# kiliant/zklaim

Measured on AMD Instinct MI355X. Metric: Groth16 proofs/sec (zklaim gadget, alt_bn128) + G1 MSM GB/s vs HBM roofline, higher is better.
Workload: dtype u32 limbs, Montgomery (254-bit Fq/Fr: 9 x 29-bit in the accumulation, reduction and NTT kernels, 8 x 32-bit elsewhere)

## Files before the change

### include/zkg.h

```cpp
#ifndef ZKG_H
#define ZKG_H

#include <stddef.h>
#include <stdint.h>

#ifdef __cplusplus
extern "C" {
#endif

#define ZKG_OK 0
#define ZKG_ERROR 1
#define ZKG_UNSATISFIED 2
#define ZKG_PROOF_BYTES 134

typedef struct zkg_r1cs {
    uint32_t num_variables;
    uint32_t num_inputs;
    uint32_t num_constraints;
    uint32_t reserved;
    const uint32_t *a_rowptr, *a_col; const uint64_t *a_val;
    const uint32_t *b_rowptr, *b_col; const uint64_t *b_val;
    const uint32_t *c_rowptr, *c_col; const uint64_t *c_val;
} zkg_r1cs;

typedef struct zkg_pk {
    zkg_r1cs cs;
    uint32_t log_m;
    uint32_t domain_size;
    const uint64_t *alpha_g1, *beta_g1, *delta_g1;
    const uint64_t *beta_g2, *delta_g2;
    const uint64_t *A_query;
    const uint64_t *B_g1;
    const uint64_t *B_g2;
    const uint64_t *H_query;
    const uint64_t *L_query;
} zkg_pk;

typedef struct zkg_crs zkg_crs;

int  zkg_init(int device);
void zkg_shutdown(void);
const char *zkg_last_error(void);
int  zkg_device_info(char *name, size_t name_len, int *compute_units);

int zkg_ntt(uint64_t *a, unsigned logN, int inverse, int coset);
int zkg_ntt_dev(void *d_a, unsigned logN, int inverse, int coset, void *stream);

int zkg_evaluation_domain_size(size_t min_size, size_t *m, int *is_step);
int zkg_ntt_domain(uint64_t *a, size_t m, int inverse, int coset);
int zkg_ntt_domain_dev(void *d_a, size_t m, int inverse, int coset, void *stream);

typedef struct zkg_domain zkg_domain;
zkg_domain *zkg_domain_new(size_t m);
void   zkg_domain_free(zkg_domain *d);
size_t zkg_domain_size(const zkg_domain *d);
size_t zkg_domain_batch_max(const zkg_domain *d);
void   zkg_domain_set_batch_max(zkg_domain *d, size_t k);
int zkg_domain_ntt_async(zkg_domain *d, void *d_a, size_t stride , size_t count,
                         int inverse, int coset, void *stream);
int zkg_domain_lagrange_async(zkg_domain *d, const uint64_t t[4], void *d_u, void *d_z, void *stream);
void zkg_domain_stats(size_t out[3]);

typedef struct zkg_qap zkg_qap;
zkg_qap *zkg_qap_new(const zkg_r1cs *cs);
void     zkg_qap_free(zkg_qap *q);
size_t   zkg_qap_domain_size(const zkg_qap *q);
uint32_t zkg_qap_num_variables(const zkg_qap *q);
size_t   zkg_qap_batch_max(const zkg_qap *q);
void     zkg_qap_set_batch_max(zkg_qap *q, size_t k);
int      zkg_qap_witness_h_async(zkg_qap *q, const void *d_witnesses, size_t stride , size_t count,
                                 void *d_h, size_t h_stride , uint32_t *d_unsat ,
                                 void *stream);
void     zkg_qap_stats(size_t out[3]);
int      zkg_qap_instance_async(zkg_qap *q, const uint64_t t[4] , void *d_abc ,
                                size_t stride , void *d_z , void *stream);
void     zkg_qap_set_column_segment(zkg_qap *q, size_t k);
void     zkg_qap_instance_stats(size_t out[2]);

int zkg_msm_g1(const uint64_t *bases, const uint64_t *scalars, size_t n, uint64_t out_jac[12]);
int zkg_msm_g2(const uint64_t *bases, const uint64_t *scalars, size_t n, uint64_t out_jac[24]);
#define ZKG_SCALARS_MONT 1
#define ZKG_SCALARS_MOSTLY_BITS 2
int zkg_msm_g1_dev(const void *d_bases, const void *d_scalars, size_t n, int scalars_mont,
                   uint64_t out_jac[12], void *stream);
int zkg_msm_g2_dev(const void *d_bases, const void *d_scalars, size_t n, int scalars_mont,
                   uint64_t out_jac[24], void *stream);
int zkg_msm_g1_host_scalars(const void *d_bases, const uint64_t *scalars, size_t n, int scalars_mont, uint64_t out_jac[12], void *stream);
int zkg_msm_host_scalars_stats(uint32_t *out, int n);
typedef struct zkg_msm_bases zkg_msm_bases;
zkg_msm_bases *zkg_msm_g1_bases_upload(const void *d_bases, size_t n);
int zkg_msm_g1_resident(zkg_msm_bases *bases, const void *d_scalars, size_t n, int scalars_mont, uint64_t out_jac[12], void *stream);
void zkg_msm_g1_bases_free(zkg_msm_bases *bases);
int zkg_msm_g1_resident_async(zkg_msm_bases *bases, const void *d_scalars, size_t n, size_t stride , size_t count,
                              int scalars_mont, void *d_out_jac , void *stream);
size_t zkg_msm_g1_resident_batch_max(const zkg_msm_bases *bases);
void zkg_msm_resident_async_stats(size_t out[3]);
int zkg_msm_combine_gpu(const uint64_t *records_jac, size_t cpw, int slots , int chunk_log, size_t vectors, uint64_t *out_jac);
typedef struct zkg_msm_g2_bases zkg_msm_g2_bases;
zkg_msm_g2_bases *zkg_msm_g2_bases_upload(const void *d_bases , size_t n);
void   zkg_msm_g2_bases_free(zkg_msm_g2_bases *bases);
int    zkg_msm_g2_resident(zkg_msm_g2_bases *bases, const void *d_scalars, size_t n, int scalars_mont, uint64_t out_jac[24], void *stream);
int    zkg_msm_g2_resident_async(zkg_msm_g2_bases *bases, const void *d_scalars, size_t n, size_t stride, size_t count,
                                 int scalars_mont, void *d_out_jac , void *stream);
size_t zkg_msm_g2_resident_batch_max(const zkg_msm_g2_bases *bases);
int    zkg_msm_combine_g2_gpu(const uint64_t *records_jac, size_t cpw, int chunk_log, size_t vectors, uint64_t *out_jac);
int zkg_msm_g1_windows_dev(const void *d_bases, const void *d_scalars, size_t n, int scalars_mont,
                           unsigned first_window, unsigned window_stride, uint64_t out_jac[12], void *stream);
int zkg_g1_sum(const uint64_t *points_jac, size_t count, uint64_t out_jac[12]);
int zkg_g2_sum(const uint64_t *points_jac, size_t count, uint64_t out_jac[24]);

typedef struct zkg_msm_shards zkg_msm_shards;
int zkg_init_multi(const int *devices, int ndev);
zkg_msm_shards *zkg_msm_g1_shards_upload(const uint64_t *bases, size_t n, const int *devices, int ndev);
void zkg_msm_g1_shards_free(zkg_msm_shards *shards);
size_t zkg_msm_g1_shards_count(const zkg_msm_shards *shards, size_t *points);
int zkg_msm_g1_multi(const zkg_msm_shards *shards, const uint64_t *scalars, uint64_t out_jac[12], uint64_t *partials_jac);
unsigned zkg_multi_rccl_calls(void);

int zkg_g1_fixed_base_dev(const uint64_t base[8], const void *d_scalars, size_t n, void *d_out_affine, void *stream);
int zkg_g2_fixed_base_dev(const uint64_t base[16], const void *d_scalars, size_t n, void *d_out_affine, void *stream);

zkg_crs *zkg_crs_upload(const zkg_pk *pk);
zkg_crs *zkg_crs_upload_blob(const void *pk_blob, size_t len);
int zkg_pk_blob_inspect(const void *pk_blob, size_t len, uint64_t out[8]);
void     zkg_crs_free(zkg_crs *crs);
int zkg_crs_shard_h(zkg_crs *crs, const int *devices, int ndev);
uint32_t zkg_crs_num_variables(const zkg_crs *crs);

int zkg_groth16_prove(const zkg_crs *crs, const uint64_t *witness, const uint64_t r[4],
                      const uint64_t s[4], int check_satisfied, uint8_t *proof_out, size_t *proof_len);
int zkg_groth16_prove_sparse(const zkg_crs *crs, const uint8_t *tags, const uint32_t *full_index, const uint64_t *full_values, size_t count,
                             const uint64_t r[4], const uint64_t s[4], int check_satisfied, uint8_t *proof_out, size_t *proof_len);
typedef struct zkg_prove_item {
    const uint64_t *witness;
    const uint8_t  *tags; const uint32_t *full_index; const uint64_t *full_values; size_t count;
    const uint64_t *r, *s;
} zkg_prove_item;
int zkg_groth16_prove_batch(const zkg_crs *crs, const zkg_prove_item *items, size_t count, int check_satisfied,
                            uint8_t *proofs_out , int *status );
void zkg_prove_batch_stats(size_t out[3]);
size_t zkg_prove_batch_chunk(const zkg_crs *crs);
int zkg_groth16_prove_dev(const zkg_crs *crs, const void *d_witness, const uint64_t r[4], const uint64_t s[4], int check_satisfied,
                          uint8_t *proof_out, size_t *proof_len, void *stream);
int zkg_groth16_prove_batch_dev(const zkg_crs *crs, const void *d_witnesses, size_t stride , size_t count,
                                const uint64_t *rs , int check_satisfied,
                                uint8_t *proofs_out , int *status , void *stream);
void zkg_prove_dev_stats(size_t out[2]);
struct zklaim_ctx;
int zkg_groth16_prove_batch_zklaim(const zkg_crs *crs, const struct zklaim_ctx *const *ctxs, size_t count, const uint64_t *rs ,
                                   int check_satisfied, uint8_t *proofs_out , int *status );
void zkg_zklaim_witness_stats(size_t out[2]);
size_t zkg_zklaim_witness_size(size_t payloads, size_t *cap_listed);
int zkg_zklaim_witness_gpu(const struct zklaim_ctx *const *ctxs, size_t count, uint8_t *tags_out , uint32_t *index_out,
                           uint64_t *values_out, size_t cap_listed , size_t *listed_counts);
int zkg_zklaim_witness_mirror(const struct zklaim_ctx *ctx, uint8_t *tags_out , uint32_t *index_out, uint64_t *values_out, size_t cap_listed,
                              size_t *listed_count);
int zkg_groth16_prove_zklaim(const zkg_crs *crs, const struct zklaim_ctx *ctx, const uint64_t r[4], const uint64_t s[4],
                             int check_satisfied, uint8_t *proof_out, size_t *proof_len);
void zkg_prove_zklaim_stats(size_t out[2]);
int zkg_zklaim_witness_gpu_parallel(const struct zklaim_ctx *const *ctxs, size_t count, uint8_t *tags_out , uint32_t *index_out,
                                    uint64_t *values_out, size_t cap_listed , size_t *listed_counts);
int zkg_zklaim_witness_mirror_parallel(const struct zklaim_ctx *ctx, uint8_t *tags_out , uint32_t *index_out, uint64_t *values_out,
                                       size_t cap_listed, size_t *listed_count);
int zkg_qap_witness_h(const zkg_crs *crs, const uint64_t *witness, uint64_t *h_out);
int zkg_prove_stage_ms(const zkg_crs *crs, float ms[8]);
int zkg_prover_peak_in_flight(int reset);

struct zklaim_ctx;
typedef struct zkg_circuit zkg_circuit;
#define ZKG_CIRCUIT_WITH_WITNESS 1
#define ZKG_CIRCUIT_REFERENCE_QUIRK 2
zkg_circuit *zkg_zklaim_circuit_new(const struct zklaim_ctx *ctx, int flags);
zkg_circuit *zkg_zklaim_witness_new(const struct zklaim_ctx *ctx);
uint32_t zkg_circuit_num_variables(const zkg_circuit *c);
void zkg_circuit_free(zkg_circuit *c);
int zkg_circuit_r1cs(const zkg_circuit *c, zkg_r1cs *out);
const uint64_t *zkg_circuit_witness(const zkg_circuit *c);
int zkg_circuit_sparse_witness(const zkg_circuit *c, const uint8_t **tags, const uint32_t **full_index, const uint64_t **full_values, size_t *count);
int zkg_circuit_is_satisfied(const zkg_circuit *c);
long zkg_circuit_first_unsatisfied(const zkg_circuit *c);
size_t zkg_zklaim_input_map(const struct zklaim_ctx *ctx, uint64_t *out, size_t cap_elems);

typedef struct zkg_keypair zkg_keypair;
zkg_keypair *zkg_groth16_setup(const zkg_r1cs *cs, const uint64_t *trapdoor);
zkg_keypair *zkg_groth16_setup_dev(const zkg_r1cs *cs, const uint64_t *trapdoor );
void zkg_keypair_free(zkg_keypair *kp);
const zkg_pk *zkg_keypair_pk(const zkg_keypair *kp);
int zkg_keypair_swapped(const zkg_keypair *kp);
size_t zkg_keypair_pk_blob(const zkg_keypair *kp, uint8_t *out, size_t cap);
size_t zkg_keypair_vk_blob(const zkg_keypair *kp, uint8_t *out, size_t cap);
int zkg_groth16_verify(const uint8_t *vk_blob, size_t vk_len, const uint64_t *primary_input, size_t n_inputs,
                       const uint8_t *proof, size_t proof_len);
int zkg_pairing_probe(const uint64_t a[4], const uint64_t b[4], uint8_t out[384]);
typedef struct zkg_verify_item {
    const uint8_t  *vk_blob;       size_t vk_len;
    const uint64_t *primary_input; size_t n_inputs;
    const uint8_t  *proof;         size_t proof_len;
} zkg_verify_item;
int zkg_groth16_verify_batch(const zkg_verify_item *items, size_t count, uint8_t *verdicts);
void zkg_verify_batch_stats(size_t out[3]);
int zkg_pairing_product(const uint64_t *g1_affine, const uint64_t *g2_affine, size_t n, uint8_t out[384]);
int  zkg_groth16_verify_each(const zkg_verify_item *items, size_t count, uint8_t *verdicts);
void zkg_verify_each_stats(size_t out[3]);
void zkg_verify_each_set_chunk(size_t positions);
int  zkg_pairing_each(const uint64_t *g1_affine, const uint64_t *g2_affine, size_t items, size_t pairs, uint8_t *out);
int  zkg_final_exp(const uint8_t *in, size_t n, int where, uint8_t *out);
int zkg_pairing_selfcheck(const uint32_t *e, int nlimbs);

int libsnark_trusted_setup(struct zklaim_ctx *ctx);
int libsnark_prove(struct zklaim_ctx *ctx);
int libsnark_verify(struct zklaim_ctx *ctx);
void zkg_compat_reset(void);
int zkg_zklaim_prove_batch(struct zklaim_ctx *const *ctxs, size_t count, int *rc);
int zkg_zklaim_verify_batch(struct zklaim_ctx *const *ctxs, size_t count, int *rc);
void zkg_zklaim_verify_batch_stats(size_t out[4]);
int zkg_proof_decode_gpu(const uint8_t *proofs, size_t count, uint64_t *A, uint64_t *B, uint64_t *C, uint8_t *ok);
int zkg_zklaim_input_sums_gpu(const struct zklaim_ctx *const *ctxs, size_t count, const uint32_t *weights, const uint8_t *mask,
                              size_t lo, size_t hi, uint64_t *sums_out, size_t cap_elems, size_t *n_elems);
size_t zkg_zklaim_input_map_mirror(const struct zklaim_ctx *ctx, uint64_t *out, size_t cap_elems);
int  zkg_zklaim_verify_each(struct zklaim_ctx *const *ctxs, size_t count, int *rc);
void zkg_zklaim_verify_each_stats(size_t out[4]);
int zkg_zklaim_ic_each(const uint64_t *ic0, const uint64_t *ic, const struct zklaim_ctx *const *ctxs, size_t count, int where, uint64_t *out);

int zkg_point_decompress(const uint8_t *records, size_t stride, size_t offset, size_t n, int g2, int where, uint64_t *out, uint32_t *flag);
int zkg_point_compress(const uint64_t *g1, const uint64_t *g2, const uint32_t *idx, size_t npoints, size_t n, int rec, int where, uint8_t *out,
                       uint8_t guard[16]);

int zkg_field_op(int field, int op, const uint64_t *a, const uint64_t *b, size_t n, uint64_t *out);

int zkg_fr29_op(int op, const uint32_t *in, size_t n, uint32_t *out);

int zkg_fq29_op(int op, const uint32_t *in, size_t n, uint32_t *out);
int zkg_fq29_op_chain(int op, int chain, const uint32_t *in, size_t n, uint32_t *out);

int zkg_fq12_op(int op, const uint32_t *a, const uint32_t *b, size_t n, int where, uint32_t *out);

int zkg_g1_add_quad29(const uint64_t *a_jac, const uint64_t *b_jac, size_t n, int chain, uint64_t *out_jac);
int zkg_g1_add_pair29(const uint64_t *a_jac, const uint64_t *b_jac, size_t n, int chain, uint64_t *out_jac);

int zkg_curve_op(int group, int op, const uint32_t *a, const uint32_t *b, const uint32_t *k, size_t n, int chain, uint32_t *out);

// ... 8 lines not shown
```

### zklaim_amd/__init__.py

```python
from .api import (ZkgError, device_info, evaluation_domain_size, fixed_base_g1_dev, fixed_base_g2_dev, g1_sum, g2_sum, init, lib, msm_g1, msm_g1_dev, msm_g1_windows_dev,
                  msm_g2, msm_g2_dev, ntt, ntt_dev, shutdown, timing_dominant_ms, timing_reset, Crs, PK, R1CS, make_r1cs, make_pk,
                  DECLARED_SYMBOLS, ZklaimCircuit, ZklaimCtx, make_ctx, zklaim_input_map, OPS, Keypair, groth16_verify, groth16_verify_batch, verify_batch_stats, groth16_prove_batch, prove_batch_stats, groth16_prove_batch_dev, prove_dev_stats, groth16_prove_batch_zklaim, zklaim_witness_stats, zklaim_witness_size, zklaim_witness_mirror, zklaim_witness_gpu, zklaim_witness_mirror_parallel, zklaim_witness_gpu_parallel, prove_zklaim_stats, pairing_product, pairing_probe, pairing_selfcheck,
                  libsnark_trusted_setup, libsnark_prove, libsnark_verify, zklaim_prove_batch, zklaim_verify_batch, zklaim_verify_batch_stats, proof_decode_gpu, zklaim_input_sums_gpu, zklaim_input_map_mirror, ctx_blob, COMPAT_SYMBOLS, field_op, fr29_op, FR29_OPS, fq29_op, FQ29_OPS, g1_add_quad29, g1_add_pair29, curve_op, CURVE_OPS, OK, ERROR, UNSATISFIED, init_multi, MsmShards, pk_blob_inspect, ResidentBases, msm_g1_host_scalars, msm_host_scalars_stats, msm_resident_async_stats, msm_combine_gpu, ResidentBasesG2, msm_combine_g2_gpu,
                  groth16_verify_each, verify_each_stats, verify_each_set_chunk, pairing_each, final_exp, fq12_op, FQ12_OPS,
                  point_decompress, point_compress, zklaim_verify_each, zklaim_verify_each_stats, zklaim_ic_each,
                  Domain, domain_stats, Qap, qap_stats, qap_instance_stats)
```

### zklaim_amd/api.py

```python
import ctypes as C
import os
import sys

import numpy as np

_HERE = os.path.dirname(os.path.abspath(__file__))
_SO = os.path.join(_HERE, "libzkg.so")

DECLARED_SYMBOLS = [
    "zkg_init", "zkg_shutdown", "zkg_last_error", "zkg_device_info", "zkg_ntt", "zkg_ntt_dev", "zkg_evaluation_domain_size", "zkg_ntt_domain", "zkg_ntt_domain_dev", "zkg_msm_g1", "zkg_msm_g2",
    "zkg_msm_g1_dev", "zkg_msm_g2_dev", "zkg_msm_g1_windows_dev", "zkg_g1_sum", "zkg_g2_sum", "zkg_g1_fixed_base_dev", "zkg_g2_fixed_base_dev",
    "zkg_groth16_prove_batch_zklaim", "zkg_zklaim_witness_stats", "zkg_zklaim_witness_size", "zkg_zklaim_witness_gpu", "zkg_zklaim_witness_mirror",
    "zkg_crs_upload", "zkg_crs_upload_blob", "zkg_pk_blob_inspect", "zkg_crs_free", "zkg_crs_num_variables", "zkg_groth16_prove", "zkg_groth16_prove_sparse", "zkg_circuit_sparse_witness", "zkg_qap_witness_h", "zkg_prove_stage_ms", "zkg_timing_reset",
    "zkg_timing_dominant_ms", "zkg_zklaim_circuit_new", "zkg_zklaim_witness_new", "zkg_circuit_num_variables", "zkg_circuit_free", "zkg_circuit_r1cs", "zkg_circuit_witness",
    "zkg_circuit_is_satisfied", "zkg_circuit_first_unsatisfied", "zkg_zklaim_input_map", "zkg_groth16_setup", "zkg_keypair_free",
    "zkg_keypair_pk", "zkg_keypair_swapped", "zkg_keypair_pk_blob", "zkg_keypair_vk_blob", "zkg_groth16_verify", "zkg_pairing_probe", "zkg_pairing_selfcheck",
    "zkg_compat_reset", "zkg_field_op", "zkg_init_multi", "zkg_msm_g1_shards_upload", "zkg_msm_g1_shards_free", "zkg_msm_g1_shards_count",
    "zkg_msm_g1_multi", "zkg_g1_add_quad29", "zkg_crs_shard_h", "zkg_msm_g1_bases_upload", "zkg_msm_g1_resident", "zkg_msm_g1_bases_free",
    "zkg_prover_peak_in_flight", "zkg_msm_g1_host_scalars", "zkg_multi_rccl_calls", "zkg_g1_add_pair29",
    "zkg_groth16_verify_batch", "zkg_pairing_product", "zkg_verify_batch_stats",
    "zkg_groth16_prove_batch", "zkg_prove_batch_stats", "zkg_prove_batch_chunk", "zkg_zklaim_prove_batch",
    "zkg_groth16_prove_zklaim", "zkg_prove_zklaim_stats", "zkg_zklaim_witness_gpu_parallel", "zkg_zklaim_witness_mirror_parallel",
    "zkg_fr29_op", "zkg_fq29_op", "zkg_fq29_op_chain",
    "zkg_zklaim_verify_batch", "zkg_zklaim_verify_batch_stats", "zkg_proof_decode_gpu", "zkg_zklaim_input_sums_gpu", "zkg_zklaim_input_map_mirror",
    "zkg_groth16_prove_dev", "zkg_groth16_prove_batch_dev", "zkg_prove_dev_stats",
    "zkg_msm_g1_resident_async", "zkg_msm_g1_resident_batch_max", "zkg_msm_resident_async_stats", "zkg_msm_combine_gpu",
    "zkg_groth16_verify_each", "zkg_verify_each_stats", "zkg_verify_each_set_chunk", "zkg_pairing_each", "zkg_final_exp",
    "zkg_fq12_op", "zkg_point_decompress", "zkg_point_compress",
    "zkg_zklaim_verify_each", "zkg_zklaim_verify_each_stats", "zkg_zklaim_ic_each",
    "zkg_curve_op",
    "zkg_domain_new", "zkg_domain_free", "zkg_domain_size", "zkg_domain_batch_max", "zkg_domain_set_batch_max", "zkg_domain_ntt_async",
    "zkg_domain_lagrange_async", "zkg_domain_stats",
    "zkg_msm_g2_bases_upload", "zkg_msm_g2_bases_free", "zkg_msm_g2_resident", "zkg_msm_g2_resident_async", "zkg_msm_g2_resident_batch_max",
    "zkg_msm_combine_g2_gpu",
    "zkg_qap_new", "zkg_qap_free", "zkg_qap_domain_size", "zkg_qap_num_variables", "zkg_qap_batch_max", "zkg_qap_set_batch_max",
    "zkg_qap_witness_h_async", "zkg_qap_stats",
    "zkg_qap_instance_async", "zkg_qap_set_column_segment", "zkg_qap_instance_stats", "zkg_groth16_setup_dev",
    "zkg_msm_host_scalars_stats",
]
COMPAT_SYMBOLS = ["libsnark_trusted_setup", "libsnark_prove", "libsnark_verify"]


OK, ERROR, UNSATISFIED = 0, 1, 2


class ZkgError(RuntimeError):
    pass


class R1CS(C.Structure):
    _fields_ = [("num_variables", C.c_uint32), ("num_inputs", C.c_uint32), ("num_constraints", C.c_uint32), ("reserved", C.c_uint32)] + \
        [(f"{m}_{f}", C.c_void_p) for m in "abc" for f in ("rowptr", "col", "val")]


class PK(C.Structure):
    _fields_ = [("cs", R1CS), ("log_m", C.c_uint32), ("domain_size", C.c_uint32)] + \
        [(k, C.c_void_p) for k in ("alpha_g1", "beta_g1", "delta_g1", "beta_g2", "delta_g2", "A_query", "B_g1", "B_g2", "H_query", "L_query")]


_lib = None


def lib():
    global _lib
    if _lib is None:
        if not os.path.exists(_SO):
            raise ZkgError(f"{_SO} is missing: build it with `python -m zklaim_amd.build` (hipcc, gfx950)")
        if "torch" not in sys.modules and not os.environ.get("ZKG_NO_TORCH"):
            try:
                import torch
            except Exception:
                pass
        _lib = C.CDLL(_SO)
        _lib.zkg_last_error.restype = C.c_char_p
        _lib.zkg_timing_dominant_ms.restype = C.c_float
        _lib.zkg_crs_upload.restype = C.c_void_p
        _lib.zkg_crs_upload.argtypes = [C.c_void_p]
        _lib.zkg_crs_upload_blob.restype = C.c_void_p
        _lib.zkg_crs_upload_blob.argtypes = [C.c_void_p, C.c_size_t]
        _lib.zkg_crs_free.argtypes = [C.c_void_p]
    return _lib


def _check(rc, what):
    if rc != 0:
        raise ZkgError(f"{what} failed (rc={rc}): {lib().zkg_last_error().decode()}")


def _p(a):
    return None if a is None else a.ctypes.data_as(C.c_void_p)


def _u64(a):
    return np.ascontiguousarray(a, dtype=np.uint64)


def _vp(x):
    return C.c_void_p(int(x) if x else 0)


_initialised = False


def init(device=0):
    global _initialised
    _check(lib().zkg_init(int(device)), "zkg_init")
    _initialised = True


def shutdown():
    global _initialised
    if _initialised:
        lib().zkg_shutdown()
    _initialised = False


def device_info():
    name = C.create_string_buffer(128); cus = C.c_int(0)
    _check(lib().zkg_device_info(name, C.c_size_t(128), C.byref(cus)), "zkg_device_info")
    return name.value.decode(), cus.value


def field_op(field, op, a, b=None):
    a = _u64(a); limbs = 8 if field == 2 else 4
    out = np.zeros_like(a)
    bb = None if b is None else _u64(b)
    _check(lib().zkg_field_op(int(field), int(op), _p(a), _p(bb), C.c_size_t(a.size // limbs), _p(out)), "zkg_field_op")
    return out


FR29_OPS = {"mul": (0, 2, 1), "mul2": (1, 4, 2), "norm": (2, 1, 1), "add_norm": (3, 2, 1), "sub_norm": (4, 2, 1), "add_lazy": (5, 2, 1), "sub_lazy": (6, 2, 1),
            "slice": (7, 1, 1), "unslice_reduce": (8, 1, 1), "r4": (9, 7, 4), "r4_stage0": (10, 7, 4), "r4_norm_stores": (11, 7, 4),
            "r4_stage0_norm_stores": (12, 7, 4), "r2_tail": (13, 3, 2), "r2_tail_stage0": (14, 3, 2)}


def fr29_op(name, x):
    op, k, m = FR29_OPS[name]
    x = np.ascontiguousarray(x, dtype=np.uint32)
    if x.ndim != 3 or x.shape[1:] != (k, 9):
        raise ZkgError(f"fr29_op {name}: input must be (n, {k}, 9), got {x.shape}")
    out = np.zeros((x.shape[0], m, 9), np.uint32)
    _check(lib().zkg_fr29_op(int(op), _p(x), C.c_size_t(x.shape[0]), _p(out)), "zkg_fr29_op")
    return out


FQ29_OPS = {"mul": (0, 2, 1), "mul2": (1, 4, 2), "sqr": (2, 1, 1), "sqr2": (3, 2, 2), "norm": (4, 1, 1), "add": (5, 2, 1), "dbl": (6, 1, 1),
            "sub_S2_1": (7, 2, 1), "sub_S4_1": (8, 2, 1), "sub_S6_1": (9, 2, 1), "sub_S4_3": (10, 2, 1), "neg_S2_1": (11, 1, 1), "is_zero": (12, 1, 1),
            "unpack": (13, 1, 1), "to29": (14, 1, 1), "from29": (15, 1, 1), "rec64": (16, 3, 3), "bucket29": (17, 5, 4), "inverse": (18, 1, 1),
            "madd": (19, 7, 5), "add_lane": (20, 8, 4), "add_pair": (21, 8, 4), "add_quad": (22, 8, 4)}


def fq29_op(name, x, chain=0):
    op, k, m = FQ29_OPS[name]
    x = np.ascontiguousarray(x, dtype=np.uint32)
    if x.ndim != 3 or x.shape[1:] != (k, 9):
        raise ZkgError(f"fq29_op {name}: input must be (n, {k}, 9), got {x.shape}")
    out = np.zeros((x.shape[0], m, 9), np.uint32)
    _check(lib().zkg_fq29_op_chain(int(op), int(chain), _p(x), C.c_size_t(x.shape[0]), _p(out)), "zkg_fq29_op")
    return out


def g1_add_quad29(a_jac, b_jac, chain=0):
    a = _u64(a_jac); b = _u64(b_jac); out = np.zeros_like(a)
    _check(lib().zkg_g1_add_quad29(_p(a), _p(b), C.c_size_t(a.size // 12), int(chain), _p(out)), "zkg_g1_add_quad29")
    return out.reshape(-1, 12)


def g1_add_pair29(a_jac, b_jac, chain=0):
    a = _u64(a_jac); b = _u64(b_jac); out = np.zeros_like(a)
    _check(lib().zkg_g1_add_pair29(_p(a), _p(b), C.c_size_t(a.size // 12), int(chain), _p(out)), "zkg_g1_add_pair29")
    return out.reshape(-1, 12)


CURVE_OPS = {"madd": 0, "add": 1, "add_quad": 2, "dbl": 3, "dbl_affine": 4, "to_affine": 5, "mul": 6}


def curve_op(group, name, a, b=None, k=None, chain=0):
    op = CURVE_OPS[name]; w = 16 if group else 8
    a = np.ascontiguousarray(a, dtype=np.uint32)
    need_a = 2 if name == "dbl_affine" else 4
    if a.ndim != 3 or a.shape[1:] != (need_a, w):
        raise ZkgError(f"curve_op {name}: a must be (n, {need_a}, {w}), got {a.shape}")
    n = a.shape[0]
    if name in ("madd", "add", "add_quad"):
        need_b = 2 if name == "madd" else 4
        b = np.ascontiguousarray(b, dtype=np.uint32)
        if b.shape != (n, need_b, w):
            raise ZkgError(f"curve_op {name}: b must be ({n}, {need_b}, {w}), got {b.shape}")
    else:
        b = None
    if name == "mul":
# ... 77 lines not shown

    def free(self):
        if self._h:
            lib().zkg_domain_free(C.c_void_p(self._h)); self._h = None


def domain_stats():
    out = (C.c_size_t * 3)()
    lib().zkg_domain_stats(out)
    return tuple(int(v) for v in out)


class Qap:

    def __init__(self, cs):
        L = lib()
        L.zkg_qap_new.restype = C.c_void_p
        L.zkg_qap_new.argtypes = [C.c_void_p]
        L.zkg_qap_free.argtypes = [C.c_void_p]
        for name in ("zkg_qap_domain_size", "zkg_qap_batch_max"):
            getattr(L, name).restype = C.c_size_t
            getattr(L, name).argtypes = [C.c_void_p]
        L.zkg_qap_num_variables.restype = C.c_uint32
        L.zkg_qap_num_variables.argtypes = [C.c_void_p]
        L.zkg_qap_set_batch_max.argtypes = [C.c_void_p, C.c_size_t]
        L.zkg_qap_witness_h_async.argtypes = [C.c_void_p, C.c_void_p, C.c_size_t, C.c_size_t, C.c_void_p, C.c_size_t, C.c_void_p, C.c_void_p]
        L.zkg_qap_instance_async.argtypes = [C.c_void_p, C.c_void_p, C.c_void_p, C.c_size_t, C.c_void_p, C.c_void_p]
        L.zkg_qap_set_column_segment.argtypes = [C.c_void_p, C.c_size_t]
        self._h = L.zkg_qap_new(C.byref(cs))
        if not self._h:
            raise ZkgError("zkg_qap_new failed: " + L.zkg_last_error().decode())
        self.m, self.n = self.domain_size(), self.num_variables()

    def witness_h_async(self, d_w_ptr, count, stride, d_h_ptr, h_stride, d_unsat_ptr=0, stream=0):
        _check(lib().zkg_qap_witness_h_async(C.c_void_p(self._h), _vp(d_w_ptr), C.c_size_t(stride), C.c_size_t(count), _vp(d_h_ptr), C.c_size_t(h_stride),
                                             _vp(d_unsat_ptr), _vp(stream)), "zkg_qap_witness_h_async")

    def instance_async(self, t, d_abc_ptr, stride=None, d_z_ptr=0, stream=0):
        tt = None if t is None else _u64(t).reshape(-1)
        if tt is not None and tt.size != 4:
            raise ZkgError("zkg_qap_instance_async: t is 4 limbs")
        _check(lib().zkg_qap_instance_async(C.c_void_p(self._h), _p(tt), _vp(d_abc_ptr), C.c_size_t(self.n + 1 if stride is None else stride), _vp(d_z_ptr),
                                            _vp(stream)), "zkg_qap_instance_async")

    def set_column_segment(self, k):
        lib().zkg_qap_set_column_segment(C.c_void_p(self._h), C.c_size_t(k))

    def domain_size(self):
        return int(lib().zkg_qap_domain_size(C.c_void_p(self._h)))

    def num_variables(self):
        return int(lib().zkg_qap_num_variables(C.c_void_p(self._h)))

    def batch_max(self):
        return int(lib().zkg_qap_batch_max(C.c_void_p(self._h)))

    def set_batch_max(self, k):
        lib().zkg_qap_set_batch_max(C.c_void_p(self._h), C.c_size_t(k))

    def free(self):
        if self._h:
            lib().zkg_qap_free(C.c_void_p(self._h)); self._h = None


def qap_stats():
    out = (C.c_size_t * 3)()
    lib().zkg_qap_stats(out)
    return tuple(int(v) for v in out)


def qap_instance_stats():
    out = (C.c_size_t * 2)()
    lib().zkg_qap_instance_stats(out)
    return tuple(int(v) for v in out)


def msm_g1(bases, scalars):
    bases = _u64(bases); scalars = _u64(scalars); out = np.zeros(12, np.uint64)
    _check(lib().zkg_msm_g1(_p(bases), _p(scalars), C.c_size_t(scalars.size // 4), _p(out)), "zkg_msm_g1")
    return out


def msm_g2(bases, scalars):
    bases = _u64(bases); scalars = _u64(scalars); out = np.zeros(24, np.uint64)
    _check(lib().zkg_msm_g2(_p(bases), _p(scalars), C.c_size_t(scalars.size // 4), _p(out)), "zkg_msm_g2")
    return out


def init_multi(devices):
    global _initialised
    d = (C.c_int * len(devices))(*devices)
    _check(lib().zkg_init_multi(d, len(devices)), "zkg_init_multi")
    _initialised = True


class MsmShards:

    def __init__(self, bases, devices):
        bases = _u64(bases)
        L = lib()
        L.zkg_msm_g1_shards_upload.restype = C.c_void_p
        L.zkg_msm_g1_shards_upload.argtypes = [C.c_void_p, C.c_size_t, C.c_void_p, C.c_int]
        L.zkg_msm_g1_shards_free.argtypes = [C.c_void_p]
        L.zkg_msm_g1_multi.argtypes = [C.c_void_p, C.c_void_p, C.c_void_p, C.c_void_p]
        d = (C.c_int * len(devices))(*devices)
        self.n = bases.size // 8; self.ndev = len(devices)
        self._h = L.zkg_msm_g1_shards_upload(_p(bases), self.n, d, len(devices))
        if not self._h:
            raise ZkgError("zkg_msm_g1_shards_upload failed: " + L.zkg_last_error().decode())

    def msm(self, scalars, with_partials=False):
        scalars = _u64(scalars); out = np.zeros(12, np.uint64); parts = np.zeros((self.ndev, 12), np.uint64)
        assert scalars.size // 4 == self.n
        _check(lib().zkg_msm_g1_multi(C.c_void_p(self._h), _p(scalars), _p(out), _p(parts)), "zkg_msm_g1_multi")
        return (out, parts) if with_partials else out

    def free(self):
        if self._h:
            lib().zkg_msm_g1_shards_free(C.c_void_p(self._h)); self._h = None

    def __del__(self):
        try:
            self.free()
        except Exception:
            pass


SCALARS_MONT, SCALARS_MOSTLY_BITS = 1, 2


def msm_g1_dev(d_bases, d_scalars, n, scalars_mont=False, stream=0, mostly_bits=False):
    out = np.zeros(12, np.uint64)
    flags = (SCALARS_MONT if scalars_mont else 0) | (SCALARS_MOSTLY_BITS if mostly_bits else 0)
    _check(lib().zkg_msm_g1_dev(_vp(d_bases), _vp(d_scalars), C.c_size_t(n), flags, _p(out), _vp(stream)), "zkg_msm_g1_dev")
    return out


def msm_g1_host_scalars(d_bases, scalars_host_ptr, n, scalars_mont=False, stream=0):
    out = np.zeros(12, np.uint64)
    lib().zkg_msm_g1_host_scalars.argtypes = [C.c_void_p, C.c_void_p, C.c_size_t, C.c_int, C.c_void_p, C.c_void_p]
    _check(lib().zkg_msm_g1_host_scalars(_vp(d_bases), _vp(scalars_host_ptr), C.c_size_t(n), SCALARS_MONT if scalars_mont else 0, _p(out), _vp(stream)), "zkg_msm_g1_host_scalars")
    return out


def msm_host_scalars_stats():
    out = (C.c_uint32 * 18)()
    words = lib().zkg_msm_host_scalars_stats(out, 18)
    if words < 2:
        return None
    pieces = int(out[0])
    return {"pieces": pieces, "stream_waits": int(out[1]),
            "heavy": [None if out[2 + 2 * k] == 0xFFFFFFFF else int(out[2 + 2 * k]) for k in range(pieces)],
            "pair": [bool(out[3 + 2 * k]) for k in range(pieces)]}


class _ResidentBases:
    _PREFIX = None
    _LIMBS = 0

    def _fn(self, suffix, argtypes, restype=C.c_int):
        fn = getattr(lib(), self._PREFIX + suffix)
        fn.argtypes = argtypes; fn.restype = restype
        return fn

    def __init__(self, d_bases, n):
        self._h = self._fn("_bases_upload", [C.c_void_p, C.c_size_t], C.c_void_p)(_vp(d_bases), C.c_size_t(n))
        if not self._h:
            raise ZkgError(self._PREFIX + "_bases_upload failed: " + last_error())
        self.n = n

    def msm(self, d_scalars, scalars_mont=False, stream=0):
        out = np.zeros(self._LIMBS, np.uint64)
        fn = self._fn("_resident", [C.c_void_p, C.c_void_p, C.c_size_t, C.c_int, C.c_void_p, C.c_void_p])
        _check(fn(C.c_void_p(self._h), _vp(d_scalars), C.c_size_t(self.n), SCALARS_MONT if scalars_mont else 0, _p(out), _vp(stream)), self._PREFIX + "_resident")
        return out

    def msm_async(self, d_scalars_ptr, d_out_ptr, count=1, stride=None, scalars_mont=False, stream=0):
        fn = self._fn("_resident_async", [C.c_void_p, C.c_void_p, C.c_size_t, C.c_size_t, C.c_size_t, C.c_int, C.c_void_p, C.c_void_p])
        _check(fn(C.c_void_p(self._h), _vp(d_scalars_ptr), C.c_size_t(self.n), C.c_size_t(self.n if stride is None else stride),
                  C.c_size_t(count), SCALARS_MONT if scalars_mont else 0, _vp(d_out_ptr), _vp(stream)), self._PREFIX + "_resident_async")

    def batch_max(self):
        return int(self._fn("_resident_batch_max", [C.c_void_p], C.c_size_t)(C.c_void_p(self._h)))

    def free(self):
        if self._h:
            self._fn("_bases_free", [C.c_void_p], None)(C.c_void_p(self._h)); self._h = None


class ResidentBases(_ResidentBases):
    _PREFIX = "zkg_msm_g1"
    _LIMBS = 12


class ResidentBasesG2(_ResidentBases):
    _PREFIX = "zkg_msm_g2"
    _LIMBS = 24


def msm_resident_async_stats():
    out = (C.c_size_t * 3)()
    lib().zkg_msm_resident_async_stats(out)
    return tuple(int(v) for v in out)


def _msm_combine(name, limbs, records_jac, cpw, slots, chunk_log, vectors, slot_args):
    rec = _u64(records_jac)
    if rec.size != vectors * cpw * slots * limbs:
        raise ZkgError("%s: records_jac must hold vectors x cpw x %s points of %d limbs" % (name, "slots" if slot_args else slots, limbs))
    out = np.zeros((vectors, limbs), np.uint64)
    fn = getattr(lib(), "zkg_" + name)
    fn.argtypes = [C.c_void_p, C.c_size_t] + [C.c_int] * len(slot_args) + [C.c_int, C.c_size_t, C.c_void_p]
    _check(fn(_p(rec), C.c_size_t(cpw), *slot_args, int(chunk_log), C.c_size_t(vectors), _p(out)), "zkg_" + name)
    return out


def msm_combine_gpu(records_jac, cpw, slots, chunk_log, vectors=1):
    return _msm_combine("msm_combine_gpu", 12, records_jac, cpw, slots, chunk_log, vectors, [int(slots)])


def msm_combine_g2_gpu(records_jac, cpw, chunk_log, vectors=1):
    return _msm_combine("msm_combine_g2_gpu", 24, records_jac, cpw, 2, chunk_log, vectors, [])


def msm_g1_windows_dev(d_bases, d_scalars, n, first_window, window_stride, scalars_mont=False, stream=0):
    out = np.zeros(12, np.uint64)
    _check(lib().zkg_msm_g1_windows_dev(_vp(d_bases), _vp(d_scalars), C.c_size_t(n), int(scalars_mont), C.c_uint(first_window), C.c_uint(window_stride),
                                        _p(out), _vp(stream)), "zkg_msm_g1_windows_dev")
    return out


def msm_g2_dev(d_bases, d_scalars, n, scalars_mont=False, stream=0, mostly_bits=False):
    out = np.zeros(24, np.uint64)
    flags = (SCALARS_MONT if scalars_mont else 0) | (SCALARS_MOSTLY_BITS if mostly_bits else 0)
    _check(lib().zkg_msm_g2_dev(_vp(d_bases), _vp(d_scalars), C.c_size_t(n), flags, _p(out), _vp(stream)), "zkg_msm_g2_dev")
    return out


def g1_sum(points_jac):
    pts = _u64(points_jac); out = np.zeros(12, np.uint64)
    _check(lib().zkg_g1_sum(_p(pts), C.c_size_t(pts.size // 12), _p(out)), "zkg_g1_sum")
    return out


def g2_sum(points_jac):
    pts = _u64(points_jac); out = np.zeros(24, np.uint64)
    _check(lib().zkg_g2_sum(_p(pts), C.c_size_t(pts.size // 24), _p(out)), "zkg_g2_sum")
    return out


def fixed_base_g1_dev(base, d_scalars, n, d_out, stream=0):
    base = _u64(base)
    _check(lib().zkg_g1_fixed_base_dev(_p(base), _vp(d_scalars), C.c_size_t(n), _vp(d_out), _vp(stream)), "zkg_g1_fixed_base_dev")


def fixed_base_g2_dev(base, d_scalars, n, d_out, stream=0):
    base = _u64(base)
    _check(lib().zkg_g2_fixed_base_dev(_p(base), _vp(d_scalars), C.c_size_t(n), _vp(d_out), _vp(stream)), "zkg_g2_fixed_base_dev")


def timing_reset():
    lib().zkg_timing_reset()


def timing_dominant_ms():
    n = C.c_int(0)
    ms = lib().zkg_timing_dominant_ms(C.byref(n))
    return float(ms), n.value


def make_r1cs(n, l, A, B, Cm, keep):
    cs = R1CS()
    cs.num_variables, cs.num_inputs, cs.num_constraints = n, l, len(A[0]) - 1
    for name, (rp, col, val) in zip("abc", (A, B, Cm)):
        rp = np.ascontiguousarray(rp, np.uint32); col = np.ascontiguousarray(col, np.uint32); val = _u64(val)
        keep += [rp, col, val]
        setattr(cs, f"{name}_rowptr", rp.ctypes.data); setattr(cs, f"{name}_col", col.ctypes.data); setattr(cs, f"{name}_val", val.ctypes.data)
    return cs


def make_pk(cs, arrays, log_m, keep, domain_size=0):
    pk = PK(); pk.cs = cs; pk.log_m = log_m; pk.domain_size = domain_size
    for k in ("alpha_g1", "beta_g1", "delta_g1", "beta_g2", "delta_g2", "A_query", "B_g1", "B_g2", "H_query", "L_query"):
        a = _u64(arrays[k]); keep.append(a)
        setattr(pk, k, a.ctypes.data)
    return pk


class Crs:

    def __init__(self, pk=None, blob=None, m=None):
        if blob is not None:
            buf = (C.c_ubyte * len(blob)).from_buffer_copy(blob)
            self._h = lib().zkg_crs_upload_blob(C.cast(buf, C.c_void_p), C.c_size_t(len(blob)))
            self.m = m
        else:
            self._h = lib().zkg_crs_upload(C.byref(pk))
            self.m = pk.domain_size or (1 << pk.log_m)
        if not self._h:
            raise ZkgError("zkg_crs_upload failed: " + lib().zkg_last_error().decode())

    def prove(self, witness, r, s, check_satisfied=True):
        out = np.zeros(256, np.uint8); ln = C.c_size_t(0)
        rc = lib().zkg_groth16_prove(C.c_void_p(self._h), _p(_u64(witness)), _p(_u64(r)), _p(_u64(s)), int(check_satisfied), _p(out), C.byref(ln))
        if rc not in (OK, UNSATISFIED):
            _check(rc, "zkg_groth16_prove")
# ... 664 lines not shown
```

### zklaim_amd/csrc/capi.hip

```cpp
#include "common.hpp"
#include "fq29.hip.hpp"
#include "fr29.hip.hpp"
#include "../../include/zkg.h"
#include <atomic>
#include <condition_variable>
#include <cstring>
#include <memory>
#include <mutex>
#include <thread>
#include <dlfcn.h>
#include <rccl/rccl.h>

namespace zk {

static thread_local std::string t_error;
static std::string g_error;
static std::mutex g_err_mu;
void set_error(const std::string &msg) { t_error = msg; std::lock_guard<std::mutex> lk(g_err_mu); g_error = msg; }
bool hip_ok(hipError_t e, const char *what, const char *file, int line) {
    if (e == hipSuccess) return true;
    set_error(std::string(what) + ": " + hipGetErrorString(e) + " at " + file + ":" + std::to_string(line));
    return false;
}

// ... 584 lines not shown
        hip_ok(hipDeviceSynchronize(), "sync", __FILE__, __LINE__) &&
        hip_ok(hipMemcpy(a, buf.p, bytes, hipMemcpyDeviceToHost), "D2H", __FILE__, __LINE__)) rc = ZKG_OK;
    buf.release();
    return rc;
}

int zkg_evaluation_domain_size(size_t min_size, size_t *m, int *is_step) {
    DomainShape sh;
    if (!evaluation_domain_shape(min_size, sh)) { set_error("zkg_evaluation_domain_size: no radix-2 or step domain for that size"); return ZKG_ERROR; }
    if (m) *m = sh.m;
    if (is_step) *is_step = sh.step ? 1 : 0;
    return ZKG_OK;
}
int zkg_ntt_domain_dev(void *d_a, size_t m, int inverse, int coset, void *stream) {
    REQUIRE_INIT();
    DomainShape sh;
    if (!domain_shape_of(m, sh)) { set_error("zkg_ntt_domain: m is neither 2^k nor 2^a + 2^b (get_evaluation_domain would not return it)"); return ZKG_ERROR; }
    if (!sh.step) return zkg_ntt_dev(d_a, sh.log_m, inverse, coset, stream);
    hipStream_t s = (hipStream_t)stream;
    StepDomain *d = step_domain(m, s);
    if (!d) return ZKG_ERROR;
    DevBuf scratch;
    if (scratch.reserve(m * NTT_SCRATCH_BYTES)) return ZKG_ERROR;
    int rc = step_ntt_run(d, (Fr *)d_a, inverse != 0, coset != 0, s, scratch.as<Fr>());
    if (!hip_ok(hipStreamSynchronize(s), "sync", __FILE__, __LINE__)) rc = ZKG_ERROR;
    scratch.release();
    return rc;
}
int zkg_ntt_domain(uint64_t *a, size_t m, int inverse, int coset) {
    REQUIRE_INIT();
    if (!a || m < 2) { set_error("zkg_ntt_domain: bad argument"); return ZKG_ERROR; }
    std::lock_guard<std::mutex> lk(g_host_ntt_mu);
    size_t bytes = m * 32;
    DevBuf buf;
    if (buf.reserve(bytes)) return ZKG_ERROR;
    int rc = ZKG_ERROR;
    if (hip_ok(hipMemcpy(buf.p, a, bytes, hipMemcpyHostToDevice), "H2D", __FILE__, __LINE__) &&
        zkg_ntt_domain_dev(buf.p, m, inverse, coset, nullptr) == ZKG_OK &&
        hip_ok(hipDeviceSynchronize(), "sync", __FILE__, __LINE__) &&
        hip_ok(hipMemcpy(a, buf.p, bytes, hipMemcpyDeviceToHost), "D2H", __FILE__, __LINE__)) rc = ZKG_OK;
    buf.release();
    return rc;
}

static constexpr size_t DOMAIN_WORKSPACE_CAP = (size_t)1 << 30;
static constexpr size_t DOMAIN_MAX_GROUP = 65535;
struct zkg_domain {
    DomainShape sh; int device = 0; std::mutex mu;
    DevBuf scratch;
    HandleOrder order;
    size_t bmax_default = 1, bmax = 1;
};
static thread_local size_t t_domain_stats[3];
static zkg_domain *domain_new_impl(size_t m) {
    if (g_device < 0) { set_error("zkg_init not called"); return nullptr; }
    DomainShape sh;
    if (m < 2 || !domain_shape_of(m, sh)) { set_error("zkg_domain_new: m is neither 2^k (k <= 28) nor 2^a + 2^b (get_evaluation_domain would not return it)"); return nullptr; }
    if (wrong_device_refused("zkg_domain_new", g_device, "zkg_init selected (the domain tables live there)")) return nullptr;
    std::unique_ptr<zkg_domain> d(new zkg_domain());
    d->sh = sh; d->device = g_device;
    d->bmax_default = d->bmax = std::max<size_t>(1, std::min(DOMAIN_MAX_GROUP, DOMAIN_WORKSPACE_CAP / (m * NTT_SCRATCH_BYTES)));
    const bool tables = sh.step ? step_domain(m, nullptr) != nullptr : ntt_domain(sh.log_m, nullptr) != nullptr;
    if (!tables || !hip_ok(hipStreamSynchronize(nullptr), "hipStreamSynchronize", __FILE__, __LINE__) || d->order.create()) return nullptr;
    return d.release();
}
static int domain_ntt_async_impl(zkg_domain *d, void *d_a, size_t stride, size_t count, int inverse, int coset, void *stream) {
    static const char *who = "zkg_domain_ntt_async";
    for (size_t &v : t_domain_stats) v = 0;
    if (count == 0) return ZKG_OK;
    REQUIRE_INIT();
    if (!d || !d_a) { set_error(std::string(who) + ": bad argument (null handle or pointer)"); return ZKG_ERROR; }
    const size_t m = d->sh.m;
    if (async_vectors_refused(who, m, "m", stride, count, d->device, "the handle was made on") ||
        dev_range_refused(d_a, ((count - 1) * stride + m) * 32, 16, d->device, who, "d_a", "handle")) return ZKG_ERROR;
    hipStream_t s = (hipStream_t)stream;
    std::lock_guard<std::mutex> lk(d->mu);
    NttDomain *nd = nullptr; StepDomain *sd = nullptr;
    if (d->sh.step) sd = step_domain(m, s); else nd = ntt_domain(d->sh.log_m, s);
    if (!nd && !sd) return ZKG_ERROR;
    size_t waits = 0, groups = 0, done = 0;
    const size_t need = std::min(d->bmax, count) * m * NTT_SCRATCH_BYTES;
    if (d->order.grow(d->scratch, need, waits) || d->order.order_behind(s)) return ZKG_ERROR;
    Fr *a = (Fr *)d_a;
    int rc = ZKG_OK;
    while (done < count && rc == ZKG_OK) {
        const size_t g = std::min(d->bmax, count - done);
        Fr *ag = a + done * stride;
        const hipEvent_t ev = done + g == count ? d->order.ev : nullptr;
        rc = sd ? step_ntt_run(sd, ag, inverse != 0, coset != 0, s, d->scratch.as<Fr>(), (unsigned)g, stride, m, ev)
                : ntt_run(nd, ag, inverse, coset, s, d->scratch.as<Fr>(), (unsigned)g, stride, m, ev);
        if (rc == ZKG_OK) { done += g; ++groups; }
    }
    t_domain_stats[0] = done; t_domain_stats[1] = groups; t_domain_stats[2] = waits;
    if (rc == ZKG_OK) { d->order.carried(s); return ZKG_OK; }
    d->order.record(s);
    return ZKG_ERROR;
}
static int domain_lagrange_async_impl(zkg_domain *d, const uint64_t t[4], void *d_u, void *d_z, void *stream) {
    static const char *who = "zkg_domain_lagrange_async";
    REQUIRE_INIT();
    if (!d || !t || !d_u) { set_error(std::string(who) + ": bad argument (null handle or pointer)"); return ZKG_ERROR; }
    if (wrong_device_refused(who, d->device, "the handle was made on") || dev_range_refused(d_u, d->sh.m * 32, 16, d->device, who, "d_u", "handle") ||
        (d_z && dev_range_refused(d_z, 32, 16, d->device, who, "d_z", "handle"))) return ZKG_ERROR;
    Fr tf; memcpy(tf.v, t, 32);
    hipStream_t s = (hipStream_t)stream;
    std::lock_guard<std::mutex> lk(d->mu);
    if (d->order.order_behind(s) || domain_lagrange_dev(d->sh, tf, (Fr *)d_u, (Fr *)d_z, s, d->order.ev)) return ZKG_ERROR;
    d->order.carried(s);
    return ZKG_OK;
}
zkg_domain *zkg_domain_new(size_t m) { return c_boundary<zkg_domain *>("zkg_domain_new", nullptr, [&] { return domain_new_impl(m); }); }
void zkg_domain_free(zkg_domain *d) {
    if (!d) return;
    c_boundary("zkg_domain_free", 0, [&] {
        int cur = 0; (void)hipGetDevice(&cur);
        if (cur != d->device) (void)hipSetDevice(d->device);
        d->order.destroy();
        d->scratch.release();
        if (cur != d->device) (void)hipSetDevice(cur);
        delete d;
        return 0;
    });
}
size_t zkg_domain_size(const zkg_domain *d) { return d ? d->sh.m : 0; }
size_t zkg_domain_batch_max(const zkg_domain *d) { return d ? d->bmax : 0; }
void zkg_domain_set_batch_max(zkg_domain *d, size_t k) {
    if (!d) return;
    c_boundary("zkg_domain_set_batch_max", 0, [&] { std::lock_guard<std::mutex> lk(d->mu); d->bmax = clamp_batch_max(k, d->bmax_default); return 0; });
}
int zkg_domain_ntt_async(zkg_domain *d, void *d_a, size_t stride, size_t count, int inverse, int coset, void *stream) {
    return c_boundary("zkg_domain_ntt_async", ZKG_ERROR, [&] { return domain_ntt_async_impl(d, d_a, stride, count, inverse, coset, stream); });
}
int zkg_domain_lagrange_async(zkg_domain *d, const uint64_t t[4], void *d_u, void *d_z, void *stream) {
    return c_boundary("zkg_domain_lagrange_async", ZKG_ERROR, [&] { return domain_lagrange_async_impl(d, t, d_u, d_z, stream); });
}
void zkg_domain_stats(size_t out[3]) { if (out) for (int i = 0; i < 3; ++i) out[i] = t_domain_stats[i]; }

int zkg_msm_g1_dev(const void *d_bases, const void *d_scalars, size_t n, int scalars_mont, uint64_t out_jac[12], void *stream) {
    REQUIRE_INIT();
    G1 r;
    if (msm_g1((const G1Affine *)d_bases, (const uint32_t *)d_scalars, n, (scalars_mont & ZKG_SCALARS_MONT) != 0, &r, (hipStream_t)stream, (scalars_mont & ZKG_SCALARS_MOSTLY_BITS) != 0)) return ZKG_ERROR;
    store_norm(out_jac, r);
    return ZKG_OK;
}
int zkg_msm_g1_host_scalars(const void *d_bases, const uint64_t *scalars, size_t n, int scalars_mont, uint64_t out_jac[12], void *stream) {
    REQUIRE_INIT();
    if (!out_jac || (n && (!d_bases || !scalars))) { set_error("zkg_msm_g1_host_scalars: bad argument"); return ZKG_ERROR; }
    G1 r;
    if (msm_g1_host_scalars((const G1Affine *)d_bases, (const uint32_t *)scalars, n, (scalars_mont & ZKG_SCALARS_MONT) != 0, &r, (hipStream_t)stream)) return ZKG_ERROR;
    store_norm(out_jac, r);
    return ZKG_OK;
}
int zkg_msm_host_scalars_stats(uint32_t *out, int n) { return out && n >= 0 ? msm_host_scalars_stats(out, n) : 0; }
int zkg_msm_g1_windows_dev(const void *d_bases, const void *d_scalars, size_t n, int scalars_mont, unsigned first_window, unsigned window_stride,
                           uint64_t out_jac[12], void *stream) {
    REQUIRE_INIT();
    if (!window_stride) { set_error("zkg_msm_g1_windows_dev: window_stride must be positive"); return ZKG_ERROR; }
    G1 r; const G1Affine *b = (const G1Affine *)d_bases;
    if (msm_shared(&b, 1, nullptr, (const uint32_t *)d_scalars, n, (scalars_mont & ZKG_SCALARS_MONT) != 0, &r, nullptr, (hipStream_t)stream, first_window, window_stride,
                   (scalars_mont & ZKG_SCALARS_MOSTLY_BITS) != 0)) return ZKG_ERROR;
    store_norm(out_jac, r);
    return ZKG_OK;
}
struct MsmResident { WindowTable table; MsmJob *job = nullptr; std::mutex mu; int device = 0; hipEvent_t ev_in = nullptr, ev_out = nullptr; };
struct zkg_msm_bases : MsmResident {};
struct zkg_msm_g2_bases : MsmResident {};
struct MsmResidentG1 { using Handle = zkg_msm_bases; using Point = G1; static constexpr bool g2 = false; static constexpr size_t limbs = 12; static constexpr unsigned n_log = 27; static constexpr const char *prefix = "zkg_msm_g1"; };
struct MsmResidentG2 { using Handle = zkg_msm_g2_bases; using Point = G2; static constexpr bool g2 = true; static constexpr size_t limbs = 24; static constexpr unsigned n_log = 25; static constexpr const char *prefix = "zkg_msm_g2"; };
static constexpr size_t G2_RESIDENT_BUCKET_CAP = (size_t)1 << 30;

extern "C++" {
static void resident_free(MsmResident *h) {
    int cur = 0; (void)hipGetDevice(&cur);
    if (cur != h->device) (void)hipSetDevice(h->device);
    if (h->job) { (void)hipStreamSynchronize(msm_job_stream(h->job)); msm_job_destroy(h->job); }
    if (h->ev_in) (void)hipEventDestroy(h->ev_in);
    if (h->ev_out) (void)hipEventDestroy(h->ev_out);
    h->table.release();
    if (cur != h->device) (void)hipSetDevice(cur);
}
template <class G> static typename G::Handle *resident_upload(const void *d_bases, size_t n) {
    const std::string who = std::string(G::prefix) + "_bases_upload";
    if (g_device < 0) { set_error("zkg_init not called"); return nullptr; }
    if (!d_bases || n == 0 || n >= ((size_t)1 << G::n_log)) { set_error(who + ": bad argument (1 <= n < 2^" + std::to_string(G::n_log) + ")"); return nullptr; }
    typename G::Handle *h = new (std::nothrow) typename G::Handle();
    if (!h) { set_error(who + ": out of memory"); return nullptr; }
    (void)hipGetDevice(&h->device);
    h->job = msm_job_create(nullptr, true);
    bool ok = h->job != nullptr && hip_ok(hipEventCreateWithFlags(&h->ev_in, hipEventDisableTiming), "hipEventCreate", __FILE__, __LINE__) &&
              hip_ok(hipEventCreateWithFlags(&h->ev_out, hipEventDisableTiming), "hipEventCreate", __FILE__, __LINE__);
    if constexpr (G::g2) ok = ok && window_table_build_g2(h->table, (const G2Affine *)d_bases, n, table_window_bits(n), nullptr) == 0;
    else ok = ok && window_table_build_g1(h->table, (const G1Affine *)d_bases, n, table_window_bits(n), nullptr) == 0 && window_table_records29(h->table, nullptr) == 0;
    if (!ok || !hip_ok(hipDeviceSynchronize(), "sync", __FILE__, __LINE__)) { resident_free(h); delete h; return nullptr; }
    msm_job_set_window(h->job, h->table.c);
    if constexpr (!G::g2) msm_job_set_row_merge(h->job, n >= 49152 ? 2u : 1u);
    return h;
}
static MsmBases resident_table_set(const MsmResident *h) { MsmBases b; b.p = h->table.buf.p; b.g2 = h->table.g2; b.level_stride = h->table.n; b.p29 = h->table.rec29.p; return b; }
template <class G> static int resident_sync(MsmResident *h, const void *d_scalars, size_t n, int scalars_mont, uint64_t *out_jac, void *stream) {
    const std::string who = std::string(G::prefix) + "_resident";
    REQUIRE_INIT();
    if (!h || !d_scalars || !out_jac || n != h->table.n) { set_error(who + ": bad argument (n must be the handle's point count)"); return ZKG_ERROR; }
    if (wrong_device_refused(who.c_str(), h->device, "the bases were uploaded on")) return ZKG_ERROR;
    std::lock_guard<std::mutex> lk(h->mu);
    ZK_HIP(hipEventRecord(h->ev_in, (hipStream_t)stream));
    ZK_HIP(hipStreamWaitEvent(msm_job_stream(h->job), h->ev_in, 0));
    const MsmBases b = resident_table_set(h);
    typename G::Point r;
    msm_job_set_device_finish(h->job, false);
    int rc;
    {
        ReserveGuard guard(msm_job_stream(h->job));
        rc = msm_job_launch(h->job, &b, 1, (const uint32_t *)d_scalars, n, (scalars_mont & ZKG_SCALARS_MONT) != 0, nullptr);
    }
    if constexpr (G::g2) rc = rc || msm_job_finish(h->job, nullptr, &r); else rc = rc || msm_job_finish(h->job, &r, nullptr);
    if (rc) return ZKG_ERROR;
    store_norm(out_jac, r);
    return ZKG_OK;
}
static thread_local size_t t_resident_async_stats[3];
template <class G> static size_t resident_batch_max(const MsmResident *h) {
    size_t p = MSM_MULTI_MAX_VECTORS;
    if constexpr (G::g2) p = std::min<size_t>(p, std::max<size_t>(1, G2_RESIDENT_BUCKET_CAP / msm_table_bucket_bytes(h->table.c, true)));
    while (p > 1 && !msm_multi_supported(h->table.n, h->table.c, (uint32_t)p)) --p;
    return p;
}
template <class G> static int resident_async(MsmResident *h, const void *d_scalars, size_t n, size_t stride, size_t count, int scalars_mont, void *d_out_jac, void *stream) {
    const std::string who_s = std::string(G::prefix) + "_resident_async"; const char *who = who_s.c_str();
    for (size_t &v : t_resident_async_stats) v = 0;
    if (count == 0) return ZKG_OK;
    REQUIRE_INIT();
    if (!h || !d_scalars || !d_out_jac || n != h->table.n) { set_error(who_s + ": bad argument (n must be the handle's point count)"); return ZKG_ERROR; }
    if (async_vectors_refused(who, n, "n", stride, count, h->device, "the bases were uploaded on")) return ZKG_ERROR;
    if (dev_range_refused(d_scalars, ((count - 1) * stride + n) * 32, 16, h->device, who, "d_scalars", "handle") ||
        dev_range_refused(d_out_jac, count * G::limbs * 8, 8, h->device, who, "d_out_jac", "handle")) return ZKG_ERROR;
    const size_t bmax = resident_batch_max<G>(h);
    const bool mont = (scalars_mont & ZKG_SCALARS_MONT) != 0;
    const uint32_t *sc = (const uint32_t *)d_scalars; uint64_t *out = (uint64_t *)d_out_jac;
    std::lock_guard<std::mutex> lk(h->mu);
    hipStream_t js = msm_job_stream(h->job);
    ZK_HIP(hipEventRecord(h->ev_in, (hipStream_t)stream));
    ZK_HIP(hipStreamWaitEvent(js, h->ev_in, 0));
    const MsmBases b = resident_table_set(h);
    msm_job_set_device_finish(h->job, true);
    int rc = ZKG_OK;
    size_t groups = 0, waits = 0, done = 0;
    while (done < count && rc == ZKG_OK) {
        const size_t g = std::min(bmax, count - done);
        ReserveGuard guard(js);
        const uint32_t *sg = sc + done * stride * 8;
        rc = g > 1 ? msm_job_launch_multi(h->job, &b, 1, sg, n, stride * 8, (uint32_t)g, mont) : msm_job_launch(h->job, &b, 1, sg, n, mont, nullptr);
        if (rc == ZKG_OK) rc = msm_job_finish_dev(h->job, out + done * G::limbs);
        waits += guard.drains;
        if (rc == ZKG_OK) { done += g; ++groups; }
    }
    const bool ordered = hip_ok(hipEventRecord(h->ev_out, js), "hipEventRecord", __FILE__, __LINE__) &&
                         hip_ok(hipStreamWaitEvent((hipStream_t)stream, h->ev_out, 0), "hipStreamWaitEvent", __FILE__, __LINE__);
    t_resident_async_stats[0] = done; t_resident_async_stats[1] = groups; t_resident_async_stats[2] = waits;
    return rc == ZKG_OK && ordered ? ZKG_OK : ZKG_ERROR;
}
}
void zkg_msm_resident_async_stats(size_t out[3]) { if (out) for (int i = 0; i < 3; ++i) out[i] = t_resident_async_stats[i]; }
#define ZKG_RESIDENT_ENTRIES(NAME, G)                                                                                                                       \
    G::Handle *NAME##_bases_upload(const void *d_bases, size_t n) {                                                                                         \
        return c_boundary<G::Handle *>(#NAME "_bases_upload", nullptr, [&] { return resident_upload<G>(d_bases, n); });                                    \
    }                                                                                                                                                       \
    void NAME##_bases_free(G::Handle *h) {                                                                                                                  \
        if (h) c_boundary(#NAME "_bases_free", 0, [&] { resident_free(h); delete h; return 0; });                                                           \
    }                                                                                                                                                       \
    int NAME##_resident(G::Handle *h, const void *d_scalars, size_t n, int scalars_mont, uint64_t *out_jac, void *stream) {                                \
        return c_boundary(#NAME "_resident", ZKG_ERROR, [&] { return resident_sync<G>(h, d_scalars, n, scalars_mont, out_jac, stream); });                  \
    }                                                                                                                                                       \
    int NAME##_resident_async(G::Handle *h, const void *d_scalars, size_t n, size_t stride, size_t count, int scalars_mont, void *d_out_jac, void *stream) { \
        return c_boundary(#NAME "_resident_async", ZKG_ERROR, [&] { return resident_async<G>(h, d_scalars, n, stride, count, scalars_mont, d_out_jac, stream); }); \
    }                                                                                                                                                       \
    size_t NAME##_resident_batch_max(const G::Handle *h) {                                                                                                  \
        return h ? c_boundary<size_t>(#NAME "_resident_batch_max", 0, [&] { return resident_batch_max<G>(h); }) : 0;                                        \
    }
ZKG_RESIDENT_ENTRIES(zkg_msm_g1, MsmResidentG1)
ZKG_RESIDENT_ENTRIES(zkg_msm_g2, MsmResidentG2)
#undef ZKG_RESIDENT_ENTRIES
int zkg_msm_combine_gpu(const uint64_t *records_jac, size_t cpw, int slots, int chunk_log, size_t vectors, uint64_t *out_jac) {
    return c_boundary("zkg_msm_combine_gpu", ZKG_ERROR, [&]() -> int { REQUIRE_INIT(); return msm_combine_records(false, records_jac, cpw, slots, chunk_log, vectors, out_jac); });
}
int zkg_msm_combine_g2_gpu(const uint64_t *records_jac, size_t cpw, int chunk_log, size_t vectors, uint64_t *out_jac) {
    return c_boundary("zkg_msm_combine_g2_gpu", ZKG_ERROR, [&]() -> int { REQUIRE_INIT(); return msm_combine_records(true, records_jac, cpw, 2, chunk_log, vectors, out_jac); });
}
int zkg_msm_g2_dev(const void *d_bases, const void *d_scalars, size_t n, int scalars_mont, uint64_t out_jac[24], void *stream) {
    REQUIRE_INIT();
    G2 r;
    if (msm_g2((const G2Affine *)d_bases, (const uint32_t *)d_scalars, n, (scalars_mont & ZKG_SCALARS_MONT) != 0, &r, (hipStream_t)stream, (scalars_mont & ZKG_SCALARS_MOSTLY_BITS) != 0)) return ZKG_ERROR;
    store_norm(out_jac, r);
    return ZKG_OK;
}
static int msm_host(const uint64_t *bases, const uint64_t *scalars, size_t n, uint64_t *out, int g2) {
    REQUIRE_INIT();
    if (n && (!bases || !scalars)) { set_error("zkg_msm: null input"); return ZKG_ERROR; }
    size_t bb = n * (g2 ? 128 : 64), sb = n * 32;
    DevBuf db, ds;
    if (db.reserve(bb + 16) || ds.reserve(sb + 16)) return ZKG_ERROR;
    int rc = ZKG_ERROR;
    if ((!n || (hip_ok(hipMemcpy(db.p, bases, bb, hipMemcpyHostToDevice), "H2D", __FILE__, __LINE__) &&
                hip_ok(hipMemcpy(ds.p, scalars, sb, hipMemcpyHostToDevice), "H2D", __FILE__, __LINE__))))
        rc = g2 ? zkg_msm_g2_dev(db.p, ds.p, n, 0, out, nullptr) : zkg_msm_g1_dev(db.p, ds.p, n, 0, out, nullptr);
    db.release(); ds.release();
    return rc;
// ... 301 lines not shown
```

### zklaim_amd/csrc/common.hpp

```cpp
#pragma once
#include <hip/hip_runtime.h>
#include <stdint.h>
#include <stddef.h>
#include <string>
#include <vector>
#include <functional>
#include <map>
#include <mutex>
#include "curve.hip.hpp"
#include "c_boundary.hpp"

struct zklaim_ctx;

namespace zk {

bool hip_ok(hipError_t e, const char *what, const char *file, int line);
#define ZK_HIP(expr) do { if (!::zk::hip_ok((expr), #expr, __FILE__, __LINE__)) return ZKG_ERROR; } while (0)
#define ZK_HIP_V(expr) do { if (!::zk::hip_ok((expr), #expr, __FILE__, __LINE__)) return; } while (0)

struct DevBuf {
    void *p = nullptr; size_t cap = 0;
    int reserve(size_t bytes);
    void release();
    template <class T> T *as() const { return reinterpret_cast<T *>(p); }
};

struct ReserveGuard;
extern thread_local ReserveGuard *t_reserve_guard;
struct ReserveGuard {
    hipStream_t stream; size_t drains = 0; ReserveGuard *prev;
    explicit ReserveGuard(hipStream_t s) : stream(s), prev(t_reserve_guard) { t_reserve_guard = this; }
    ReserveGuard(const ReserveGuard &) = delete;
    ReserveGuard &operator=(const ReserveGuard &) = delete;
    ~ReserveGuard() { t_reserve_guard = prev; }
};

struct ScopedDevBuf : DevBuf {
    ScopedDevBuf() = default;
    ScopedDevBuf(const ScopedDevBuf &) = delete;
    ScopedDevBuf &operator=(const ScopedDevBuf &) = delete;
    ~ScopedDevBuf() { release(); }
};

struct HandleOrder {
    hipEvent_t ev = nullptr; bool pending = false; hipStream_t last = nullptr;
    int create();
    int order_behind(hipStream_t s);
    int wait_host();
    int grow(DevBuf &ws, size_t need, size_t &waits);
    void carried(hipStream_t s) { pending = true; last = s; }
    void record(hipStream_t s);
    void destroy();
};
inline size_t clamp_batch_max(size_t k, size_t dflt) { return k == 0 || k > dflt ? dflt : k; }

struct KernelTimer {
    std::vector<std::pair<hipEvent_t, hipEvent_t>> pairs; size_t used = 0; bool enabled = true, pending = false;
    size_t calls = 0, calls_seen = 0, calls_timed = 0; bool sample = true;
    void new_call();
    void begin(hipStream_t s); void end(hipStream_t s);
    float drain(int *launches);
    void reset();
};
extern KernelTimer g_dominant_timer;

void host_parallel_for(int n, const std::function<void(int)> &fn);
void host_parallel_for_wait(int n, const std::function<void(int)> &fn);
void host_parallel_for_spawn(int n, const std::function<void(int)> &fn);

struct NttDomain {
    unsigned logn = 0;
    DevBuf tw_fwd, tw_inv;
    DevBuf coset_pre;
    DevBuf icoset_post;
    DevBuf tw_fwd29, tw_inv29, coset_pre29, icoset_post29;
    DevBuf scratch;
    Fr n_inv;
    std::mutex mu; bool first_stream_set = false; hipStream_t first_stream = nullptr;
    std::map<hipStream_t, DevBuf> stream_scratch;
    Fr *scratch_for(hipStream_t s);
    int init(unsigned logn, hipStream_t s);
    void release();
};
NttDomain *ntt_domain(unsigned logn, hipStream_t s);
int ntt_run(NttDomain *d, Fr *d_a, int inverse, int coset, hipStream_t s, Fr *scratch = nullptr, unsigned batch = 1, size_t batch_stride = 0,
            size_t scratch_stride = 0, hipEvent_t done = nullptr);
static constexpr size_t NTT_SCRATCH_BYTES = 40;
int ntt_run_ex(NttDomain *d, Fr *d_a, bool inverse, const Fr *pre, const Fr *post, const Fr *post_scalar, hipStream_t s, Fr *scratch = nullptr,
               unsigned batch = 1, size_t batch_stride = 0, const void *pre29 = nullptr, const void *post29 = nullptr, size_t scratch_stride = 0, hipEvent_t done = nullptr);
int ntt_table29(DevBuf &out, const Fr *d_in, size_t n, hipStream_t s);

struct DomainShape { size_t m = 0, big = 0, small = 0; bool step = false; unsigned log_m = 0;  };
bool evaluation_domain_shape(size_t min_size, DomainShape &d);
bool domain_shape_of(size_t m, DomainShape &d);
Fr fr_root_of_unity_pow2(unsigned logn);
int domain_lagrange(const DomainShape &d, const Fr &t, std::vector<Fr> &u, Fr &Zt);
Fr domain_vanishing_at(const DomainShape &d, const Fr &t);
int domain_lagrange_dev(const DomainShape &d, const Fr &t, Fr *d_u, Fr *d_z, hipStream_t s, hipEvent_t done = nullptr);

struct StepDomain {
    DomainShape shape;
    NttDomain *dbig = nullptr, *dsmall = nullptr;
    DevBuf w;
    DevBuf winv_half;
    DevBuf g_pow, ginv_pow;
    DevBuf zinv;
    Fr zinv_small;
    Fr big_inv, small_inv, half;
    int init(const DomainShape &sh, hipStream_t s);
    void release();
};
StepDomain *step_domain(size_t m, hipStream_t s);
int step_ntt_run(StepDomain *d, Fr *d_a, bool inverse, bool coset, hipStream_t s, Fr *scratch, unsigned batch = 1, size_t batch_stride = 0,
                 size_t scratch_stride = 0, hipEvent_t done = nullptr);
int powers_table(Fr *d_out, size_t n, const Fr &base, const Fr &scale, hipStream_t s);
void ntt_release_all();
int ntt_configure();

static constexpr int MSM_MAX_SETS = 4;
struct MsmBases { const void *p = nullptr; bool g2 = false; size_t level_stride = 0; uint32_t index_sub = 0; const uint32_t *remap = nullptr; const void *p29 = nullptr; };
struct OwnedCsr { std::vector<uint32_t> rp[3], col[3]; std::vector<uint64_t> val[3]; };
struct WindowTable { DevBuf buf, rec29; size_t n = 0; int c = 0, W = 0; bool g2 = false; void release() { buf.release(); rec29.release(); n = 0; } };
int window_table_records29(WindowTable &t, hipStream_t s);
int window_table_build_g1(WindowTable &t, const G1Affine *d_bases, size_t n, int c, hipStream_t s);
int table_window_bits(size_t n);
int window_table_build_g2(WindowTable &t, const G2Affine *d_bases, size_t n, int c, hipStream_t s);
struct MsmJob;
MsmJob *msm_job_create(hipStream_t s, bool own_stream, bool high_priority = false);
hipStream_t msm_job_stream(MsmJob *j);
void msm_job_set_window_subset(MsmJob *j, uint32_t w0, uint32_t ws);
void msm_job_set_skewed(MsmJob *j, bool skewed);
void msm_job_set_row_merge(MsmJob *j, uint32_t f);
void msm_job_set_window(MsmJob *j, int c);
void msm_job_set_critical(MsmJob *j, bool critical);
static constexpr unsigned CRIT_PRIORITY_MIN_LOG = 20;
bool crit_priority_for(int part, unsigned log_m);
bool crit_priority_enabled();
void msm_job_destroy(MsmJob *j);
int msm_job_launch(MsmJob *job, const MsmBases *sets, int nsets, const uint32_t *d_scalars, size_t n, bool scalars_mont, const uint32_t *d_gather = nullptr);
int msm_job_finish(MsmJob *job, G1 *out_g1, G2 *out_g2);
bool msm_multi_supported(size_t n, int c, uint32_t count);
static constexpr uint32_t MSM_MULTI_MAX_VECTORS = 16;
static constexpr size_t ZKG_MSM_ASYNC_MAX_COUNT = (size_t)1 << 24, ZKG_MSM_ASYNC_MAX_STRIDE = (size_t)1 << 32;
int msm_job_launch_multi(MsmJob *job, const MsmBases *sets, int nsets, const uint32_t *d_scalars, size_t n, size_t scalar_stride, uint32_t count, bool scalars_mont);
int msm_job_finish_multi(MsmJob *job, G1 *out_g1, G2 *out_g2);
void msm_job_set_device_finish(MsmJob *j, bool on);
int msm_job_finish_dev(MsmJob *job, uint64_t *d_out);
int msm_combine_records(bool g2, const uint64_t *records_jac, size_t cpw, int slots, int chunk_log, size_t vectors, uint64_t *out_jac);
size_t msm_table_bucket_bytes(int c, bool g2);
static constexpr uint32_t SUBSET_NONE = 0xffffffffu;
int witness_classify(const Fr *d_z, size_t n1, uint8_t *d_tags, uint32_t *d_listed, uint32_t *d_count, hipStream_t s, const uint32_t *d_subset_pos = nullptr);
int gather_points_g1(const G1Affine *d_src, const uint32_t *d_idx, size_t count, uint32_t index_sub, G1Affine *d_out, hipStream_t s);
int gather_points_g2(const G2Affine *d_src, const uint32_t *d_idx, size_t count, uint32_t index_sub, G2Affine *d_out, hipStream_t s);
int scatter_points_g1(const G1Affine *d_src, const uint32_t *d_idx, size_t count, G1Affine *d_out, hipStream_t s);
int scatter_points_g2(const G2Affine *d_src, const uint32_t *d_idx, size_t count, G2Affine *d_out, hipStream_t s);
struct OnesSum {
    DevBuf partials; void *host = nullptr; size_t host_bytes = 0; bool g2 = false; int nsets = 0; void release();
    const G1 &g1(int i) const { return reinterpret_cast<const G1 *>(host)[i]; }
    const G2 &g2pt(int i) const { return reinterpret_cast<const G2 *>(host)[i]; }
};
int ones_sum_launch(OnesSum &o, const MsmBases *sets, int nsets, const uint8_t *d_tags, size_t n1, hipStream_t s);
int ones_sum_launch_multi(OnesSum &o, const MsmBases *sets, int nsets, const uint8_t *d_tags, size_t tag_stride, size_t n1, uint32_t count, hipStream_t s);
int msm_g1(const G1Affine *d_bases, const uint32_t *d_scalars, size_t n, bool scalars_mont, G1 *out, hipStream_t s, bool mostly_bits = false);
int msm_g2(const G2Affine *d_bases, const uint32_t *d_scalars, size_t n, bool scalars_mont, G2 *out, hipStream_t s, bool mostly_bits = false);
int msm_g1_host_scalars(const G1Affine *d_bases, const uint32_t *h_scalars, size_t n, bool scalars_mont, G1 *out, hipStream_t s);
int msm_host_scalars_stats(uint32_t *out, int n);
int msm_shared(const G1Affine *const *d_g1_bases, int n_g1, const G2Affine *d_g2_bases, const uint32_t *d_scalars, size_t n,
               bool scalars_mont, G1 *out_g1, G2 *out_g2, hipStream_t s, uint32_t w0 = 0, uint32_t ws = 1,
               bool mostly_bits = false);
int fixed_base_g1(const G1Affine &base, const uint32_t *d_scalars, size_t n, G1Affine *d_out, hipStream_t s, bool scalars_mont = false);
int fixed_base_g2(const G2Affine &base, const uint32_t *d_scalars, size_t n, G2Affine *d_out, hipStream_t s, bool scalars_mont = false);
void msm_release_all();
int msm_configure();

int compress_g1_records(const G1Affine *d_in, size_t n, uint8_t *d_out, hipStream_t s);
int compress_kc_records(const G2Affine *d_g2, const G1Affine *d_g1, const uint32_t *d_idx, size_t nidx, uint8_t *d_out, hipStream_t s);

static constexpr size_t VERIFY_PROD_BLOCKS = 64;
int verify_g2_subgroup(const G2Affine *d_B, size_t n, uint8_t *d_ok, hipStream_t s);
int verify_g1_mul128(const G1Affine *d_in, const uint32_t *d_w, size_t nw, size_t n, G1Affine *d_out, hipStream_t s);
int verify_miller(const G1Affine *d_P, const G2Affine *d_Q, const uint8_t *d_use, size_t n, void *d_out, hipStream_t s);
int verify_fq12_product(const void *d_in, size_t lo, size_t hi, void *d_partial, void *d_out, hipStream_t s);
int verify_proof_decode_b(const uint8_t *d_rec, size_t n, G2Affine *d_B, uint8_t *d_dec, hipStream_t s);
int verify_proof_decode_ac(const uint8_t *d_rec, size_t n, G1Affine *d_AC, uint8_t *d_dec, hipStream_t s);
int verify_use_mask(size_t n, const uint8_t *d_in_g2, const uint8_t *d_dec_b, const uint8_t *d_dec_ac, uint8_t *d_use, hipStream_t s);
static constexpr size_t ZV_SUM_SLICES = 16;
int verify_zklaim_input_sums(const uint8_t *d_pub, uint32_t npl, size_t base, const uint32_t *d_w, const uint8_t *d_mask, size_t lo, size_t hi,
                             void *d_part, void *d_out, hipStream_t s);
size_t zklaim_bit_table_entries(uint32_t npl);
size_t zklaim_bit_table_tmp_bytes(uint32_t npl);
int verify_zklaim_bit_table(const G1Affine *d_ic, uint32_t npl, void *d_tmp, G1Affine *d_T, hipStream_t s);
int verify_zklaim_ic_each(const G1Affine *d_ic0, const G1Affine *d_T, const uint8_t *d_pub, uint32_t npl, size_t n, G1Affine *d_out,
                          const G1Affine *d_c, G1Affine *d_negc, hipStream_t s);
void zklaim_ic_each_device_code_on_host(const G1Affine &ic0, const G1Affine *ic, const uint8_t *pub, uint32_t npl, size_t n, G1Affine *out);
void verify_keys_release_all();
int initialised_device();
int dev_range_refused(const void *d, size_t bytes, size_t align, int device, const char *who, const char *what, const char *owner);
int wrong_device_refused(const char *who, int device, const char *made);
int async_vectors_refused(const char *who, size_t n, const char *n_name, size_t stride, size_t count, int device, const char *made);
int verify_ic_each(const G1Affine *d_ic0, const G1Affine *d_ic, uint32_t nidx, const void *d_x, size_t n, G1Affine *d_out, hipStream_t s);
int verify_g2_replicate(const G2Affine *d_key2, size_t n, G2Affine *d_Q, hipStream_t s);
size_t verify_final_exp_ws_bytes(size_t n);
int verify_final_exp_check(const void *d_M, size_t n, uint32_t pairs, void *d_ws, const void *d_ab, uint8_t *d_verdict, void *d_gt, hipStream_t s);
void final_exp_device_code_on_host(const uint8_t in[384], uint8_t out[384]);
enum { FQ12_MUL = 0, FQ12_SQR, FQ12_LINE, FQ12_CSQR, FQ12_INV, FQ12_CONJ, FQ12_FROB1, FQ12_FROB2, FQ12_FROB3, FQ12_MUL_BY_V, FQ12_OPS };
int verify_fq12_op(int op, const void *d_a, const void *d_b, size_t n, void *d_out, hipStream_t s);
void fq12_op_device_code_on_host(int op, const uint32_t a[96], const uint32_t b[96], uint32_t out[96]);
struct VerifyWorkspace { DevBuf buf; hipStream_t s = nullptr, s2 = nullptr; hipEvent_t ev = nullptr, ev2 = nullptr; };
VerifyWorkspace *verify_workspace_acquire();
void verify_workspace_release(VerifyWorkspace *w);
void verify_workspace_destroy(VerifyWorkspace *w);
void verify_release_all();

struct ZwPlan { uint32_t k = 0, per = 0, n = 0, cap = 0; };
uint32_t zklaim_payload_vars_host();
bool zklaim_witness_plan(uint32_t k, ZwPlan &pl);
bool zklaim_witness_plan_for_n(size_t n, ZwPlan &pl);
size_t zklaim_witness_input_bytes(const ZwPlan &pl, uint32_t P);
void zklaim_witness_pack(const ZwPlan &pl, const struct ::zklaim_ctx *const *ctxs, uint32_t P, uint8_t *host_in, uint8_t *ok);
extern thread_local size_t t_zklaim_witness_stats[2];
extern thread_local size_t t_prove_zklaim_stats[2];
int zklaim_witness_launch(const ZwPlan &pl, uint32_t P, uint8_t *d_in, uint32_t *d_desc, Fr *d_vals, uint32_t *d_idx, uint8_t *d_tags, size_t tag_stride, hipStream_t s);
bool zklaim_witness_par_ready(const ZwPlan &pl);
size_t zklaim_witness_par_input_bytes(const ZwPlan &pl, uint32_t P);
void zklaim_witness_par_pack(const ZwPlan &pl, const struct ::zklaim_ctx *const *ctxs, uint32_t P, uint8_t *host_in, uint8_t *ok);
int zklaim_witness_par_launch(const ZwPlan &pl, uint32_t P, uint8_t *d_in, uint32_t *d_desc, Fr *d_vals, uint32_t *d_idx, uint8_t *d_tags, size_t tag_stride, hipStream_t s);
void zklaim_witness_release_all();

void store_norm(uint64_t *out, const G1 &p);
void store_norm(uint64_t *out, const G2 &p);
G1 load_norm_g1(const uint64_t *in);
G2 load_norm_g2(const uint64_t *in);

}
```

### zklaim_amd/csrc/host/horner_jac.hpp

```cpp
#pragma once
#include "../curve.hip.hpp"
#include <cstring>

namespace zk {

static inline Fq fq_sqr_host(const Fq &a) {
    typedef unsigned __int128 u128;
    constexpr uint64_t P4[4] = {Fq::p64(0), Fq::p64(1), Fq::p64(2), Fq::p64(3)};
    uint64_t A[4], r[8];
    memcpy(A, a.v, 32);
    u128 x = (u128)A[0] * A[1];                r[1] = (uint64_t)x; uint64_t c = (uint64_t)(x >> 64);
    x = (u128)A[0] * A[2] + c;                 r[2] = (uint64_t)x; c = (uint64_t)(x >> 64);
    x = (u128)A[0] * A[3] + c;                 r[3] = (uint64_t)x; r[4] = (uint64_t)(x >> 64);
    x = (u128)A[1] * A[2] + r[3];              r[3] = (uint64_t)x; c = (uint64_t)(x >> 64);
    x = (u128)A[1] * A[3] + r[4] + c;          r[4] = (uint64_t)x; r[5] = (uint64_t)(x >> 64);
    x = (u128)A[2] * A[3] + r[5];              r[5] = (uint64_t)x; r[6] = (uint64_t)(x >> 64);
    r[7] = r[6] >> 63;
    for (int j = 6; j >= 2; --j) r[j] = (r[j] << 1) | (r[j - 1] >> 63);
    r[1] <<= 1;
    x = (u128)A[0] * A[0];                     r[0] = (uint64_t)x; c = (uint64_t)(x >> 64);
    x = (u128)r[1] + c;                        r[1] = (uint64_t)x; c = (uint64_t)(x >> 64);
    x = (u128)A[1] * A[1] + r[2] + c;          r[2] = (uint64_t)x; c = (uint64_t)(x >> 64);
    x = (u128)r[3] + c;                        r[3] = (uint64_t)x; c = (uint64_t)(x >> 64);
    x = (u128)A[2] * A[2] + r[4] + c;          r[4] = (uint64_t)x; c = (uint64_t)(x >> 64);
    x = (u128)r[5] + c;                        r[5] = (uint64_t)x; c = (uint64_t)(x >> 64);
    x = (u128)A[3] * A[3] + r[6] + c;          r[6] = (uint64_t)x; c = (uint64_t)(x >> 64);
    r[7] += c;
    uint64_t top = 0;
    for (int i = 0; i < 4; ++i) {
        const uint64_t m = r[i] * FqParams::INV64;
        c = 0;
        for (int j = 0; j < 4; ++j) { x = (u128)m * P4[j] + r[i + j] + c; r[i + j] = (uint64_t)x; c = (uint64_t)(x >> 64); }
        x = (u128)r[i + 4] + c + top; r[i + 4] = (uint64_t)x; top = (uint64_t)(x >> 64);
    }
    uint64_t s[4]; unsigned long long br = 0;
    for (int j = 0; j < 4; ++j) s[j] = __builtin_subcll(r[4 + j], P4[j], br, &br);
    const uint64_t keep = 0ull - (uint64_t)br;
    for (int j = 0; j < 4; ++j) s[j] ^= (s[j] ^ r[4 + j]) & keep;
    Fq out; memcpy(out.v, s, 32);
    return out;
}

template <class F> static inline XYZZ<F> xyzz_times_pow2(const XYZZ<F> &p, uint32_t n) {
    if (p.is_inf() || n == 0) return p;
    if constexpr (std::is_same<F, Fq>::value) {
        if (n >= 3) {
            Fq X = p.x * p.zz, Y = p.y * p.zzz, Z = p.zz;
            for (uint32_t i = 0; i < n; ++i) {
                const Fq A = fq_sqr_host(X), B = fq_sqr_host(Y), C = fq_sqr_host(B);
                const Fq D = (fq_sqr_host(X + B) - A - C).dbl(), E = A.dbl() + A, E2 = fq_sqr_host(E);
                Z = (Y * Z).dbl();
                X = E2 - D.dbl();
                Y = E * (D - X) - C.dbl().dbl().dbl();
            }
            if (Z.is_zero()) return XYZZ<Fq>::inf();
            const Fq zz = fq_sqr_host(Z);
            return {X, Y, zz, zz * Z};
        }
    }
    XYZZ<F> r = p;
    for (uint32_t i = 0; i < n; ++i) r = r.dbl();
    return r;
}

}
```

### zklaim_amd/csrc/msm.hip

```cpp
#include "common.hpp"
#include "fq29.hip.hpp"
#include "host/horner_jac.hpp"
#include "../../include/zkg.h"
#include <algorithm>
#include <chrono>
#include <cstdio>
#include <cstdlib>
#include <cstring>
#include <mutex>

#define ZK_VGPR_CAP(n) __attribute__((amdgpu_num_vgpr((n) / 2)))
static constexpr int ACC29_VGPRS = 192;

namespace zk {

static constexpr int SCALAR_BITS = 255;
template <class F> struct RedGeom { static constexpr int LANES_LOG = sizeof(F) == sizeof(Fq) ? 7 : 6, LANES = 1 << LANES_LOG, THREADS = 4 * LANES; };
static constexpr int RED_L_LOG_TINY = 0, RED_L_LOG_SMALL = 2, RED_L_LOG_LARGE = 4;
static constexpr size_t RED_SMALL_BUCKETS = (size_t)1 << 16, RED_LARGE_BUCKETS = (size_t)1 << 18;
static constexpr int MAX_C = 16;
static constexpr uint32_t HEAVY_S = 512;
static constexpr uint32_t HEAVY_T_MAX = 1024;
static constexpr uint32_t CLASS_HIST_COPIES = 8;
static constexpr int HEAVY_PART_BLOCKS = 512, HEAVY_MERGE_BLOCKS = 128;
static constexpr int SORT_THREADS = 1024;
static constexpr int SCAN_ITEMS = 4;

struct MsmGeom { uint32_t c, W, B, Wt, w0, ws; };
struct SetLayout { size_t buckets, items, heavy, partials, folded, red_out; };
template <class F> struct BaseView {
    const Affine<F> *p; size_t level_stride; const uint32_t *gather; uint32_t index_sub, B; const uint32_t *remap;
    template <bool PLAIN = false> ZK_D Affine<F> load(uint32_t e, size_t gb) const {
        if constexpr (PLAIN) return p[e >> 1];
        uint32_t i = e >> 1;
        if (gather) i = gather[i];
        if (remap) i = remap[i];
        if (i < index_sub) return Affine<F>::inf();
        return p[(level_stride ? (gb / B) * level_stride : 0) + (i - index_sub)];
    }
};
template <class F> struct ViewSet { BaseView<F> v[MSM_MAX_SETS]; };
struct HeavyItem { uint32_t start, end, gb, single; };
struct HeavyBucket { uint32_t gb, first_item, nparts; };

static MsmGeom pick_geom(size_t n, int window_hint, uint32_t w0 = 0, uint32_t ws = 1) {
    int lg = 0; while (((size_t)1 << (lg + 1)) <= n) ++lg;
    int c = lg >= 15 ? 16 : lg >= 11 ? 12 : lg + 1;
    if (c < 4) c = 4;
    if (window_hint > 0) c = window_hint;
    static const char *force = getenv("ZKG_MSM_C");
    if (force && atoi(force) >= 2) c = atoi(force);
    if (c > MAX_C) c = MAX_C;
    MsmGeom g; g.c = c; g.Wt = (SCALAR_BITS + c - 1) / c; g.B = 1u << (c - 1);
    g.w0 = w0; g.ws = ws ? ws : 1; g.W = w0 < g.Wt ? (g.Wt - w0 + g.ws - 1) / g.ws : 0;
    return g;
}

ZK_D uint32_t bits_at(const uint32_t v[8], uint32_t off, uint32_t c) {
    uint32_t limb = off >> 5, sh = off & 31;
    if (limb >= 8) return 0;
    uint64_t x = v[limb];
    if (limb + 1 < 8) x |= (uint64_t)v[limb + 1] << 32;
    return (uint32_t)(x >> sh) & ((1u << c) - 1);
}

ZK_D void sort_wave_priority() { __builtin_amdgcn_s_setprio(3); }


struct ZeroList { uint32_t *p[4]; uint32_t words[4]; };
__global__ __launch_bounds__(256) void k_digits(const uint32_t *scalars, const uint32_t *gather, size_t n, int mont, MsmGeom g, uint32_t *digits, ZeroList zl) {
    sort_wave_priority();
    size_t i = (size_t)blockIdx.x * blockDim.x + threadIdx.x;
    const size_t lanes = (size_t)gridDim.x * blockDim.x;
#pragma unroll
    for (int k = 0; k < 4; ++k) for (size_t z = i; z < zl.words[k]; z += lanes) zl.p[k][z] = 0;
    if (i >= n) return;
    Fr f;
    const uint4 *p = reinterpret_cast<const uint4 *>(scalars + 8 * (gather ? (size_t)gather[i] : i));
    uint4 a = p[0], b = p[1];
    f.v[0] = a.x; f.v[1] = a.y; f.v[2] = a.z; f.v[3] = a.w; f.v[4] = b.x; f.v[5] = b.y; f.v[6] = b.z; f.v[7] = b.w;
    if (mont) f = f.from_mont();
    uint32_t carry = 0;
    for (uint32_t w = 0, own = g.w0, slot = 0; w < g.Wt; ++w) {
        uint32_t raw = bits_at(f.v, w * g.c, g.c) + carry, code = 0;
        if (raw > g.B) { uint32_t d = (1u << g.c) - raw; carry = 1; if (d) code = (d << 1) | 1u; }
        else { carry = 0; if (raw) code = raw << 1; }
        if (w == own) { digits[(size_t)slot * n + i] = code; ++slot; own += g.ws; }
    }
}

template <int C>
__global__ __launch_bounds__(256) void k_digits_c(const uint32_t *scalars, const uint32_t *gather, size_t n, int mont, MsmGeom g, uint32_t *digits, ZeroList zl) {
    sort_wave_priority();
    size_t i = (size_t)blockIdx.x * blockDim.x + threadIdx.x;
    const size_t lanes = (size_t)gridDim.x * blockDim.x;
#pragma unroll
    for (int k = 0; k < 4; ++k) for (size_t z = i; z < zl.words[k]; z += lanes) zl.p[k][z] = 0;
    if (i >= n) return;
    Fr f;
    const uint4 *p = reinterpret_cast<const uint4 *>(scalars + 8 * (gather ? (size_t)gather[i] : i));
    uint4 a = p[0], b = p[1];
    f.v[0] = a.x; f.v[1] = a.y; f.v[2] = a.z; f.v[3] = a.w; f.v[4] = b.x; f.v[5] = b.y; f.v[6] = b.z; f.v[7] = b.w;
    if (mont) f = f.from_mont();
    constexpr int WT = (SCALAR_BITS + C - 1) / C;
    constexpr uint32_t B = 1u << (C - 1), MASK = (1u << C) - 1;
    uint32_t carry = 0, own = g.w0, slot = 0;
#pragma unroll
    for (int w = 0; w < WT; ++w) {
        const int off = w * C, limb = off >> 5, sh = off & 31;
        uint32_t v = limb < 8 ? f.v[limb < 8 ? limb : 7] >> sh : 0u;
        if (sh + C > 32 && limb + 1 < 8) v |= f.v[limb + 1 < 8 ? limb + 1 : 7] << (32 - sh);
        const uint32_t raw = (v & MASK) + carry;
        const bool neg = raw > B;
        const uint32_t d = neg ? (1u << C) - raw : raw;
        carry = neg ? 1u : 0u;
        const uint32_t code = d ? (d << 1) | (neg ? 1u : 0u) : 0u;
        if ((uint32_t)w == own) { digits[(size_t)slot * n + i] = code; ++slot; own += g.ws; }
    }
}

template <int C>
__global__ __launch_bounds__(256) void k_digits_multi(const uint32_t *scalars, size_t scalar_stride , size_t n, int mont, uint32_t merge, uint32_t *digits, ZeroList zl) {
    sort_wave_priority();
    size_t i = (size_t)blockIdx.x * blockDim.x + threadIdx.x;
    const size_t lanes = (size_t)gridDim.x * blockDim.x;
    if (blockIdx.y == 0) {
#pragma unroll
        for (int k = 0; k < 4; ++k) for (size_t z = i; z < zl.words[k]; z += lanes) zl.p[k][z] = 0;
    }
    if (i >= n) return;
    const uint32_t p = blockIdx.y, P = gridDim.y;
    Fr f;
    const uint4 *src = reinterpret_cast<const uint4 *>(scalars + (size_t)p * scalar_stride + 8 * i);
    uint4 a = src[0], b = src[1];
    f.v[0] = a.x; f.v[1] = a.y; f.v[2] = a.z; f.v[3] = a.w; f.v[4] = b.x; f.v[5] = b.y; f.v[6] = b.z; f.v[7] = b.w;
    if (mont) f = f.from_mont();
    constexpr int WT = (SCALAR_BITS + C - 1) / C;
    constexpr uint32_t B = 1u << (C - 1), MASK = (1u << C) - 1;
    uint32_t carry = 0;
#pragma unroll
    for (int w = 0; w < WT; ++w) {
        const int off = w * C, limb = off >> 5, sh = off & 31;
        uint32_t v = limb < 8 ? f.v[limb < 8 ? limb : 7] >> sh : 0u;
        if (sh + C > 32 && limb + 1 < 8) v |= f.v[limb + 1 < 8 ? limb + 1 : 7] << (32 - sh);
        const uint32_t raw = (v & MASK) + carry;
        const bool neg = raw > B;
        const uint32_t d = neg ? (1u << C) - raw : raw;
        carry = neg ? 1u : 0u;
        const uint32_t code = d ? (d << 1) | (neg ? 1u : 0u) : 0u;
        const size_t row = ((size_t)((uint32_t)w / merge) * P + p) * merge + (uint32_t)w % merge;
        digits[row * n + i] = code;
    }
}

__global__ __launch_bounds__(256) void k_digits_multi_any(const uint32_t *scalars, size_t scalar_stride, size_t n, int mont, MsmGeom g, uint32_t merge, uint32_t *digits, ZeroList zl) {
    sort_wave_priority();
    size_t i = (size_t)blockIdx.x * blockDim.x + threadIdx.x;
    const size_t lanes = (size_t)gridDim.x * blockDim.x;
    if (blockIdx.y == 0) {
#pragma unroll
        for (int k = 0; k < 4; ++k) for (size_t z = i; z < zl.words[k]; z += lanes) zl.p[k][z] = 0;
    }
    if (i >= n) return;
    const uint32_t p = blockIdx.y, P = gridDim.y;
    Fr f;
    const uint4 *src = reinterpret_cast<const uint4 *>(scalars + (size_t)p * scalar_stride + 8 * i);
    uint4 a = src[0], b = src[1];
    f.v[0] = a.x; f.v[1] = a.y; f.v[2] = a.z; f.v[3] = a.w; f.v[4] = b.x; f.v[5] = b.y; f.v[6] = b.z; f.v[7] = b.w;
    if (mont) f = f.from_mont();
    uint32_t carry = 0;
    for (uint32_t w = 0; w < g.Wt; ++w) {
        uint32_t raw = bits_at(f.v, w * g.c, g.c) + carry, code = 0;
        if (raw > g.B) { uint32_t d = (1u << g.c) - raw; carry = 1; if (d) code = (d << 1) | 1u; }
        else { carry = 0; if (raw) code = raw << 1; }
        const size_t row = ((size_t)(w / merge) * P + p) * merge + w % merge;
        digits[row * n + i] = code;
    }
}

template <int C>
__global__ __launch_bounds__(256) void k_digits_c4(const uint32_t *scalars, size_t n, int mont, MsmGeom g, uint32_t *digits, ZeroList zl) {
    sort_wave_priority();
    size_t i = (size_t)blockIdx.x * blockDim.x + threadIdx.x;
    const size_t lanes = (size_t)gridDim.x * blockDim.x;
#pragma unroll
    for (int k = 0; k < 4; ++k) for (size_t z = i; z < zl.words[k]; z += lanes) zl.p[k][z] = 0;
    if (4 * i >= n) return;
    Fr f[4];
#pragma unroll
    for (int q = 0; q < 4; ++q) {
        const uint4 *p = reinterpret_cast<const uint4 *>(scalars + 8 * (4 * i + q));
        const uint4 a = p[0], b = p[1];
        f[q].v[0] = a.x; f[q].v[1] = a.y; f[q].v[2] = a.z; f[q].v[3] = a.w; f[q].v[4] = b.x; f[q].v[5] = b.y; f[q].v[6] = b.z; f[q].v[7] = b.w;
        if (mont) f[q] = f[q].from_mont();
    }
    constexpr int WT = (SCALAR_BITS + C - 1) / C;
    constexpr uint32_t B = 1u << (C - 1), MASK = (1u << C) - 1;
    uint32_t carry[4] = {0, 0, 0, 0};
#pragma unroll
    for (int w = 0; w < WT; ++w) {
        const int off = w * C, limb = off >> 5, sh = off & 31;
        uint32_t code[4];
#pragma unroll
        for (int q = 0; q < 4; ++q) {
            uint32_t v = limb < 8 ? f[q].v[limb < 8 ? limb : 7] >> sh : 0u;
            if (sh + C > 32 && limb + 1 < 8) v |= f[q].v[limb + 1 < 8 ? limb + 1 : 7] << (32 - sh);
            const uint32_t raw = (v & MASK) + carry[q];
            const bool neg = raw > B;
            const uint32_t d = neg ? (1u << C) - raw : raw;
            carry[q] = neg ? 1u : 0u;
            code[q] = d ? (d << 1) | (neg ? 1u : 0u) : 0u;
        }
        *reinterpret_cast<uint4 *>(digits + (size_t)w * n + 4 * i) = make_uint4(code[0], code[1], code[2], code[3]);
    }
}

__global__ __launch_bounds__(SORT_THREADS) void k_hist(const uint32_t *digits, size_t n, uint32_t B, uint32_t S, uint32_t slice_len, uint32_t *hist) {
    extern __shared__ uint32_t lds_u32[];
    const uint32_t s = blockIdx.x, w = blockIdx.y, t = threadIdx.x;
    for (uint32_t b = t; b < B; b += SORT_THREADS) lds_u32[b] = 0;
    __syncthreads();
    size_t lo = (size_t)s * slice_len, hi = lo + slice_len < n ? lo + slice_len : n;
    const uint32_t *d = digits + (size_t)w * n;
    for (size_t i = lo + t; i < hi; i += SORT_THREADS) { uint32_t code = d[i]; if (code) atomicAdd(&lds_u32[(code >> 1) - 1], 1u); }
    __syncthreads();
    uint32_t *out = hist + ((size_t)w * S + s) * B;
    for (uint32_t b = t; b < B; b += SORT_THREADS) out[b] = lds_u32[b];
}

__global__ __launch_bounds__(256) void k_colscan(uint32_t *hist, uint32_t B, uint32_t S, size_t total, uint32_t *counts) {
    size_t gb = (size_t)blockIdx.x * blockDim.x + threadIdx.x;
    if (gb >= total) return;
    uint32_t w = (uint32_t)(gb / B), b = (uint32_t)(gb % B), run = 0;
    uint32_t *col = hist + (size_t)w * S * B + b;
    for (uint32_t s = 0; s < S; ++s) { uint32_t v = col[(size_t)s * B]; col[(size_t)s * B] = run; run += v; }
    counts[gb] = run;
}

__global__ __launch_bounds__(1024) void k_scan_blocks(const uint32_t *in, uint32_t *out, uint32_t *sums, size_t total) {
    __shared__ uint32_t part[1024];
    const uint32_t t = threadIdx.x;
    size_t base = ((size_t)blockIdx.x * 1024 + t) * SCAN_ITEMS;
    uint32_t v[SCAN_ITEMS], s = 0;
    for (int j = 0; j < SCAN_ITEMS; ++j) { v[j] = base + j < total ? in[base + j] : 0; s += v[j]; }
    part[t] = s;
    __syncthreads();
    for (uint32_t d = 1; d < 1024; d <<= 1) {
        uint32_t x = (t >= d) ? part[t - d] : 0;
        __syncthreads();
        part[t] += x;
        __syncthreads();
    }
    uint32_t run = part[t] - s;
    for (int j = 0; j < SCAN_ITEMS; ++j) { if (base + j < total) out[base + j] = run; run += v[j]; }
    if (t == 1023) sums[blockIdx.x] = part[1023];
}
__global__ __launch_bounds__(1024) void k_scan_sums(uint32_t *sums, uint32_t nblk, uint32_t *grand_total) {
    __shared__ uint32_t part[1024];
    const uint32_t t = threadIdx.x;
    uint32_t s = t < nblk ? sums[t] : 0;
    part[t] = s;
    __syncthreads();
    for (uint32_t d = 1; d < 1024; d <<= 1) {
        uint32_t x = (t >= d) ? part[t - d] : 0;
        __syncthreads();
        part[t] += x;
        __syncthreads();
    }
    if (t < nblk) sums[t] = part[t] - s;
    if (t == 1023) *grand_total = part[1023];
}
__global__ __launch_bounds__(1024) void k_scan_apply(uint32_t *out, const uint32_t *sums, size_t total) {
    size_t base = ((size_t)blockIdx.x * 1024 + threadIdx.x) * SCAN_ITEMS;
    uint32_t add = sums[blockIdx.x];
    for (int j = 0; j < SCAN_ITEMS; ++j) if (base + j < total) out[base + j] += add;
}

__global__ __launch_bounds__(SORT_THREADS) void k_place(const uint32_t *digits, size_t n, uint32_t B, uint32_t S, uint32_t slice_len,
                                                         const uint32_t *hist, const uint32_t *offsets, uint32_t *sorted) {
    extern __shared__ uint32_t lds_u32[];
    const uint32_t s = blockIdx.x, w = blockIdx.y, t = threadIdx.x;
    const uint32_t *rel = hist + ((size_t)w * S + s) * B, *off = offsets + (size_t)w * B;
    for (uint32_t b = t; b < B; b += SORT_THREADS) lds_u32[b] = off[b] + rel[b];
    __syncthreads();
    size_t lo = (size_t)s * slice_len, hi = lo + slice_len < n ? lo + slice_len : n;
    const uint32_t *d = digits + (size_t)w * n;
    for (size_t i = lo + t; i < hi; i += SORT_THREADS) {
        uint32_t code = d[i];
        if (code) { uint32_t pos = atomicAdd(&lds_u32[(code >> 1) - 1], 1u); sorted[pos] = ((uint32_t)i << 1) | (code & 1u); }
    }
}


static constexpr uint32_t RX_MAX_CBITS = 10, RX_MAX_CB = 1u << RX_MAX_CBITS, RX_SLICE = 16384, RX_PER_THREAD = 16, RX_FINE_MAX = 8192, RX_BIN_AVG = 4096;
ZK_D uint32_t heavy_threshold_dev(const uint32_t *offsets, size_t total_buckets, uint32_t divisor) {
    uint32_t entries = offsets[total_buckets];
    uint32_t avg6 = (uint32_t)(6 * (uint64_t)entries / total_buckets), slack = 8 + avg6 > 32 ? 32 : 8 + avg6;
    uint32_t t = (uint32_t)(4 * (uint64_t)entries / total_buckets) + slack;
    t = t > HEAVY_T_MAX ? HEAVY_T_MAX : t;
    t /= divisor;
    return t < 4 ? 4 : t;
}
ZK_D uint32_t wave_sum(uint32_t v) {
#pragma unroll
    for (int d = 32; d >= 1; d >>= 1) v += __shfl_xor(v, d, 64);
    return v;
}
__global__ __launch_bounds__(1024) void k_rx_count(const uint32_t *digits, size_t n, uint32_t fbits, uint32_t cbits, uint32_t *cnt, uint32_t *wtot) {
    sort_wave_priority();
    __shared__ uint32_t c[RX_MAX_CB];
    __shared__ uint32_t tot;
    const uint32_t sl = blockIdx.x, w = blockIdx.y, t = threadIdx.x, CB = 1u << cbits;
    if (t < CB) c[t] = 0;
    if (t == 0) tot = 0;
    __syncthreads();
    size_t lo = (size_t)sl * RX_SLICE, hi = lo + RX_SLICE < n ? lo + RX_SLICE : n;
    const uint32_t *d = digits + (size_t)w * n;
    if ((n & 3) == 0) {
        for (size_t i = lo + 4 * t; i < hi; i += 4096) {
            const uint4 q = *reinterpret_cast<const uint4 *>(d + i);
            if (q.x) atomicAdd(&c[((q.x >> 1) - 1) >> fbits], 1u);
            if (q.y) atomicAdd(&c[((q.y >> 1) - 1) >> fbits], 1u);
            if (q.z) atomicAdd(&c[((q.z >> 1) - 1) >> fbits], 1u);
            if (q.w) atomicAdd(&c[((q.w >> 1) - 1) >> fbits], 1u);
        }
    } else
    for (size_t i = lo + t; i < hi; i += 1024) { uint32_t code = d[i]; if (code) atomicAdd(&c[((code >> 1) - 1) >> fbits], 1u); }
    __syncthreads();
    if (t < CB) {
        const uint32_t mine = c[t];
        if (mine) atomicAdd(&cnt[w * CB + t], mine);
        const uint32_t in_wave = wave_sum(mine);
        if ((t & 63) == 0 && in_wave) atomicAdd(&tot, in_wave);
    }
    __syncthreads();
    if (t == 0 && tot) atomicAdd(&wtot[w], tot);
}
ZK_D uint32_t rx_entries_before(const uint32_t *cnt, const uint32_t *wtot, uint32_t w, uint32_t cb, uint32_t cbits) {
    uint32_t v = 0;
    for (uint32_t i = threadIdx.x; i < w; i += blockDim.x) v += wtot[i];
    for (uint32_t b = threadIdx.x; b < cb; b += blockDim.x) v += cnt[(w << cbits) + b];
    return v;
}
template <int T>
__global__ __launch_bounds__(T) void k_rx_scatter(const uint32_t *digits, size_t n, uint32_t fbits, uint32_t cbits, const uint32_t *cnt, const uint32_t *wtot, uint32_t W,
                                                   uint32_t *cursor, uint32_t *tmp, uint32_t *grand_total) {
    sort_wave_priority();
    extern __shared__ uint32_t lds_u32[];
    constexpr uint32_t SLICE = RX_PER_THREAD * T;
    const uint32_t CB = 1u << cbits;
    uint32_t *stage = lds_u32, *c = lds_u32 + SLICE, *off = c + RX_MAX_CB, *gb = off + RX_MAX_CB + 1, *cur = gb + RX_MAX_CB, *wsum = cur + RX_MAX_CB;
    const uint32_t sl = blockIdx.x, w = blockIdx.y, t = threadIdx.x;
    for (uint32_t b = t; b < CB; b += T) c[b] = 0;
    if (t < 2) wsum[t] = 0;
    __syncthreads();
    const uint32_t b0 = t, b1 = t + T;
    const uint32_t g0 = b0 < CB ? cnt[w * CB + b0] : 0, g1 = b1 < CB ? cnt[w * CB + b1] : 0;
    {
        const uint32_t below = wave_sum(rx_entries_before(cnt, wtot, w, 0, cbits));
        if ((t & 63) == 0 && below) atomicAdd(&wsum[0], below);
        if (sl == 0 && w == 0) {
            uint32_t all = 0;
            for (uint32_t i = t; i < W; i += T) all += wtot[i];
            all = wave_sum(all);
// ... 666 lines not shown
    }
    if (t < FB && b < B) out[b] = sh[t].normalized();
}

template <class F> ZK_D F inverse_fast(const F &x) {
    if constexpr (std::is_same<F, Fq>::value) return f29::from29(f29::inverse(f29::to29(x.normalized())));
    else { const Fq d = inverse_fast<Fq>(x.c0.sqr() + x.c1.sqr()); return F{x.c0 * d, (x.c1 * d).neg()}; }
}
template <class F, int K>
__global__ __launch_bounds__(256) void k_table_levels(const Affine<F> *in, Affine<F> *out, size_t n, uint32_t c, int levels) {
    size_t i = (size_t)blockIdx.x * blockDim.x + threadIdx.x;
    if (i >= n) return;
    Affine<F> a = in[i];
    if (a.is_inf()) { for (int l = 0; l < levels; ++l) out[(size_t)l * n + i] = a; return; }
    F x[K], y[K], zz[K], zzz[K];
    XYZZ<F> p = XYZZ<F>::dbl_affine_inl(a);
#pragma unroll
    for (int l = 0; l < K; ++l) {
        if (l < levels) {
            for (uint32_t k = (l == 0 ? 1u : 0u); k < c; ++k) p = p.dbl();
            x[l] = p.x; y[l] = p.y; zz[l] = p.zz; zzz[l] = p.zzz;
        } else { x[l] = F::zero(); y[l] = F::zero(); zz[l] = F::zero(); zzz[l] = F::zero(); }
    }
    F pre[K], run = F::one();
#pragma unroll
    for (int l = 0; l < K; ++l) { pre[l] = run; if (!zzz[l].is_zero()) run = run * zzz[l]; }
    F inv = inverse_fast(run);
#pragma unroll
    for (int l = K - 1; l >= 0; --l) {
        if (l >= levels) continue;
        if (zzz[l].is_zero()) { out[(size_t)l * n + i] = Affine<F>::inf(); continue; }
        F zi = inv * pre[l];
        inv = inv * zzz[l];
        F t = zi * zz[l];
        F zi2 = t.sqr();
        out[(size_t)l * n + i] = Affine<F>{x[l] * zi2, y[l] * zi}.normalized();
    }
}

__global__ __launch_bounds__(256) void k_classify(const Fr *z, size_t n1, uint8_t *tags, uint32_t *listed, uint32_t *count, const uint32_t *subset_pos) {
    size_t i = (size_t)blockIdx.x * blockDim.x + threadIdx.x;
    uint32_t tag = 0;
    if (i < n1) {
        Fr v = z[i];
        uint32_t any = 0, diff = 0;
#pragma unroll
        for (int j = 0; j < 8; ++j) { any |= v.v[j]; diff |= v.v[j] ^ FrParams::ONE[j]; }
        tag = any == 0 ? 0u : (diff == 0 ? 1u : 2u);
        tags[i] = (uint8_t)tag;
    }
    const unsigned long long mask = __ballot(tag == 2);
    if (!mask) return;
    const uint32_t lane = threadIdx.x & 63;
    uint32_t base = 0;
    if (lane == (uint32_t)(__ffsll((long long)mask) - 1)) base = atomicAdd(count, (uint32_t)__popcll(mask));
    base = __shfl(base, __ffsll((long long)mask) - 1, 64);
    if (tag == 2) {
        listed[base + (uint32_t)__popcll(mask & ((1ull << lane) - 1))] = (uint32_t)i;
        if (subset_pos && subset_pos[i] == SUBSET_NONE) count[1] = 1;
    }
}
template <class F>
__global__ __launch_bounds__(256) void k_gather_points(const Affine<F> *src, const uint32_t *idx, size_t count, uint32_t index_sub, Affine<F> *out) {
    size_t j = (size_t)blockIdx.x * blockDim.x + threadIdx.x;
    if (j >= count) return;
    const uint32_t i = idx[j];
    out[j] = i >= index_sub ? src[i - index_sub] : Affine<F>::inf();
}
template <class F>
__global__ __launch_bounds__(256) void k_scatter_points(const Affine<F> *src, const uint32_t *idx, size_t count, Affine<F> *out) {
    size_t j = (size_t)blockIdx.x * blockDim.x + threadIdx.x;
    if (j < count) out[idx[j]] = src[j];
}
template <class F>
__global__ __launch_bounds__(256) void k_ones_sum(const ViewSet<F> views, const uint8_t *tags, size_t n1, uint32_t span, XYZZ<F> *partials,
                                                   size_t tag_stride, size_t vec_stride ) {
    extern __shared__ unsigned char red_smem[];
    LdsPoint<F> *sh = reinterpret_cast<LdsPoint<F> *>(red_smem);
    uint32_t *list = reinterpret_cast<uint32_t *>(red_smem + 256 * sizeof(LdsPoint<F>));
    __shared__ uint32_t seg_count[4];
    const Affine<F> *bases = views.v[blockIdx.y].p; const uint32_t index_sub = views.v[blockIdx.y].index_sub;
    tags += (size_t)blockIdx.z * tag_stride;
    partials += (size_t)blockIdx.z * vec_stride + (size_t)blockIdx.y * (gridDim.x + 1);
    const uint32_t tid = threadIdx.x, lane = tid & 63, wv = tid >> 6, cap = span >> 2;
    const size_t first = (size_t)blockIdx.x * span + (size_t)wv * cap;
    uint32_t count = 0;
    for (uint32_t o = 0; o < cap; o += 64) {
        const size_t i = first + o + lane;
        const bool one = i < n1 && i >= index_sub && tags[i] == 1;
        const unsigned long long mask = __ballot(one);
        if (one) list[wv * cap + count + (uint32_t)__popcll(mask & ((1ull << lane) - 1))] = (uint32_t)(i - index_sub);
        count += (uint32_t)__popcll(mask);
    }
    if (lane == 0) seg_count[wv] = count;
    __syncthreads();
    const uint32_t c0 = seg_count[0], c1 = c0 + seg_count[1], c2 = c1 + seg_count[2], total = c2 + seg_count[3];
    XYZZ<F> acc = XYZZ<F>::inf();
    for (uint32_t k = tid; k < total; k += 256) {
        const uint32_t seg = (k >= c0) + (k >= c1) + (k >= c2), off = seg == 0 ? 0u : (seg == 1 ? c0 : (seg == 2 ? c1 : c2));
        acc.madd(bases[list[seg * cap + (k - off)]]);
    }
    sh[tid] = acc;
    __syncthreads();
    lds_tree_reduce<F>(sh, 256, tid, 256, [] { __syncthreads(); });
    if (tid == 0) partials[blockIdx.x] = sh[0].normalized();
}
template <class F>
__global__ __launch_bounds__(256) void k_sum_partials(XYZZ<F> *partials_all, uint32_t count, size_t vec_stride) {
    extern __shared__ unsigned char red_smem[];
    LdsPoint<F> *sh = reinterpret_cast<LdsPoint<F> *>(red_smem);
    XYZZ<F> *partials = partials_all + (size_t)blockIdx.y * vec_stride + (size_t)blockIdx.x * (count + 1), *out = partials + count;
    XYZZ<F> acc = XYZZ<F>::inf();
    for (uint32_t i = threadIdx.x; i < count; i += 256) acc.add(partials[i]);
    sh[threadIdx.x] = acc;
    __syncthreads();
    lds_tree_reduce<F>(sh, 256, threadIdx.x, 256, [] { __syncthreads(); });
    if (threadIdx.x == 0) out[0] = sh[0].normalized();
}

struct MsmGroup {
    DevBuf buckets, folded, red_out, heavy_items, heavy_buckets, heavy_partials;
    DevBuf bases29;
    void *host_red = nullptr; size_t host_cap = 0; bool g2 = false, table = false; int nsets = 0;
    int out_index[MSM_MAX_SETS] = {0};
    int red_slots = 2; size_t red_stride = 0;
    uint32_t cpw = 0, red_windows = 0; size_t nred = 0; int chunk_log = 0;
    int host_reserve(size_t bytes) {
        if (bytes <= host_cap) return 0;
        if (host_red) (void)hipHostFree(host_red);
        host_red = nullptr; host_cap = 0;
        if (!hip_ok(hipHostMalloc(&host_red, bytes + 4096, hipHostMallocDefault), "hipHostMalloc", __FILE__, __LINE__)) return 1;
        host_cap = bytes + 4096;
        return 0;
    }
    void release() {
        for (DevBuf *b : {&buckets, &folded, &red_out, &heavy_items, &heavy_buckets, &heavy_partials, &bases29}) b->release();
        if (host_red) (void)hipHostFree(host_red);
        host_red = nullptr; host_cap = 0;
    }
};
struct MsmSortSpace {
    DevBuf digits, hist, counts, offsets, scan_sums, class_hist, order, sorted, rx_tmp, rx_meta, heavy_counters[2];
    void release() { for (DevBuf *b : {&digits, &hist, &counts, &offsets, &scan_sums, &class_hist, &order, &sorted, &rx_tmp, &rx_meta, &heavy_counters[0], &heavy_counters[1]}) b->release(); }
};
struct MsmLaunchMode {
    hipStream_t sort_stream = nullptr;
    uint32_t *heavy_out = nullptr;
    int window = 0;
    bool resume = false;
    bool defer_reduce = false;
    bool heavy_pair = true;
    bool beside = false;
    bool timed = false;
    uint32_t *stream_waits = nullptr;
};
struct MsmJob {
    hipStream_t stream = nullptr; bool own_stream = false;
    MsmSortSpace space;
    MsmGroup group[2];
    MsmGeom g{}; size_t n = 0;
    int window_hint = 0;
    uint32_t merge_hint = 1, merge = 1;
    hipStream_t aux = nullptr; hipEvent_t ev_fork = nullptr, ev_join = nullptr; bool converted_aside = false;
    bool one_pass_sort = false;
    bool critical = false;
    uint32_t w0 = 0, ws = 1;
    bool empty = false;
    bool dev_finish = false;
    uint32_t multi = 1; size_t multi_stride = 0;
    std::mutex mu;
    int ensure_side() {
        if (aux) return ZKG_OK;
        if (hipStreamCreateWithFlags(&aux, hipStreamNonBlocking) == hipSuccess && hipEventCreateWithFlags(&ev_fork, hipEventDisableTiming) == hipSuccess &&
            hipEventCreateWithFlags(&ev_join, hipEventDisableTiming) == hipSuccess) return ZKG_OK;
        release_side(); set_error("msm: side stream"); return ZKG_ERROR;
    }
    void release_side() {
        if (aux) { (void)hipStreamSynchronize(aux); (void)hipStreamDestroy(aux); }
        if (ev_fork) (void)hipEventDestroy(ev_fork);
        if (ev_join) (void)hipEventDestroy(ev_join);
        aux = nullptr; ev_fork = ev_join = nullptr;
    }
    void release_device() {
        space.release();
        for (MsmGroup &gr : group) gr.release();
        release_side();
    }
};
struct MsmLaunchSets { MsmBases by_field[2][MSM_MAX_SETS]; MsmGeom g{}; size_t n = 0; bool empty = false; MsmSortSpace *space = nullptr; };

template <class F>
static int launch_accumulate(MsmJob *job, MsmGroup &gr, const MsmLaunchSets &ls, const uint32_t *d_gather, const MsmLaunchMode &mode, bool time_it) {
    const MsmSortSpace &sp = *ls.space; const MsmBases *sets = ls.by_field[gr.g2 ? 1 : 0];
    const MsmGeom g = ls.g; const size_t n = ls.n, total_buckets = (size_t)g.W * g.B; const unsigned ns = (unsigned)gr.nsets;
    const uint32_t P = job->multi, BP = g.B * P, Wp = g.W / P;
    hipStream_t s = job->stream;
    size_t n_entries_max = n * g.W;
    const size_t max_heavy = std::min(total_buckets, n_entries_max / (sizeof(F) != sizeof(Fq) ? 4 : 8)) + 1,
                 max_items = max_heavy + n_entries_max / HEAVY_S + 1;
    typedef RedGeom<F> RG;
    gr.table = sets[0].level_stride != 0;
    gr.red_windows = gr.table ? P : g.W;
    const size_t red_buckets = (size_t)gr.red_windows * g.B;
    static const char *force_l = getenv("ZKG_RED_L_LOG");
    const int red_l_log = force_l ? atoi(force_l) : red_buckets >= RED_LARGE_BUCKETS ? RED_L_LOG_LARGE : red_buckets > RED_SMALL_BUCKETS ? RED_L_LOG_SMALL : RED_L_LOG_TINY;
    gr.chunk_log = RG::LANES_LOG + red_l_log;
    gr.cpw = (g.B + (1u << gr.chunk_log) - 1) >> gr.chunk_log; gr.nred = (size_t)gr.red_windows * gr.cpw;
    gr.red_slots = 2;
    SetLayout L; L.buckets = total_buckets; L.items = max_items; L.heavy = max_heavy; L.partials = max_items; L.folded = BP; L.red_out = gr.nred * 3;
    if (gr.heavy_items.reserve(ns * max_items * sizeof(HeavyItem)) || gr.heavy_buckets.reserve(ns * max_heavy * sizeof(HeavyBucket)) ||
        gr.heavy_partials.reserve(ns * max_items * sizeof(XYZZ<F>)) ||
        gr.buckets.reserve(ns * total_buckets * std::max(sizeof(XYZZ<F>), sizeof(Bucket29))) || (job->dev_finish && gr.red_out.reserve(ns * L.red_out * sizeof(XYZZ<F>))) || ((gr.red_stride = L.red_out), false) ||
        (gr.table && gr.folded.reserve(ns * (size_t)BP * std::max(sizeof(XYZZ<F>), sizeof(Bucket29)))) || (!job->dev_finish && gr.host_reserve(ns * L.red_out * sizeof(XYZZ<F>)))) return ZKG_ERROR;
    XYZZ<F> *buckets = gr.buckets.as<XYZZ<F>>();
    uint32_t *heavy_counters = sp.heavy_counters[gr.g2 ? 1 : 0].as<uint32_t>();
    ViewSet<F> views;
    for (unsigned i = 0; i < (unsigned)MSM_MAX_SETS; ++i) {
        const MsmBases &b = sets[i < ns ? i : 0];
        views.v[i] = BaseView<F>{reinterpret_cast<const Affine<F> *>(b.p), b.level_stride, d_gather, b.index_sub, BP, b.remap};
    }
    const size_t lanes = gr.table ? std::min(total_buckets, n_entries_max) : total_buckets;
    bool plain = !d_gather;
    for (unsigned i = 0; i < ns; ++i) plain = plain && sets[i].level_stride == 0 && sets[i].index_sub == 0 && !sets[i].remap;
    bool use29 = false; const Rec64 *rec29 = nullptr; size_t stride29 = 0;
    if constexpr (sizeof(F) == sizeof(Fq)) {
        if (ns == 1 && plain) {
            use29 = true;
            if (sets[0].p29) rec29 = reinterpret_cast<const Rec64 *>(sets[0].p29);
            else {
                ZK_HIP(hipStreamWaitEvent(s, job->ev_join, 0));
                if (mode.stream_waits) ++*mode.stream_waits;
                rec29 = gr.bases29.as<Rec64>();
            }
        } else if (ns == 1 && !d_gather && sets[0].p29 && !sets[0].remap && sets[0].index_sub == 0) {
            use29 = true; rec29 = reinterpret_cast<const Rec64 *>(sets[0].p29); stride29 = sets[0].level_stride;
        }
    }
    const bool out29 = use29 && (stride29 == 0 ? !gr.table : (gr.table && ns == 1 && Wp <= 8));
    const int resume = mode.resume ? 1 : 0;
    if (time_it) g_dominant_timer.begin(s);
    if constexpr (sizeof(F) == sizeof(Fq)) {
        static const int waves_env = getenv("ZKG_ACC29_WAVES") ? atoi(getenv("ZKG_ACC29_WAVES")) : 0;
        const int waves29 = waves_env ? waves_env : (mode.beside || gr.table) ? 2 : 3;
        auto launch29 = [&](auto kern) {
            hipLaunchKernelGGL(kern, dim3((unsigned)((lanes + 255) / 256)), dim3(256), 0, s, rec29, stride29, BP, sp.sorted.as<uint32_t>(),
                               sp.offsets.as<uint32_t>(), sp.order.as<uint32_t>(), lanes, (void *)buckets, gr.heavy_items.as<HeavyItem>(),
                               gr.heavy_buckets.as<HeavyBucket>(), heavy_counters, L, resume | (job->critical ? 2 : 0));
        };
        if (use29 && waves29 == 3) { if (out29) launch29(k_bucket_accum29<3, true>); else launch29(k_bucket_accum29<3, false>); }
        else if (use29) { if (out29) launch29(k_bucket_accum29<2, true>); else launch29(k_bucket_accum29<2, false>); }
    }
    auto launch32 = [&](auto kern) {
        hipLaunchKernelGGL(kern, dim3((unsigned)((lanes + 255) / 256), ns), dim3(256), 0, s, views, sp.sorted.as<uint32_t>(), sp.offsets.as<uint32_t>(), sp.order.as<uint32_t>(),
                           lanes, buckets, gr.heavy_items.as<HeavyItem>(), gr.heavy_buckets.as<HeavyBucket>(), heavy_counters, L);
    };
    if (!use29) { if (plain) launch32(k_bucket_accum<F, true>); else launch32(k_bucket_accum<F, false>); }
    if (time_it) g_dominant_timer.end(s);
    if (mode.heavy_pair) {
    hipLaunchKernelGGL(k_heavy_parts<F>, dim3(HEAVY_PART_BLOCKS, ns), dim3(256), 256 * sizeof(LdsPoint<F>), s,
                       views, sp.sorted.as<uint32_t>(), gr.heavy_items.as<HeavyItem>(), heavy_counters, gr.heavy_partials.as<XYZZ<F>>(), buckets, L, (int)out29);
    hipLaunchKernelGGL(k_heavy_merge<F>, dim3(HEAVY_MERGE_BLOCKS, ns), dim3(256), 256 * sizeof(LdsPoint<F>), s,
                       gr.heavy_buckets.as<HeavyBucket>(), heavy_counters, gr.heavy_partials.as<XYZZ<F>>(), buckets, L, (int)out29, resume);
    }
    if (mode.defer_reduce) {
        if (hipGetLastError() != hipSuccess) { set_error("msm kernel launch failed"); return ZKG_ERROR; }
        return ZKG_OK;
    }
    const XYZZ<F> *red_in = buckets; size_t in_stride = L.buckets;
    XYZZ<F> *red_dst = job->dev_finish ? gr.red_out.as<XYZZ<F>>() : reinterpret_cast<XYZZ<F> *>(gr.host_red);
    bool folded29 = false;
    if constexpr (sizeof(F) == sizeof(Fq)) {
        if (gr.table && out29) {
            hipLaunchKernelGGL(k_bucket_fold29, dim3((2 * BP + 255) / 256), dim3(256), 0, s, reinterpret_cast<const Bucket29 *>(buckets), sp.counts.as<uint32_t>(), Wp, BP,
                               gr.folded.as<Bucket29>(), job->critical ? 1 : 0);
            red_in = gr.folded.as<XYZZ<F>>(); in_stride = L.folded; folded29 = true;
        }
    }
    if (gr.table && !folded29) {
        uint32_t slots = 1; while (slots < Wp && slots < 32) slots <<= 1;
        uint32_t fold_b_log = 0; while ((FOLD_THREADS >> (fold_b_log + 1)) >= slots) ++fold_b_log;
        hipLaunchKernelGGL(k_bucket_fold<F>, dim3((BP + (1u << fold_b_log) - 1) >> fold_b_log, ns), dim3(FOLD_THREADS), FOLD_THREADS * sizeof(LdsPoint<F>), s,
                           buckets, sp.counts.as<uint32_t>(), Wp, BP, fold_b_log, gr.folded.as<XYZZ<F>>(), L);
        red_in = gr.folded.as<XYZZ<F>>(); in_stride = L.folded;
    }
    if constexpr (sizeof(F) == sizeof(Fq)) {
        const size_t lds = 2 * RG::LANES * sizeof(LdsPoint29);
        const void *rin = red_in; XYZZ<Fq> *rout = reinterpret_cast<XYZZ<Fq> *>(red_dst);
        auto launch_red = [&](auto kern, unsigned threads) { hipLaunchKernelGGL(kern, dim3((unsigned)gr.nred, ns), dim3(threads), lds, s, rin, g.B, gr.cpw, rout, in_stride, L.red_out, job->critical ? 1 : 0); };
        if (out29 && red_l_log == RED_L_LOG_LARGE) {
            gr.red_slots = 3;
            hipLaunchKernelGGL(k_bucket_reduce29l, dim3((unsigned)gr.nred, ns), dim3(2 * RG::LANES), 4 * RG::LANES * sizeof(LdsPoint29), s,
                               reinterpret_cast<const Bucket29 *>(rin), g.B, gr.cpw, rout, in_stride, L.red_out, job->critical ? 1 : 0);
        } else if (red_l_log != RED_L_LOG_TINY) {
            if (red_l_log == RED_L_LOG_LARGE) launch_red(k_bucket_reduce29p<RED_L_LOG_LARGE, false>, 2 * RG::LANES);
            else if (out29) launch_red(k_bucket_reduce29p<RED_L_LOG_SMALL, true>, 2 * RG::LANES);
            else launch_red(k_bucket_reduce29p<RED_L_LOG_SMALL, false>, 2 * RG::LANES);
        } else {
            if (out29) launch_red(k_bucket_reduce29<RED_L_LOG_TINY, true>, RG::THREADS);
            else launch_red(k_bucket_reduce29<RED_L_LOG_TINY, false>, RG::THREADS);
        }
    } else {
        auto launch_red = [&](auto kern) { hipLaunchKernelGGL(kern, dim3((unsigned)gr.nred, ns), dim3(RG::THREADS), 2 * RG::LANES * sizeof(LdsPoint<F>), s, red_in, g.B, gr.cpw, red_dst, in_stride, L.red_out); };
        if (red_l_log == RED_L_LOG_LARGE) launch_red(k_bucket_reduce<F, RED_L_LOG_LARGE>);
        else if (red_l_log == RED_L_LOG_SMALL) launch_red(k_bucket_reduce<F, RED_L_LOG_SMALL>);
        else launch_red(k_bucket_reduce<F, RED_L_LOG_TINY>);
    }
    if (hipGetLastError() != hipSuccess) { set_error("msm kernel launch failed"); return ZKG_ERROR; }
    return ZKG_OK;
}

template <class F>
static XYZZ<F> host_combine(const MsmJob *job, const MsmGroup &gr, int set, int vec = 0 ) {
    const MsmGeom g = job->g; const uint32_t cpw = gr.cpw, W = gr.red_windows;
    const bool multi = gr.table && job->multi > 1;
    const XYZZ<F> *red = reinterpret_cast<const XYZZ<F> *>(gr.host_red) + (size_t)set * gr.red_stride;
    const size_t sl = (size_t)gr.red_slots;
    std::vector<XYZZ<F>> V(W);
    auto window = [&](int w) {
        XYZZ<F> Usum = XYZZ<F>::inf(), suffix = XYZZ<F>::inf(), weighted = XYZZ<F>::inf(), Asum = XYZZ<F>::inf();
        for (int ch = (int)cpw - 1; ch >= 0; --ch) {
            const XYZZ<F> &P = red[sl * ((size_t)w * cpw + ch)], &U = red[sl * ((size_t)w * cpw + ch) + 1];
            Usum.add(U);
            if (sl == 3) Asum.add(red[sl * ((size_t)w * cpw + ch) + 2]);
            if (ch >= 1) { suffix.add(P); weighted.add(suffix); }
            else suffix.add(P);
        }
        if (sl == 3 && !Asum.is_inf()) Usum.add(xyzz_times_pow2(Asum, 3));
        weighted = xyzz_times_pow2(weighted, (uint32_t)gr.chunk_log);
        Usum.add(weighted); Usum.add(suffix);
        V[w] = Usum;
    };
    if (multi) { window(vec); return V[vec]; }
    if (gr.table) {
        const int SEG = 16, nseg = ((int)cpw + SEG - 1) / SEG;
        if (nseg <= 1) { window(0); return V[0]; }
        std::vector<XYZZ<F>> Us(nseg), Ps(nseg), Wt(nseg);
        host_parallel_for(nseg, [&](int sg) {
            XYZZ<F> Usum = XYZZ<F>::inf(), suffix = XYZZ<F>::inf(), weighted = XYZZ<F>::inf();
            const int lo = sg * SEG, hi = std::min<int>((int)cpw, lo + SEG);
            for (int ch = hi - 1; ch >= lo; --ch) {
                Usum.add(red[2 * (size_t)ch + 1]);
                suffix.add(red[2 * (size_t)ch]);
                if (ch > lo) weighted.add(suffix);
            }
            Us[sg] = Usum; Ps[sg] = suffix; Wt[sg] = weighted;
        });
        XYZZ<F> Usum = XYZZ<F>::inf(), suffix = XYZZ<F>::inf(), seg_weighted = XYZZ<F>::inf(), weighted = XYZZ<F>::inf();
        for (int sg = nseg - 1; sg >= 0; --sg) { Usum.add(Us[sg]); weighted.add(Wt[sg]); suffix.add(Ps[sg]); if (sg >= 1) seg_weighted.add(suffix); }
        weighted.add(xyzz_times_pow2(seg_weighted, 4));
        weighted = xyzz_times_pow2(weighted, (uint32_t)gr.chunk_log);
        Usum.add(weighted); Usum.add(suffix);
        return Usum;
    }
    host_parallel_for((int)W, window);
    XYZZ<F> acc = XYZZ<F>::inf();
    for (int w = (int)W - 1; w >= 0; --w) {
        acc = xyzz_times_pow2(acc, g.c * g.ws);
        acc.add(V[w]);
    }
    return xyzz_times_pow2(acc, g.c * g.w0);
}

template <class F> constexpr int COMBINE_THREADS = 256;
template <> constexpr int COMBINE_THREADS<Fq2> = 128;
template <class F> constexpr int COMBINE_MAX_SLOTS = 3;
template <> constexpr int COMBINE_MAX_SLOTS<Fq2> = 2;
template <class F> constexpr int POINT_WORDS = 3 * sizeof(F) / 4;
template <class F> static __host__ __device__ uint32_t combine_lanes(uint32_t cpw) { uint32_t n = 1; while (n < cpw && n < (uint32_t)COMBINE_THREADS<F>) n <<= 1; return n; }
template <class F> static size_t combine_lds_bytes(uint32_t cpw) { return combine_lanes<F>(cpw) * sizeof(LdsPoint<F>); }
ZK_D void store_limbs(uint32_t *out, const Fq &a) { for (int i = 0; i < 8; ++i) out[i] = a.v[i]; }
ZK_D void store_limbs(uint32_t *out, const Fq2 &a) { store_limbs(out, a.c0); store_limbs(out + 8, a.c1); }
ZK_D void load_limbs(Fq &a, const uint32_t *in) { for (int i = 0; i < 8; ++i) a.v[i] = in[i]; }
ZK_D void load_limbs(Fq2 &a, const uint32_t *in) { load_limbs(a.c0, in); load_limbs(a.c1, in + 8); }
template <class F> ZK_D void store_norm_dev(uint32_t *out , const XYZZ<F> &v) {
    F X = F::zero(), Y = F::one(), Z = F::zero();
    if (!v.is_inf()) { const Affine<F> a = v.to_affine().normalized(); X = a.x; Y = a.y; Z = F::one(); }
    store_limbs(out, X); store_limbs(out + sizeof(F) / 4, Y); store_limbs(out + 2 * (sizeof(F) / 4), Z);
}
template <class F, int THREADS>
__global__ __launch_bounds__(THREADS) void k_msm_combine(const XYZZ<F> *red, uint32_t cpw, int slots, int chunk_log, size_t set_stride, uint32_t *out) {
    extern __shared__ unsigned char red_smem[];
    LdsPoint<F> *sh = reinterpret_cast<LdsPoint<F> *>(red_smem);
    const uint32_t t = threadIdx.x, w = blockIdx.x, set = blockIdx.y;
    const uint32_t n = combine_lanes<F>(cpw);
    int l_log = 0; while (((uint64_t)n << l_log) < cpw) ++l_log;
    const XYZZ<F> *rec = red + (size_t)set * set_stride + (size_t)slots * w * cpw;
    const uint64_t first = (uint64_t)t << l_log, end = first + ((uint64_t)1 << l_log) < cpw ? first + ((uint64_t)1 << l_log) : cpw;
    XYZZ<F> U = XYZZ<F>::inf(), Q = XYZZ<F>::inf(), T0 = XYZZ<F>::inf();
    {
        const bool has_a = COMBINE_MAX_SLOTS<F> == 3 && slots == 3;
        XYZZ<F> A = XYZZ<F>::inf();
        for (uint64_t ch = end; ch > first; --ch) {
            const XYZZ<F> *r = rec + (size_t)slots * (ch - 1);
            Q.add(r[0]); U.add(r[1]);
            if (has_a) A.add(r[2]);
            if (ch - 1 > first) T0.add(Q);
        }
        if (has_a) { for (int i = 0; i < 3; ++i) A = A.dbl(); U.add(A); }
    }
    for (uint32_t d = 1; d < n; d <<= 1) {
        if (t < n) sh[t] = Q;
        __syncthreads();
        if (t + d < n) Q.add(sh[t + d]);
        __syncthreads();
    }
    if (t == 0) { U.add(Q); Q = XYZZ<F>::inf(); }
    for (int i = 0; i < l_log; ++i) Q = Q.dbl();
    Q.add(T0);
    for (int i = 0; i < chunk_log; ++i) Q = Q.dbl();
    U.add(Q);
    if (t < n) sh[t] = U;
    __syncthreads();
    lds_tree_reduce<F>(sh, n, t, THREADS, [] { __syncthreads(); });
    if (t == 0) store_norm_dev<F>(out + POINT_WORDS<F> * ((size_t)w * gridDim.y + set), sh[0]);
}
template <class F> static void launch_combine(dim3 grid, hipStream_t s, const XYZZ<F> *red, uint32_t cpw, int slots, int chunk_log, size_t set_stride, uint32_t *out) {
    hipLaunchKernelGGL((k_msm_combine<F, COMBINE_THREADS<F>>), grid, dim3(COMBINE_THREADS<F>), combine_lds_bytes<F>(cpw), s, red, cpw, slots, chunk_log, set_stride, out);
}
template <class F> __global__ __launch_bounds__(64) void k_msm_store_inf(uint32_t *out, uint32_t count) {
    const uint32_t i = blockIdx.x * blockDim.x + threadIdx.x;
    if (i < count) store_norm_dev(out + POINT_WORDS<F> * (size_t)i, XYZZ<F>::inf());
}
template <class F> __global__ __launch_bounds__(256) void k_jac_to_records(const uint32_t *jac, size_t count, XYZZ<F> *rec) {
    const size_t i = (size_t)blockIdx.x * blockDim.x + threadIdx.x;
    if (i >= count) return;
    const uint32_t *in = jac + POINT_WORDS<F> * i;
    F X, Y, Z;
    load_limbs(X, in); load_limbs(Y, in + sizeof(F) / 4); load_limbs(Z, in + 2 * (sizeof(F) / 4));
    rec[i] = Z.is_zero() ? XYZZ<F>::inf() : XYZZ<F>{X, Y, F::one(), F::one()};
}

static int sort_digits(MsmJob *job, MsmLaunchSets &ls, const uint32_t *d_scalars, bool mont, const uint32_t *d_gather, const MsmLaunchMode &mode) {
    MsmSortSpace &sp = *ls.space;
    const MsmGeom g0 = job->g; const size_t n0 = job->n;
    if (job->merge > 1) { job->g.W /= job->merge; job->g.Wt = job->g.W; job->n *= job->merge; }
    if (job->multi > 1) { job->g.W *= job->multi; job->g.Wt = job->g.W; }
    const MsmGeom g = ls.g = job->g; const size_t n = ls.n = job->n;
    hipStream_t s = mode.sort_stream ? mode.sort_stream : job->stream;
    const size_t total = (size_t)g.W * g.B;
    uint32_t slice_len = (uint32_t)std::min<size_t>(65536, std::max<size_t>(4096, ((n + 15) / 16 + 1023) / 1024 * 1024));
    uint32_t S = (uint32_t)std::max<size_t>(1, (n + slice_len - 1) / slice_len);
    size_t nblk = (total + 1024 * SCAN_ITEMS - 1) / (1024 * SCAN_ITEMS);
    if (nblk > 1024) { set_error("msm: too many buckets for the block scan"); return ZKG_ERROR; }
    if (sp.digits.reserve(std::max<size_t>(1, n * g.W) * 4) || sp.hist.reserve((size_t)g.W * S * g.B * 4) || sp.counts.reserve(total * 4) ||
        sp.offsets.reserve((total + 1) * 4) || sp.scan_sums.reserve(1024 * 4) || sp.class_hist.reserve((CLASS_HIST_COPIES + 1) * (HEAVY_T_MAX + 2) * 4) ||
        sp.order.reserve(total * 4) || sp.sorted.reserve(std::max<size_t>(1, n * g.W) * 4)) return ZKG_ERROR;
    uint32_t *digits = sp.digits.as<uint32_t>(), *hist = sp.hist.as<uint32_t>(), *counts = sp.counts.as<uint32_t>(),
             *offsets = sp.offsets.as<uint32_t>(), *sums = sp.scan_sums.as<uint32_t>(), *chist = sp.class_hist.as<uint32_t>();
    uint32_t cbits = 6;
    static const uint32_t bin_avg = getenv("ZKG_RX_AVG") ? (uint32_t)atoi(getenv("ZKG_RX_AVG")) : RX_BIN_AVG;
    while (cbits < RX_MAX_CBITS && cbits + 1 < g.c - 1 && (n >> cbits) > bin_avg) ++cbits;
    const bool two_pass = !job->one_pass_sort && g.c >= 12 && n >= 49152 && (n >> cbits) <= RX_FINE_MAX && n <= ((size_t)1 << (31 - (g.c - 1 - cbits)));
    {
        ZeroList zl{};
        int k = 0;
        zl.p[k] = chist; zl.words[k++] = (CLASS_HIST_COPIES + 1) * (HEAVY_T_MAX + 2);
        for (int f = 0; f < 2; ++f) if (job->group[f].nsets) {
            if (sp.heavy_counters[f].reserve(8 * MSM_MAX_SETS)) return ZKG_ERROR;
            zl.p[k] = sp.heavy_counters[f].as<uint32_t>(); zl.words[k++] = 2 * MSM_MAX_SETS;
        }
        if (two_pass) {
            const uint32_t nbins = g.W << cbits;
            if (sp.rx_meta.reserve((2 * (size_t)nbins + g.W) * 4)) return ZKG_ERROR;
            zl.p[k] = sp.rx_meta.as<uint32_t>(); zl.words[k++] = 2 * nbins + g.W;
        }
        const dim3 dg((unsigned)((n0 + 255) / 256));
        const bool four = !d_gather && (n0 & 3) == 0 && g0.w0 == 0 && g0.ws == 1 && g0.W == g0.Wt;
        const dim3 dg4((unsigned)((n0 / 4 + 255) / 256));
        if (job->multi > 1) {
            const dim3 dgm(dg.x, job->multi);
            if (g0.c == 16) hipLaunchKernelGGL(k_digits_multi<16>, dgm, dim3(256), 0, s, d_scalars, job->multi_stride, n0, (int)mont, job->merge, digits, zl);
            else if (g0.c == 12) hipLaunchKernelGGL(k_digits_multi<12>, dgm, dim3(256), 0, s, d_scalars, job->multi_stride, n0, (int)mont, job->merge, digits, zl);
            else hipLaunchKernelGGL(k_digits_multi_any, dgm, dim3(256), 0, s, d_scalars, job->multi_stride, n0, (int)mont, g0, job->merge, digits, zl);
        }
        else if (four && g0.c == 16) hipLaunchKernelGGL(k_digits_c4<16>, dg4, dim3(256), 0, s, d_scalars, n0, (int)mont, g0, digits, zl);
        else if (four && g0.c == 12) hipLaunchKernelGGL(k_digits_c4<12>, dg4, dim3(256), 0, s, d_scalars, n0, (int)mont, g0, digits, zl);
        else if (g0.c == 16) hipLaunchKernelGGL(k_digits_c<16>, dg, dim3(256), 0, s, d_scalars, d_gather, n0, (int)mont, g0, digits, zl);
        else if (g0.c == 12) hipLaunchKernelGGL(k_digits_c<12>, dg, dim3(256), 0, s, d_scalars, d_gather, n0, (int)mont, g0, digits, zl);
        else hipLaunchKernelGGL(k_digits, dg, dim3(256), 0, s, d_scalars, d_gather, n0, (int)mont, g0, digits, zl);
    }
    if (two_pass) {
        const uint32_t fbits = g.c - 1 - cbits, CB = 1u << cbits, nbins = g.W * CB, S1 = (uint32_t)((n + RX_SLICE - 1) / RX_SLICE);
        if (sp.rx_tmp.reserve(n * g.W * 4)) return ZKG_ERROR;
        uint32_t *cnt = sp.rx_meta.as<uint32_t>(), *cursor = cnt + nbins, *wtot = cursor + nbins, *tmp = sp.rx_tmp.as<uint32_t>();
        const size_t fine_lds = (RX_FINE_MAX + 3 * (1u << fbits)) * 4;
        hipLaunchKernelGGL(k_rx_count, dim3(S1, g.W), dim3(1024), 0, s, digits, n, fbits, cbits, cnt, wtot);
        static const int wg_env = getenv("ZKG_SORT_WG") ? atoi(getenv("ZKG_SORT_WG")) : 0;
        const bool half = (wg_env ? wg_env == 512 : mode.sort_stream != nullptr) && fbits <= 9;
        if (half) {
            const uint32_t S2 = (uint32_t)((n + 512 * RX_PER_THREAD - 1) / (512 * RX_PER_THREAD));
            hipLaunchKernelGGL(k_rx_scatter<512>, dim3(S2, g.W), dim3(512), (512 * RX_PER_THREAD + 4 * RX_MAX_CB + 8) * 4, s, digits, n, fbits, cbits, cnt, wtot, g.W, cursor, tmp, offsets + total);
            hipLaunchKernelGGL(k_rx_fine<512>, dim3(CB, g.W), dim3(512), fine_lds, s, tmp, fbits, cbits, g.B, cnt, wtot, counts, offsets, total, chist,
                               sp.sorted.as<uint32_t>());
        } else {
            hipLaunchKernelGGL(k_rx_scatter<1024>, dim3(S1, g.W), dim3(1024), (RX_SLICE + 4 * RX_MAX_CB + 8) * 4, s, digits, n, fbits, cbits, cnt, wtot, g.W, cursor, tmp, offsets + total);
            hipLaunchKernelGGL(k_rx_fine<1024>, dim3(CB, g.W), dim3(1024), fine_lds, s, tmp, fbits, cbits, g.B, cnt, wtot, counts, offsets, total, chist,
                               sp.sorted.as<uint32_t>());
        }
    } else {
    hipLaunchKernelGGL(k_hist, dim3(S, g.W), dim3(SORT_THREADS), g.B * 4, s, digits, n, g.B, S, slice_len, hist);
    hipLaunchKernelGGL(k_colscan, dim3((unsigned)((total + 255) / 256)), dim3(256), 0, s, hist, g.B, S, total, counts);
    hipLaunchKernelGGL(k_scan_blocks, dim3((unsigned)nblk), dim3(1024), 0, s, counts, offsets, sums, total);
    hipLaunchKernelGGL(k_scan_sums, dim3(1), dim3(1024), 0, s, sums, (uint32_t)nblk, offsets + total);
    hipLaunchKernelGGL(k_scan_apply, dim3((unsigned)nblk), dim3(1024), 0, s, offsets, sums, total);
    hipLaunchKernelGGL(k_place, dim3(S, g.W), dim3(SORT_THREADS), g.B * 4, s, digits, n, g.B, S, slice_len, hist, offsets, sp.sorted.as<uint32_t>());
    hipLaunchKernelGGL(k_class_hist, dim3((unsigned)((total + 1023) / 1024)), dim3(1024), 0, s, counts, offsets, total, chist);
    }
    hipLaunchKernelGGL(k_order_place, dim3((unsigned)((total + 1023) / 1024)), dim3(1024), 0, s, counts, offsets, total, chist, chist + CLASS_HIST_COPIES * (HEAVY_T_MAX + 2), sp.order.as<uint32_t>(), mode.heavy_out);
    if (hipGetLastError() != hipSuccess) { set_error("msm sort launch failed"); return ZKG_ERROR; }
    return ZKG_OK;
}

MsmJob *msm_job_create(hipStream_t s, bool own_stream, bool high_priority) {
    MsmJob *j = new MsmJob();
    j->stream = s;
    if (own_stream) {
        int prio_lo = 0, prio_hi = 0;
        (void)hipDeviceGetStreamPriorityRange(&prio_lo, &prio_hi);
        if (!hip_ok(hipStreamCreateWithPriority(&j->stream, hipStreamNonBlocking, high_priority ? prio_hi : prio_lo), "hipStreamCreate", __FILE__, __LINE__)) { delete j; return nullptr; }
        j->own_stream = true;
    }
    return j;
}
void msm_job_set_window(MsmJob *j, int c) { if (j) j->window_hint = c; }
bool crit_priority_enabled() { static const bool on = !(getenv("ZKG_CRIT_PRIO") && atoi(getenv("ZKG_CRIT_PRIO")) == 0); return on; }
void msm_job_set_critical(MsmJob *j, bool critical) { if (j) j->critical = critical && crit_priority_enabled(); }
void msm_job_set_row_merge(MsmJob *j, uint32_t f) { if (j) j->merge_hint = f ? f : 1; }
void msm_job_set_skewed(MsmJob *j, bool skewed) { if (j) j->one_pass_sort = skewed; }
void msm_job_set_window_subset(MsmJob *j, uint32_t w0, uint32_t ws) { if (j) { j->w0 = w0; j->ws = ws ? ws : 1; } }
hipStream_t msm_job_stream(MsmJob *j) { return j->stream; }
void msm_job_destroy(MsmJob *j) {
    if (!j) return;
    j->release_device();
    if (j->own_stream) (void)hipStreamDestroy(j->stream);
    delete j;
}

static MsmJob g_default_job;
struct HostScalarsStats { uint32_t pieces = 0, waits = 0, heavy[8] = {0}, pair[8] = {0}; };
struct PieceStep {
    DevBuf scalars; MsmSortSpace space;
    hipStream_t copy = nullptr, sort = nullptr;
    hipEvent_t ev_piece[8] = {nullptr}, ev_sorted[2] = {nullptr}, ev_acc_done[2] = {nullptr}, ev_caller = nullptr;
    uint32_t *heavy_words = nullptr;
    HostScalarsStats stats;
    bool ready = false;
    template <class Fn> void each_event(Fn f) { for (hipEvent_t &e : ev_piece) f(e); for (hipEvent_t &e : ev_sorted) f(e); for (hipEvent_t &e : ev_acc_done) f(e); f(ev_caller); }
    int ensure() {
        if (ready) return ZKG_OK;
        int lo = 0, hi = 0; (void)hipDeviceGetStreamPriorityRange(&lo, &hi);
        bool ok = hipStreamCreateWithFlags(&copy, hipStreamNonBlocking) == hipSuccess && hipStreamCreateWithPriority(&sort, hipStreamNonBlocking, hi) == hipSuccess &&
                  hipHostMalloc(reinterpret_cast<void **>(&heavy_words), 8 * sizeof(uint32_t), hipHostMallocDefault) == hipSuccess;
        each_event([&](hipEvent_t &e) { ok = ok && hipEventCreateWithFlags(&e, hipEventDisableTiming) == hipSuccess; });
        if (!ok) { release(); set_error("msm: streams, events and pinned words of the piece-wise step"); return ZKG_ERROR; }
        ready = true;
        return ZKG_OK;
    }
    void release() {
        for (hipStream_t *s : {&sort, &copy}) if (*s) { (void)hipStreamSynchronize(*s); (void)hipStreamDestroy(*s); *s = nullptr; }
        each_event([](hipEvent_t &e) { if (e) { (void)hipEventDestroy(e); e = nullptr; } });
        if (heavy_words) { (void)hipHostFree(heavy_words); heavy_words = nullptr; }
        scalars.release(); space.release();
        ready = false;
    }
};
static PieceStep g_step;

static int msm_launch_failed(MsmJob *job) {
    if (job->converted_aside) { (void)hipStreamSynchronize(job->aux); job->converted_aside = false; }
    return ZKG_ERROR;
}
static void msm_job_split_sets(MsmJob *job, const MsmBases *sets, int nsets, size_t n, bool gathered, MsmLaunchSets &ls) {
    for (MsmGroup &gr : job->group) gr.nsets = 0;
    job->group[0].g2 = false; job->group[1].g2 = true;
    for (int i = 0; i < nsets; ++i) { MsmGroup &gr = job->group[sets[i].g2 ? 1 : 0]; ls.by_field[sets[i].g2 ? 1 : 0][gr.nsets] = sets[i]; gr.out_index[gr.nsets] = gr.nsets; ++gr.nsets; }
    bool merge = nsets > 0 && n > 0 && job->g.W > 0 && job->merge_hint > 1 && !gathered && job->g.W % job->merge_hint == 0 && (uint64_t)n * job->merge_hint < ((uint64_t)1 << 31);
    for (int i = 0; i < nsets; ++i) merge = merge && sets[i].level_stride == n && sets[i].index_sub == 0 && !sets[i].remap;
    job->merge = merge ? job->merge_hint : 1;
    for (int k = 0; k < 2; ++k) for (int i = 0; i < job->group[k].nsets; ++i) ls.by_field[k][i].level_stride *= job->merge;
}
static int msm_job_convert_aside(MsmJob *job, const void *bases, size_t n) {
    if (job->ensure_side() || job->group[0].bases29.reserve(n * sizeof(Rec64))) return ZKG_ERROR;
    ZK_HIP(hipEventRecord(job->ev_fork, job->stream));
    ZK_HIP(hipStreamWaitEvent(job->aux, job->ev_fork, 0));
    hipLaunchKernelGGL(k_bases_to29, dim3((unsigned)((n + 255) / 256)), dim3(256), 0, job->aux, reinterpret_cast<const Affine<Fq> *>(bases), n, job->group[0].bases29.as<Rec64>());
    ZK_HIP(hipEventRecord(job->ev_join, job->aux));
    return ZKG_OK;
}
static int msm_job_enqueue_sort(MsmJob *job, MsmSortSpace &space, const MsmBases *sets, int nsets, const uint32_t *d_scalars, size_t n, bool scalars_mont, const uint32_t *d_gather,
                                const MsmLaunchMode &mode, MsmLaunchSets &ls) {
    if (n >= ((size_t)1 << 31) || nsets < 0 || nsets > MSM_MAX_SETS) { set_error("msm: bad size"); return ZKG_ERROR; }
    const int window = mode.window > 0 ? mode.window : job->window_hint;
    bool any_table = false;
    for (int i = 0; i < nsets; ++i) any_table = any_table || sets[i].level_stride != 0;
    for (int i = 0; i < nsets; ++i) if ((sets[i].level_stride != 0) != any_table) { set_error("msm: table and plain base sets cannot share a launch"); return ZKG_ERROR; }
    if (any_table && (job->w0 != 0 || job->ws != 1 || window <= 0)) { set_error("msm: a table launch covers all windows at the table's window size"); return ZKG_ERROR; }
    job->g = pick_geom(n, window, job->w0, job->ws); job->n = n;
    job->empty = false; job->multi = 1;
    ls.space = &space; ls.empty = false;
    msm_job_split_sets(job, sets, nsets, n, d_gather != nullptr, ls);
    if (job->g.W == 0 || n == 0) { job->empty = ls.empty = true; return ZKG_OK; }
    if ((uint64_t)n * job->g.W >= ((uint64_t)1 << 32)) { set_error("msm: n * windows exceeds the 32-bit index space of the sorted list (n < 2^28)"); return ZKG_ERROR; }
    job->converted_aside = false;
    const MsmBases &g1 = ls.by_field[0][0];
    if (!any_table && !d_gather && job->group[0].nsets == 1 && g1.index_sub == 0 && !g1.remap && !g1.p29) {
        if (msm_job_convert_aside(job, g1.p, n)) return ZKG_ERROR;
        job->converted_aside = true;
    }
    if (sort_digits(job, ls, d_scalars, scalars_mont, d_gather, mode)) return msm_launch_failed(job);
    return ZKG_OK;
}
static int msm_job_enqueue_accumulate(MsmJob *job, const MsmLaunchSets &ls, const uint32_t *d_gather, const MsmLaunchMode &mode) {
    if (ls.empty) return ZKG_OK;
    const bool timed_field_g2 = job->group[0].nsets == 0;
    if (job->group[1].nsets && launch_accumulate<Fq2>(job, job->group[1], ls, d_gather, mode, mode.timed && timed_field_g2)) return msm_launch_failed(job);
    if (job->group[0].nsets && launch_accumulate<Fq>(job, job->group[0], ls, d_gather, mode, mode.timed)) return msm_launch_failed(job);
    return ZKG_OK;
}
static int msm_job_launch_as(MsmJob *job, const MsmBases *sets, int nsets, const uint32_t *d_scalars, size_t n, bool scalars_mont, const uint32_t *d_gather, const MsmLaunchMode &mode) {
    static const bool dbg = getenv("ZKG_DEBUG_TIMING") != nullptr;
    auto t0 = std::chrono::steady_clock::now();
    auto lap = [&](const char *w) { if (dbg) fprintf(stderr, "[zkg]     %-18s %8.3f ms\n", w, std::chrono::duration<float, std::milli>(std::chrono::steady_clock::now() - t0).count()); };
    MsmLaunchSets ls;
    if (msm_job_enqueue_sort(job, job->space, sets, nsets, d_scalars, n, scalars_mont, d_gather, mode, ls)) return ZKG_ERROR;
    lap("sort enqueued");
    if (msm_job_enqueue_accumulate(job, ls, d_gather, mode)) return ZKG_ERROR;
    lap("accum enqueued");
    return ZKG_OK;
}
int msm_job_launch(MsmJob *job, const MsmBases *sets, int nsets, const uint32_t *d_scalars, size_t n, bool scalars_mont, const uint32_t *d_gather) {
    MsmLaunchMode mode; mode.timed = job == &g_default_job;
    return msm_job_launch_as(job, sets, nsets, d_scalars, n, scalars_mont, d_gather, mode);
}
bool msm_multi_supported(size_t n, int c, uint32_t count) {
    const MsmGeom g = pick_geom(n, c);
    return c > 0 && count >= 1 && n >= 1 && (uint64_t)n * g.W * count < ((uint64_t)1 << 31) &&
           ((uint64_t)g.W * g.B * count + 1024 * SCAN_ITEMS - 1) / (1024 * SCAN_ITEMS) <= 1024;
}
int msm_job_launch_multi(MsmJob *job, const MsmBases *sets, int nsets, const uint32_t *d_scalars, size_t n, size_t scalar_stride, uint32_t count, bool scalars_mont) {
    bool ok = job->w0 == 0 && job->ws == 1 && nsets >= 1 && nsets <= MSM_MAX_SETS && msm_multi_supported(n, job->window_hint, count);
    for (int i = 0; i < nsets && ok; ++i) ok = sets[i].level_stride != 0 && !sets[i].remap && sets[i].index_sub == 0;
    if (!ok) { set_error("msm: unsupported multi launch"); return ZKG_ERROR; }
    job->g = pick_geom(n, job->window_hint); job->n = n;
    job->empty = false; job->converted_aside = false;
    MsmLaunchSets ls; ls.space = &job->space;
    msm_job_split_sets(job, sets, nsets, n, false, ls);
    job->multi = count; job->multi_stride = scalar_stride;
    const MsmLaunchMode mode;
    if (sort_digits(job, ls, d_scalars, scalars_mont, nullptr, mode)) return ZKG_ERROR;
    return msm_job_enqueue_accumulate(job, ls, nullptr, mode);
}
int msm_job_finish_multi(MsmJob *job, G1 *out_g1, G2 *out_g2) {
    ZK_HIP(hipStreamSynchronize(job->stream));
    const int n1 = job->group[0].nsets, n2 = job->group[1].nsets;
    host_parallel_for((int)job->multi, [&](int p) {
        for (int k = 0; k < n1; ++k) out_g1[p * n1 + k] = host_combine<Fq>(job, job->group[0], k, p);
        for (int k = 0; k < n2; ++k) out_g2[p * n2 + k] = host_combine<Fq2>(job, job->group[1], k, p);
    });
    return ZKG_OK;
}
int msm_job_finish(MsmJob *job, G1 *out_g1, G2 *out_g2) {
    static const bool dbg = getenv("ZKG_DEBUG_TIMING") != nullptr;
    const auto t0 = std::chrono::steady_clock::now();
    ZK_HIP(hipStreamSynchronize(job->stream));
    const auto t1 = std::chrono::steady_clock::now();
    struct Lap { bool on; std::chrono::steady_clock::time_point a, b; ~Lap() { if (on) fprintf(stderr, "[zkg]     job finish: waited %.3f ms, host combine %.3f ms\n", std::chrono::duration<float, std::milli>(b - a).count(), std::chrono::duration<float, std::milli>(std::chrono::steady_clock::now() - b).count()); } } lap_{dbg, t0, t1};
    for (int k = 0; k < job->group[0].nsets; ++k) out_g1[k] = job->empty ? G1::inf() : host_combine<Fq>(job, job->group[0], k);
    for (int k = 0; k < job->group[1].nsets; ++k) out_g2[k] = job->empty ? G2::inf() : host_combine<Fq2>(job, job->group[1], k);
    return ZKG_OK;
}

void msm_job_set_device_finish(MsmJob *j, bool on) { if (j) j->dev_finish = on; }
template <class F> static int finish_dev(MsmJob *job, const MsmGroup &gr, uint32_t *out) {
    const uint32_t vectors = job->multi > 1 ? job->multi : 1;
    if (job->empty) {
        const uint32_t count = vectors * (uint32_t)gr.nsets;
        hipLaunchKernelGGL(k_msm_store_inf<F>, dim3((count + 63) / 64), dim3(64), 0, job->stream, out, count);
    } else {
        if (!gr.table || gr.red_windows != vectors || gr.red_slots > COMBINE_MAX_SLOTS<F>) { set_error("msm_job_finish_dev: table sets only (a plain set's windows need the Horner doublings)"); return ZKG_ERROR; }
        launch_combine<F>(dim3(vectors, (unsigned)gr.nsets), job->stream, gr.red_out.as<XYZZ<F>>(), gr.cpw, gr.red_slots, gr.chunk_log, gr.red_stride, out);
    }
    if (hipGetLastError() != hipSuccess) { set_error("msm combine launch failed"); return ZKG_ERROR; }
    return ZKG_OK;
}
int msm_job_finish_dev(MsmJob *job, uint64_t *d_out) {
    const bool g2 = job->group[0].nsets == 0;
    const MsmGroup &gr = job->group[g2 ? 1 : 0];
    if (!job->dev_finish || (job->group[0].nsets && job->group[1].nsets) || gr.nsets < 1) { set_error("msm_job_finish_dev: a device-finish launch of G1 sets only, or of G2 sets only"); return ZKG_ERROR; }
    uint32_t *out = reinterpret_cast<uint32_t *>(d_out);
    return g2 ? finish_dev<Fq2>(job, gr, out) : finish_dev<Fq>(job, gr, out);
}
template <class F> static int combine_records(const uint64_t *records_jac, size_t cpw, int slots, int chunk_log, size_t vectors, uint64_t *out_jac) {
    constexpr size_t point_bytes = POINT_WORDS<F> * 4;
    const size_t count = vectors * cpw * (size_t)slots;
    ScopedDevBuf in, rec, out;
    if (in.reserve(count * point_bytes) || rec.reserve(count * sizeof(XYZZ<F>)) || out.reserve(vectors * point_bytes)) return ZKG_ERROR;
    ZK_HIP(hipMemcpy(in.p, records_jac, count * point_bytes, hipMemcpyHostToDevice));
    hipLaunchKernelGGL(k_jac_to_records<F>, dim3((unsigned)((count + 255) / 256)), dim3(256), 0, nullptr, in.as<uint32_t>(), count, rec.as<XYZZ<F>>());
    launch_combine<F>(dim3((unsigned)vectors, 1), nullptr, rec.as<XYZZ<F>>(), (uint32_t)cpw, slots, chunk_log, (size_t)0, out.as<uint32_t>());
    if (hipGetLastError() != hipSuccess) { set_error("msm combine launch failed"); return ZKG_ERROR; }
    ZK_HIP(hipMemcpy(out_jac, out.p, vectors * point_bytes, hipMemcpyDeviceToHost));
    return ZKG_OK;
}
int msm_combine_records(bool g2, const uint64_t *records_jac, size_t cpw, int slots, int chunk_log, size_t vectors, uint64_t *out_jac) {
    const bool args = records_jac && out_jac && cpw >= 1 && cpw <= ((size_t)1 << 16) && chunk_log >= 0 && chunk_log <= 24 && vectors >= 1 && vectors <= 1024;
    if (g2) {
        if (!args || slots != 2) { set_error("zkg_msm_combine_g2_gpu: bad argument (1 <= cpw <= 2^16, 0 <= chunk_log <= 24, 1 <= vectors <= 1024)"); return ZKG_ERROR; }
        return combine_records<Fq2>(records_jac, cpw, slots, chunk_log, vectors, out_jac);
    }
    if (!args || (slots != 2 && slots != 3)) { set_error("zkg_msm_combine_gpu: bad argument (1 <= cpw <= 2^16, slots 2 or 3, 0 <= chunk_log <= 24, 1 <= vectors <= 1024)"); return ZKG_ERROR; }
    return combine_records<Fq>(records_jac, cpw, slots, chunk_log, vectors, out_jac);
}
size_t msm_table_bucket_bytes(int c, bool g2) {
    const MsmGeom g = pick_geom(1, c);
    return (size_t)g.W * g.B * (g2 ? std::max(sizeof(XYZZ<Fq2>), sizeof(Bucket29)) : std::max(sizeof(XYZZ<Fq>), sizeof(Bucket29)));
}


int msm_shared(const G1Affine *const *d_g1_bases, int n_g1, const G2Affine *d_g2_bases, const uint32_t *d_scalars, size_t n,
               bool scalars_mont, G1 *out_g1, G2 *out_g2, hipStream_t s, uint32_t w0, uint32_t ws, bool mostly_bits) {
    if (n_g1 < 0 || n_g1 + (d_g2_bases ? 1 : 0) > MSM_MAX_SETS) { set_error("msm: too many base sets"); return ZKG_ERROR; }
    std::lock_guard<std::mutex> lk(g_default_job.mu);
    g_dominant_timer.new_call();
    g_default_job.stream = s; g_default_job.w0 = w0; g_default_job.ws = ws ? ws : 1; g_default_job.one_pass_sort = mostly_bits;
    MsmBases sets[MSM_MAX_SETS]; int nsets = 0;
    for (int i = 0; i < n_g1; ++i) { sets[nsets] = MsmBases(); sets[nsets].p = d_g1_bases[i]; ++nsets; }
    if (d_g2_bases) { sets[nsets] = MsmBases(); sets[nsets].p = d_g2_bases; sets[nsets].g2 = true; ++nsets; }
    if (n >= ((size_t)1 << 28)) { set_error("msm: at most 2^28 - 1 points per call"); return ZKG_ERROR; }
    const size_t PIECE = (size_t)1 << 23;
    if (n <= PIECE || w0 != 0 || g_default_job.ws != 1) {
        if (msm_job_launch(&g_default_job, sets, nsets, d_scalars, n, scalars_mont, nullptr)) return ZKG_ERROR;
        return msm_job_finish(&g_default_job, out_g1, out_g2);
    }
    G1 acc1[MSM_MAX_SETS]; G2 acc2[MSM_MAX_SETS];
    for (int i = 0; i < MSM_MAX_SETS; ++i) { acc1[i] = G1::inf(); acc2[i] = G2::inf(); }
    for (size_t lo = 0; lo < n; lo += PIECE) {
        const size_t cnt = std::min(PIECE, n - lo);
        MsmBases piece[MSM_MAX_SETS];
        for (int i = 0; i < nsets; ++i) { piece[i] = sets[i]; piece[i].p = (const char *)sets[i].p + lo * (sets[i].g2 ? sizeof(G2Affine) : sizeof(G1Affine)); }
        G1 p1[MSM_MAX_SETS]; G2 p2[MSM_MAX_SETS];
        if (msm_job_launch(&g_default_job, piece, nsets, d_scalars + 8 * lo, cnt, scalars_mont, nullptr) || msm_job_finish(&g_default_job, p1, p2)) return ZKG_ERROR;
        for (int i = 0; i < n_g1; ++i) acc1[i].add(p1[i]);
        if (d_g2_bases) acc2[0].add(p2[0]);
    }
    for (int i = 0; i < n_g1; ++i) out_g1[i] = acc1[i];
    if (d_g2_bases) out_g2[0] = acc2[0];
    return ZKG_OK;
}

static int host_scalars_cuts(size_t n, int max_pieces, size_t cut[9]) {
    int P = max_pieces;
    cut[P] = n;
    for (int k = P - 1; k >= 1; --k) cut[k] = (cut[k + 1] / 2) & ~(size_t)255;
    cut[0] = 0;
    if (const char *e = getenv("ZKG_MSM_CUTS")) {
        int k = 1; const char *q = e;
        while (*q && k < 8) { const long v = strtol(q, const_cast<char **>(&q), 10); if (v <= 0 || v >= 64) break; cut[k++] = (n * (size_t)v / 64) & ~(size_t)255; if (*q == ',') ++q; }
        if (k > 1) { P = k; cut[P] = n; for (int i = 1; i < P; ++i) if (cut[i] < cut[i - 1]) cut[i] = cut[i - 1]; }
    }
    return P;
}
int msm_g1_host_scalars(const G1Affine *d_bases, const uint32_t *h_scalars, size_t n, bool mont, G1 *out, hipStream_t s) {
    if (n >= ((size_t)1 << 28)) { set_error("msm: at most 2^28 - 1 points per call"); return ZKG_ERROR; }
    if (!n) { *out = G1::inf(); return ZKG_OK; }
    static const int max_pieces = getenv("ZKG_MSM_PIECES") ? std::max(1, std::min(8, atoi(getenv("ZKG_MSM_PIECES")))) : 4;
    const bool pieces = max_pieces > 1 && n >= ((size_t)1 << 19) && n <= ((size_t)1 << 23);
    if (n > ((size_t)1 << 23)) {
        ScopedDevBuf tmp;
        if (tmp.reserve(n * 32)) return ZKG_ERROR;
        ZK_HIP(hipMemcpyAsync(tmp.p, h_scalars, n * 32, hipMemcpyHostToDevice, s));
        return msm_g1(d_bases, tmp.as<uint32_t>(), n, mont, out, s, false);
    }
    MsmJob &J = g_default_job; PieceStep &T = g_step;
    std::lock_guard<std::mutex> lk(J.mu);
    g_dominant_timer.new_call();
    if (T.scalars.reserve(n * 32)) return ZKG_ERROR;
    uint32_t *d_sc = T.scalars.as<uint32_t>();
    J.stream = s; J.w0 = 0; J.ws = 1; J.one_pass_sort = false;
    MsmBases set; set.p = d_bases;
    T.stats = HostScalarsStats();
    MsmLaunchMode mode; mode.timed = true; mode.stream_waits = &T.stats.waits;
    if (!pieces) {
        ZK_HIP(hipMemcpyAsync(d_sc, h_scalars, n * 32, hipMemcpyHostToDevice, s));
        if (msm_job_launch_as(&J, &set, 1, d_sc, n, mont, nullptr, mode)) return ZKG_ERROR;
        T.stats.pieces = 1; T.stats.heavy[0] = 0xffffffffu; T.stats.pair[0] = 1;
        return msm_job_finish(&J, out, nullptr);
    }
    if (T.ensure()) return ZKG_ERROR;
    size_t cut[9]; const int P = host_scalars_cuts(n, max_pieces, cut);
    if (hipStreamQuery(s) != hipSuccess) {
        (void)hipGetLastError();
        ZK_HIP(hipEventRecord(T.ev_caller, s));
        ZK_HIP(hipStreamWaitEvent(T.copy, T.ev_caller, 0));
    }
    for (int k = 0; k < P; ++k) {
        ZK_HIP(hipMemcpyAsync(d_sc + 8 * cut[k], h_scalars + 8 * cut[k], (cut[k + 1] - cut[k]) * 32, hipMemcpyHostToDevice, T.copy));
        ZK_HIP(hipEventRecord(T.ev_piece[k], T.copy));
    }
    if (msm_job_convert_aside(&J, d_bases, n)) return ZKG_ERROR;
    ZK_HIP(hipStreamWaitEvent(T.sort, J.ev_fork, 0));
    mode.sort_stream = T.sort; mode.beside = true;
    mode.window = (int)pick_geom(n, J.window_hint).c;
    int run[8], R = 0;
    for (int k = 0; k < P; ++k) if (cut[k + 1] != cut[k] || k + 1 == P) run[R++] = k;
    MsmLaunchSets ls[2];
    int rc = ZKG_OK; bool used[2] = {false, false};
    auto enqueue_sort = [&](int i) {
        const int k = run[i], which = (R - 1 - i) & 1;
        MsmBases piece = set; piece.p = reinterpret_cast<const char *>(d_bases) + cut[k] * sizeof(G1Affine);
        piece.p29 = J.group[0].bases29.as<Rec64>() + cut[k];
        mode.heavy_out = T.heavy_words + i;
        if (hipStreamWaitEvent(T.sort, T.ev_piece[k], 0) != hipSuccess) return ZKG_ERROR;
        if (used[which] && hipStreamWaitEvent(T.sort, T.ev_acc_done[which], 0) != hipSuccess) return ZKG_ERROR;
        if (msm_job_enqueue_sort(&J, which ? T.space : J.space, &piece, 1, d_sc + 8 * cut[k], cut[k + 1] - cut[k], mont, nullptr, mode, ls[which])) return ZKG_ERROR;
        return !ls[which].empty && hipEventRecord(T.ev_sorted[which], T.sort) != hipSuccess ? ZKG_ERROR : ZKG_OK;
    };
    rc = enqueue_sort(0);
    for (int i = 0; i < R && rc == ZKG_OK; ++i) {
        const int which = (R - 1 - i) & 1;
        if (i + 1 < R && (rc = enqueue_sort(i + 1)) != ZKG_OK) break;
        if (i == 0 && hipEventSynchronize(J.ev_join) != hipSuccess) { rc = ZKG_ERROR; break; }
        uint32_t heavy = 0;
        if (!ls[which].empty) {
            if (hipEventSynchronize(T.ev_sorted[which]) != hipSuccess) { rc = ZKG_ERROR; break; }
            heavy = *static_cast<volatile const uint32_t *>(T.heavy_words + i);
        }
        mode.resume = i > 0; mode.defer_reduce = i + 1 < R; mode.heavy_pair = heavy != 0;
        rc = msm_job_enqueue_accumulate(&J, ls[which], nullptr, mode);
        if (rc == ZKG_OK && hipEventRecord(T.ev_acc_done[which], s) != hipSuccess) rc = ZKG_ERROR;
        used[which] = true;
        T.stats.heavy[i] = heavy; T.stats.pair[i] = heavy != 0; T.stats.pieces = (uint32_t)(i + 1);
    }
    if (rc != ZKG_OK) { (void)hipStreamSynchronize(T.copy); (void)hipStreamSynchronize(J.aux); (void)hipStreamSynchronize(T.sort); (void)hipStreamSynchronize(s); return ZKG_ERROR; }
    return msm_job_finish(&J, out, nullptr);
}
int msm_host_scalars_stats(uint32_t *out, int n) {
    std::lock_guard<std::mutex> lk(g_default_job.mu);
    const HostScalarsStats &st = g_step.stats;
    if (!st.pieces) return 0;
    uint32_t rec[2 + 2 * 8] = {st.pieces, st.waits};
    for (uint32_t k = 0; k < st.pieces; ++k) { rec[2 + 2 * k] = st.heavy[k]; rec[3 + 2 * k] = st.pair[k]; }
    const int words = 2 + 2 * (int)st.pieces;
    for (int i = 0; i < words && i < n; ++i) out[i] = rec[i];
    return words;
}

int msm_g1(const G1Affine *d_bases, const uint32_t *d_scalars, size_t n, bool mont, G1 *out, hipStream_t s, bool mostly_bits) {
    return msm_shared(&d_bases, 1, nullptr, d_scalars, n, mont, out, nullptr, s, 0, 1, mostly_bits);
}
int msm_g2(const G2Affine *d_bases, const uint32_t *d_scalars, size_t n, bool mont, G2 *out, hipStream_t s, bool mostly_bits) {
    return msm_shared(nullptr, 0, d_bases, d_scalars, n, mont, nullptr, out, s, 0, 1, mostly_bits);
}

template <class F>
static int window_table_build_t(WindowTable &t, const Affine<F> *d_bases, size_t n, int c, hipStream_t s) {
    t.n = n; t.c = c; t.W = (SCALAR_BITS + c - 1) / c; t.g2 = sizeof(F) != sizeof(Fq);
    if (t.buf.reserve(std::max<size_t>(1, n) * t.W * sizeof(Affine<F>))) return ZKG_ERROR;
    if (!n) return ZKG_OK;
    Affine<F> *lv = t.buf.as<Affine<F>>();
    ZK_HIP(hipMemcpyAsync(lv, d_bases, n * sizeof(Affine<F>), hipMemcpyDeviceToDevice, s));
    constexpr int K = sizeof(F) != sizeof(Fq) ? 2 : 4;
    for (int w = 1; w < t.W; w += K)
        hipLaunchKernelGGL((k_table_levels<F, K>), dim3((unsigned)((n + 255) / 256)), dim3(256), 0, s, lv + (size_t)(w - 1) * n, lv + (size_t)w * n, n, (uint32_t)c,
                           std::min(K, t.W - w));
    if (hipGetLastError() != hipSuccess) { set_error("window table launch failed"); return ZKG_ERROR; }
    return ZKG_OK;
}
int window_table_build_g1(WindowTable &t, const G1Affine *d_bases, size_t n, int c, hipStream_t s) { return window_table_build_t<Fq>(t, d_bases, n, c, s); }
int window_table_records29(WindowTable &t, hipStream_t s) {
    if (t.g2) { set_error("window_table_records29: G1 tables only"); return ZKG_ERROR; }
    const size_t total = t.n * (size_t)t.W;
    if (t.rec29.reserve(std::max<size_t>(1, total) * sizeof(Rec64))) return ZKG_ERROR;
    if (total) hipLaunchKernelGGL(k_bases_to29, dim3((unsigned)((total + 255) / 256)), dim3(256), 0, s, t.buf.as<Affine<Fq>>(), total, t.rec29.as<Rec64>());
    if (hipGetLastError() != hipSuccess) { set_error("window table records launch failed"); return ZKG_ERROR; }
    return ZKG_OK;
}
int window_table_build_g2(WindowTable &t, const G2Affine *d_bases, size_t n, int c, hipStream_t s) { return window_table_build_t<Fq2>(t, d_bases, n, c, s); }

int witness_classify(const Fr *d_z, size_t n1, uint8_t *d_tags, uint32_t *d_listed, uint32_t *d_count, hipStream_t s, const uint32_t *d_subset_pos) {
    ZK_HIP(hipMemsetAsync(d_count, 0, 8, s));
    if (n1) hipLaunchKernelGGL(k_classify, dim3((unsigned)((n1 + 255) / 256)), dim3(256), 0, s, d_z, n1, d_tags, d_listed, d_count, d_subset_pos);
    return hipGetLastError() == hipSuccess ? ZKG_OK : ZKG_ERROR;
}
template <class F> static int gather_points_t(const Affine<F> *d_src, const uint32_t *d_idx, size_t count, uint32_t index_sub, Affine<F> *d_out, hipStream_t s) {
    if (count) hipLaunchKernelGGL(k_gather_points<F>, dim3((unsigned)((count + 255) / 256)), dim3(256), 0, s, d_src, d_idx, count, index_sub, d_out);
    return hipGetLastError() == hipSuccess ? ZKG_OK : ZKG_ERROR;
}
int gather_points_g1(const G1Affine *d_src, const uint32_t *d_idx, size_t count, uint32_t index_sub, G1Affine *d_out, hipStream_t s) { return gather_points_t<Fq>(d_src, d_idx, count, index_sub, d_out, s); }
int gather_points_g2(const G2Affine *d_src, const uint32_t *d_idx, size_t count, uint32_t index_sub, G2Affine *d_out, hipStream_t s) { return gather_points_t<Fq2>(d_src, d_idx, count, index_sub, d_out, s); }
template <class F> static int scatter_points_t(const Affine<F> *d_src, const uint32_t *d_idx, size_t count, Affine<F> *d_out, hipStream_t s) {
    if (count) hipLaunchKernelGGL(k_scatter_points<F>, dim3((unsigned)((count + 255) / 256)), dim3(256), 0, s, d_src, d_idx, count, d_out);
    return hipGetLastError() == hipSuccess ? ZKG_OK : ZKG_ERROR;
}
int scatter_points_g1(const G1Affine *d_src, const uint32_t *d_idx, size_t count, G1Affine *d_out, hipStream_t s) { return scatter_points_t<Fq>(d_src, d_idx, count, d_out, s); }
int scatter_points_g2(const G2Affine *d_src, const uint32_t *d_idx, size_t count, G2Affine *d_out, hipStream_t s) { return scatter_points_t<Fq2>(d_src, d_idx, count, d_out, s); }
template <class F>
static int ones_sum_launch_t(OnesSum &o, const MsmBases *sets, int nsets, const uint8_t *d_tags, size_t n1, hipStream_t s, size_t tag_stride = 0, uint32_t vecs = 1) {
    if (nsets < 1 || nsets > MSM_MAX_SETS) { set_error("ones-sum: bad set count"); return ZKG_ERROR; }
    const uint32_t span = (uint32_t)std::min<size_t>(8192, std::max<size_t>(1024, ((n1 + 255) / 256 + 255) / 256 * 256));
    const unsigned blocks = (unsigned)std::max<size_t>(1, (n1 + span - 1) / span);
    o.g2 = sizeof(F) != sizeof(Fq); o.nsets = nsets;
    const size_t vec_stride = (size_t)nsets * (blocks + 1), host_bytes = std::max<size_t>(MSM_MAX_SETS, (size_t)vecs * nsets) * sizeof(G2);
    if (o.partials.reserve(vecs * vec_stride * sizeof(XYZZ<F>))) return ZKG_ERROR;
    if (o.host_bytes < host_bytes) {
        if (o.host) (void)hipHostFree(o.host);
        o.host = nullptr; o.host_bytes = 0;
        if (!hip_ok(hipHostMalloc(&o.host, host_bytes, hipHostMallocDefault), "hipHostMalloc", __FILE__, __LINE__)) return ZKG_ERROR;
        o.host_bytes = host_bytes;
    }
    XYZZ<F> *part = o.partials.as<XYZZ<F>>();
    ViewSet<F> views;
    for (int i = 0; i < MSM_MAX_SETS; ++i) { const MsmBases &b = sets[i < nsets ? i : 0]; views.v[i] = BaseView<F>{reinterpret_cast<const Affine<F> *>(b.p), 0, nullptr, b.index_sub, 1, nullptr}; }
    hipLaunchKernelGGL(k_ones_sum<F>, dim3(blocks, (unsigned)nsets, vecs), dim3(256), 256 * sizeof(LdsPoint<F>) + (size_t)span * 4, s, views, d_tags, n1, span, part, tag_stride, vec_stride);
    hipLaunchKernelGGL(k_sum_partials<F>, dim3((unsigned)nsets, vecs), dim3(256), 256 * sizeof(LdsPoint<F>), s, part, blocks, vec_stride);
    if (hipGetLastError() != hipSuccess) { set_error("ones-sum launch failed"); return ZKG_ERROR; }
    if (vecs > 1) {
        ZK_HIP(hipMemcpy2DAsync(o.host, sizeof(XYZZ<F>), part + blocks, (blocks + 1) * sizeof(XYZZ<F>), sizeof(XYZZ<F>), (size_t)vecs * nsets, hipMemcpyDeviceToHost, s));
        return ZKG_OK;
    }
    for (int i = 0; i < nsets; ++i)
        ZK_HIP(hipMemcpyAsync((char *)o.host + (size_t)i * sizeof(XYZZ<F>), part + (size_t)i * (blocks + 1) + blocks, sizeof(XYZZ<F>), hipMemcpyDeviceToHost, s));
    return ZKG_OK;
}
int ones_sum_launch(OnesSum &o, const MsmBases *sets, int nsets, const uint8_t *d_tags, size_t n1, hipStream_t s) {
    for (int i = 1; i < nsets; ++i) if (sets[i].g2 != sets[0].g2) { set_error("ones-sum: one field per launch"); return ZKG_ERROR; }
    return sets[0].g2 ? ones_sum_launch_t<Fq2>(o, sets, nsets, d_tags, n1, s) : ones_sum_launch_t<Fq>(o, sets, nsets, d_tags, n1, s);
}
int ones_sum_launch_multi(OnesSum &o, const MsmBases *sets, int nsets, const uint8_t *d_tags, size_t tag_stride, size_t n1, uint32_t count, hipStream_t s) {
    for (int i = 1; i < nsets; ++i) if (sets[i].g2 != sets[0].g2) { set_error("ones-sum: one field per launch"); return ZKG_ERROR; }
    if (count < 1 || count > 65535) { set_error("ones-sum: bad witness count"); return ZKG_ERROR; }
    return sets[0].g2 ? ones_sum_launch_t<Fq2>(o, sets, nsets, d_tags, n1, s, tag_stride, count) : ones_sum_launch_t<Fq>(o, sets, nsets, d_tags, n1, s, tag_stride, count);
}
void OnesSum::release() { partials.release(); if (host) (void)hipHostFree(host); host = nullptr; host_bytes = 0; }

static constexpr int FB_WINDOWS = 32, FB_DIGITS = 255, FB_K = 4;
template <class F>
__global__ __launch_bounds__(256) void k_fixed_table(const Affine<F> *rows , Affine<F> *table) {
    const uint32_t t = blockIdx.x * blockDim.x + threadIdx.x;
    if (t >= FB_WINDOWS * FB_DIGITS) return;
    const uint32_t j = t / FB_DIGITS, d = t % FB_DIGITS + 1;
    const Affine<F> r = rows[j];
    XYZZ<F> acc = XYZZ<F>::inf();
    for (int bit = 7; bit >= 0; --bit) { acc = acc.dbl(); if ((d >> bit) & 1u) acc.madd(r); }
    XYZZ<F> fin = acc;
    table[t] = fin.to_affine().normalized();
}
template <class F>
__global__ __launch_bounds__(256) void k_fixed_base(const Affine<F> *table, const uint32_t *scalars, size_t n, int mont, Affine<F> *out) {
    const size_t lane = (size_t)blockIdx.x * blockDim.x + threadIdx.x, i0 = lane * FB_K;
    if (i0 >= n) return;
    F x[FB_K], y[FB_K], zz[FB_K], zzz[FB_K];
#pragma unroll
    for (int k = 0; k < FB_K; ++k) {
        XYZZ<F> acc = XYZZ<F>::inf();
        if (i0 + k < n) {
            Fr f;
            for (int j = 0; j < 8; ++j) f.v[j] = scalars[8 * (i0 + k) + j];
            if (mont) f = f.from_mont();
            else f = f.normalized();
            for (int j = 0; j < FB_WINDOWS; ++j) {
                const uint32_t d = (f.v[j >> 2] >> (8 * (j & 3))) & 255u;
                if (d) acc.madd(table[j * FB_DIGITS + d - 1]);
            }
        }
        x[k] = acc.x; y[k] = acc.y; zz[k] = acc.zz; zzz[k] = acc.zzz;
    }
    F pre[FB_K], run = F::one();
#pragma unroll
    for (int k = 0; k < FB_K; ++k) { pre[k] = run; if (!zzz[k].is_zero()) run = run * zzz[k]; }
    F inv = inverse_fast(run);
#pragma unroll
    for (int k = FB_K - 1; k >= 0; --k) {
        if (i0 + k >= n) continue;
        if (zzz[k].is_zero()) { out[i0 + k] = Affine<F>::inf(); continue; }
        F zi = inv * pre[k];
        inv = inv * zzz[k];
        F t = zi * zz[k];
        F zi2 = t.sqr();
        out[i0 + k] = Affine<F>{x[k] * zi2, y[k] * zi}.normalized();
    }
}

template <class F> struct FixedTableCache { std::mutex mu; std::vector<std::pair<Affine<F>, DevBuf>> entries; };
template <class F> static FixedTableCache<F> &fixed_cache() { static FixedTableCache<F> c; return c; }
template <class F>
static const Affine<F> *fixed_table_for(const Affine<F> &base, hipStream_t s) {
    FixedTableCache<F> &c = fixed_cache<F>();
    std::lock_guard<std::mutex> lk(c.mu);
    for (auto &e : c.entries) if (memcmp(&e.first, &base, sizeof(base)) == 0) return e.second.template as<Affine<F>>();
    std::vector<Affine<F>> rows(FB_WINDOWS);
    XYZZ<F> cur = XYZZ<F>::from_affine(base);
    for (int j = 0; j < FB_WINDOWS; ++j) { rows[j] = cur.to_affine(); for (int k = 0; k < 8; ++k) cur = cur.dbl(); }
    DevBuf d_rows, d_table;
    if (d_rows.reserve(rows.size() * sizeof(Affine<F>)) || d_table.reserve((size_t)FB_WINDOWS * FB_DIGITS * sizeof(Affine<F>))) return nullptr;
    if (!hip_ok(hipMemcpyAsync(d_rows.p, rows.data(), rows.size() * sizeof(Affine<F>), hipMemcpyHostToDevice, s), "H2D", __FILE__, __LINE__)) return nullptr;
    hipLaunchKernelGGL(k_fixed_table<F>, dim3((FB_WINDOWS * FB_DIGITS + 255) / 256), dim3(256), 0, s, d_rows.as<Affine<F>>(), d_table.as<Affine<F>>());
    const bool ok = hipGetLastError() == hipSuccess && hip_ok(hipStreamSynchronize(s), "sync", __FILE__, __LINE__);
    d_rows.release();
    if (!ok) { d_table.release(); set_error("fixed-base table build failed"); return nullptr; }
// ... 49 lines not shown
```

Baseline: 56.87.

## Fold top MSM window into spare bucket range using scalar parity split

For single-set G1 MSMs, the top signed-digit window is only partly used because the scalar has 254 bits. The change re-encodes top-window digits of odd scalars into the unused upper bucket range, offset by 2^t. The host combine step then subtracts the shifted suffix so the result stays correct. If any top digit does not fit, a pinned flag is set and the whole MSM is rerun without the split. This adds an extra readback-driven retry path and a small stats API.

```diff
diff --git a/include/zkg.h b/include/zkg.h
--- a/include/zkg.h
+++ b/include/zkg.h
@@ -87,6 +87,7 @@
                    uint64_t out_jac[24], void *stream);
 int zkg_msm_g1_host_scalars(const void *d_bases, const uint64_t *scalars, size_t n, int scalars_mont, uint64_t out_jac[12], void *stream);
 int zkg_msm_host_scalars_stats(uint32_t *out, int n);
+void zkg_msm_top_window_stats(uint32_t out[2]);
 typedef struct zkg_msm_bases zkg_msm_bases;
 zkg_msm_bases *zkg_msm_g1_bases_upload(const void *d_bases, size_t n);
 int zkg_msm_g1_resident(zkg_msm_bases *bases, const void *d_scalars, size_t n, int scalars_mont, uint64_t out_jac[12], void *stream);
diff --git a/zklaim_amd/__init__.py b/zklaim_amd/__init__.py
--- a/zklaim_amd/__init__.py
+++ b/zklaim_amd/__init__.py
@@ -4,4 +4,4 @@
                   libsnark_trusted_setup, libsnark_prove, libsnark_verify, zklaim_prove_batch, zklaim_verify_batch, zklaim_verify_batch_stats, proof_decode_gpu, zklaim_input_sums_gpu, zklaim_input_map_mirror, ctx_blob, COMPAT_SYMBOLS, field_op, fr29_op, FR29_OPS, fq29_op, FQ29_OPS, g1_add_quad29, g1_add_pair29, curve_op, CURVE_OPS, OK, ERROR, UNSATISFIED, init_multi, MsmShards, pk_blob_inspect, ResidentBases, msm_g1_host_scalars, msm_host_scalars_stats, msm_resident_async_stats, msm_combine_gpu, ResidentBasesG2, msm_combine_g2_gpu,
                   groth16_verify_each, verify_each_stats, verify_each_set_chunk, pairing_each, final_exp, fq12_op, FQ12_OPS,
                   point_decompress, point_compress, zklaim_verify_each, zklaim_verify_each_stats, zklaim_ic_each,
-                  Domain, domain_stats, Qap, qap_stats, qap_instance_stats)
+                  Domain, domain_stats, Qap, qap_stats, qap_instance_stats, msm_top_window_stats)
diff --git a/zklaim_amd/api.py b/zklaim_amd/api.py
--- a/zklaim_amd/api.py
+++ b/zklaim_amd/api.py
@@ -36,7 +36,7 @@
     "zkg_qap_new", "zkg_qap_free", "zkg_qap_domain_size", "zkg_qap_num_variables", "zkg_qap_batch_max", "zkg_qap_set_batch_max",
     "zkg_qap_witness_h_async", "zkg_qap_stats",
     "zkg_qap_instance_async", "zkg_qap_set_column_segment", "zkg_qap_instance_stats", "zkg_groth16_setup_dev",
-    "zkg_msm_host_scalars_stats",
+    "zkg_msm_host_scalars_stats", "zkg_msm_top_window_stats",
 ]
 COMPAT_SYMBOLS = ["libsnark_trusted_setup", "libsnark_prove", "libsnark_verify"]
 
@@ -420,6 +420,12 @@
     return {"pieces": pieces, "stream_waits": int(out[1]),
             "heavy": [None if out[2 + 2 * k] == 0xFFFFFFFF else int(out[2 + 2 * k]) for k in range(pieces)],
             "pair": [bool(out[3 + 2 * k]) for k in range(pieces)]}
+
+
+def msm_top_window_stats():
+    out = (C.c_uint32 * 2)()
+    lib().zkg_msm_top_window_stats(out)
+    return {"split": bool(out[0]), "repeated": bool(out[1])}
 
 
 class _ResidentBases:
diff --git a/zklaim_amd/csrc/capi.hip b/zklaim_amd/csrc/capi.hip
--- a/zklaim_amd/csrc/capi.hip
+++ b/zklaim_amd/csrc/capi.hip
@@ -760,6 +760,7 @@
     return ZKG_OK;
 }
 int zkg_msm_host_scalars_stats(uint32_t *out, int n) { return out && n >= 0 ? msm_host_scalars_stats(out, n) : 0; }
+void zkg_msm_top_window_stats(uint32_t out[2]) { if (out) msm_top_window_stats(out); }
 int zkg_msm_g1_windows_dev(const void *d_bases, const void *d_scalars, size_t n, int scalars_mont, unsigned first_window, unsigned window_stride,
                            uint64_t out_jac[12], void *stream) {
     REQUIRE_INIT();
diff --git a/zklaim_amd/csrc/common.hpp b/zklaim_amd/csrc/common.hpp
--- a/zklaim_amd/csrc/common.hpp
+++ b/zklaim_amd/csrc/common.hpp
@@ -164,6 +164,7 @@
 int msm_g1(const G1Affine *d_bases, const uint32_t *d_scalars, size_t n, bool scalars_mont, G1 *out, hipStream_t s, bool mostly_bits = false);
 int msm_g2(const G2Affine *d_bases, const uint32_t *d_scalars, size_t n, bool scalars_mont, G2 *out, hipStream_t s, bool mostly_bits = false);
 int msm_g1_host_scalars(const G1Affine *d_bases, const uint32_t *h_scalars, size_t n, bool scalars_mont, G1 *out, hipStream_t s);
+void msm_top_window_stats(uint32_t out[2]);
 int msm_host_scalars_stats(uint32_t *out, int n);
 int msm_shared(const G1Affine *const *d_g1_bases, int n_g1, const G2Affine *d_g2_bases, const uint32_t *d_scalars, size_t n,
                bool scalars_mont, G1 *out_g1, G2 *out_g2, hipStream_t s, uint32_t w0 = 0, uint32_t ws = 1,
diff --git a/zklaim_amd/csrc/host/horner_jac.hpp b/zklaim_amd/csrc/host/horner_jac.hpp
--- a/zklaim_amd/csrc/host/horner_jac.hpp
+++ b/zklaim_amd/csrc/host/horner_jac.hpp
@@ -63,4 +63,22 @@
     return r;
 }
 
+template <class F> static inline XYZZ<F> chunk_window_value(const XYZZ<F> *rec, uint32_t cpw, size_t slots, uint32_t chunk_log, uint32_t split_t = 0) {
+    XYZZ<F> Usum = XYZZ<F>::inf(), suffix = XYZZ<F>::inf(), weighted = XYZZ<F>::inf(), Asum = XYZZ<F>::inf(), moved = XYZZ<F>::inf();
+    const int split_ch = split_t ? (int)((1u << split_t) >> chunk_log) : -1;
+    for (int ch = (int)cpw - 1; ch >= 0; --ch) {
+        const XYZZ<F> &P = rec[slots * (size_t)ch], &U = rec[slots * (size_t)ch + 1];
+        Usum.add(U);
+        if (slots == 3) Asum.add(rec[slots * (size_t)ch + 2]);
+        if (ch >= 1) { suffix.add(P); weighted.add(suffix); }
+        else suffix.add(P);
+        if (ch == split_ch) moved = suffix;
+    }
+    if (slots == 3 && !Asum.is_inf()) Usum.add(xyzz_times_pow2(Asum, 3));
+    weighted = xyzz_times_pow2(weighted, chunk_log);
+    Usum.add(weighted); Usum.add(suffix);
+    if (!moved.is_inf()) Usum.add(xyzz_times_pow2(moved, split_t).neg());
+    return Usum;
 }
+
+}
diff --git a/zklaim_amd/csrc/msm.hip b/zklaim_amd/csrc/msm.hip
--- a/zklaim_amd/csrc/msm.hip
+++ b/zklaim_amd/csrc/msm.hip
@@ -26,7 +26,7 @@
 static constexpr int SORT_THREADS = 1024;
 static constexpr int SCAN_ITEMS = 4;
 
-struct MsmGeom { uint32_t c, W, B, Wt, w0, ws; };
+struct MsmGeom { uint32_t c, W, B, Wt, w0, ws, split_t; };
 struct SetLayout { size_t buckets, items, heavy, partials, folded, red_out; };
 template <class F> struct BaseView {
     const Affine<F> *p; size_t level_stride; const uint32_t *gather; uint32_t index_sub, B; const uint32_t *remap;
@@ -53,7 +53,18 @@
     if (c > MAX_C) c = MAX_C;
     MsmGeom g; g.c = c; g.Wt = (SCALAR_BITS + c - 1) / c; g.B = 1u << (c - 1);
     g.w0 = w0; g.ws = ws ? ws : 1; g.W = w0 < g.Wt ? (g.Wt - w0 + g.ws - 1) / g.ws : 0;
+    g.split_t = 0;
     return g;
+}
+static int pick_red_l_log(size_t red_buckets) {
+    static const char *force_l = getenv("ZKG_RED_L_LOG");
+    return force_l ? atoi(force_l) : red_buckets >= RED_LARGE_BUCKETS ? RED_L_LOG_LARGE : red_buckets > RED_SMALL_BUCKETS ? RED_L_LOG_SMALL : RED_L_LOG_TINY;
+}
+static uint32_t pick_top_split(const MsmGeom &g, int chunk_log) {
+    const uint32_t top = g.Wt - 1;
+    if (g.W == 0 || top < g.w0 || (top - g.w0) % g.ws != 0 || g.c * top >= 254) return 0;
+    const uint32_t t = 254 - g.c * top;
+    return t < 31 && ((uint64_t)2 << t) <= g.B && (uint32_t)chunk_log <= t ? t : 0;
 }
 
 ZK_D uint32_t bits_at(const uint32_t v[8], uint32_t off, uint32_t c) {
@@ -67,7 +78,12 @@
 ZK_D void sort_wave_priority() { __builtin_amdgcn_s_setprio(3); }
 
 
-struct ZeroList { uint32_t *p[4]; uint32_t words[4]; };
+struct ZeroList { uint32_t *p[4]; uint32_t words[4]; uint32_t *wide; };
+ZK_D uint32_t top_window_code(uint32_t code, uint32_t t, uint32_t odd, uint32_t *wide) {
+    if (!code) return 0;
+    if ((code >> 1) > (1u << t)) { *wide = 1u; return code; }
+    return code + (odd ? (1u << t) << 1 : 0u);
+}
 __global__ __launch_bounds__(256) void k_digits(const uint32_t *scalars, const uint32_t *gather, size_t n, int mont, MsmGeom g, uint32_t *digits, ZeroList zl) {
     sort_wave_priority();
     size_t i = (size_t)blockIdx.x * blockDim.x + threadIdx.x;
@@ -85,6 +101,7 @@
         uint32_t raw = bits_at(f.v, w * g.c, g.c) + carry, code = 0;
         if (raw > g.B) { uint32_t d = (1u << g.c) - raw; carry = 1; if (d) code = (d << 1) | 1u; }
         else { carry = 0; if (raw) code = raw << 1; }
+        if (g.split_t && w + 1 == g.Wt) code = top_window_code(code, g.split_t, f.v[0] & 1u, zl.wide);
         if (w == own) { digits[(size_t)slot * n + i] = code; ++slot; own += g.ws; }
     }
 }
@@ -114,7 +131,8 @@
         const bool neg = raw > B;
         const uint32_t d = neg ? (1u << C) - raw : raw;
         carry = neg ? 1u : 0u;
-        const uint32_t code = d ? (d << 1) | (neg ? 1u : 0u) : 0u;
+        uint32_t code = d ? (d << 1) | (neg ? 1u : 0u) : 0u;
+        if (w + 1 == WT && g.split_t) code = top_window_code(code, g.split_t, f.v[0] & 1u, zl.wide);
         if ((uint32_t)w == own) { digits[(size_t)slot * n + i] = code; ++slot; own += g.ws; }
     }
 }
@@ -210,6 +228,7 @@
             const uint32_t d = neg ? (1u << C) - raw : raw;
             carry[q] = neg ? 1u : 0u;
             code[q] = d ? (d << 1) | (neg ? 1u : 0u) : 0u;
+            if (w + 1 == WT && g.split_t) code[q] = top_window_code(code[q], g.split_t, f[q].v[0] & 1u, zl.wide);
         }
         *reinterpret_cast<uint4 *>(digits + (size_t)w * n + 4 * i) = make_uint4(code[0], code[1], code[2], code[3]);
     }
@@ -1182,6 +1201,7 @@
     bool heavy_pair = true;
     bool beside = false;
     bool timed = false;
+    uint32_t *wide_out = nullptr;
     uint32_t *stream_waits = nullptr;
 };
 struct MsmJob {
@@ -1199,6 +1219,11 @@
     bool dev_finish = false;
     uint32_t multi = 1; size_t multi_stride = 0;
     std::mutex mu;
+    uint32_t *wide_flag = nullptr;
+    int ensure_wide_flag() {
+        if (wide_flag || hipHostMalloc(reinterpret_cast<void **>(&wide_flag), sizeof(uint32_t), hipHostMallocDefault) == hipSuccess) return ZKG_OK;
+        wide_flag = nullptr; set_error("msm: pinned word of the top-window split"); return ZKG_ERROR;
+    }
     int ensure_side() {
         if (aux) return ZKG_OK;
         if (hipStreamCreateWithFlags(&aux, hipStreamNonBlocking) == hipSuccess && hipEventCreateWithFlags(&ev_fork, hipEventDisableTiming) == hipSuccess &&
@@ -1215,6 +1240,7 @@
         space.release();
         for (MsmGroup &gr : group) gr.release();
         release_side();
+        if (wide_flag) { (void)hipHostFree(wide_flag); wide_flag = nullptr; }
     }
 };
 struct MsmLaunchSets { MsmBases by_field[2][MSM_MAX_SETS]; MsmGeom g{}; size_t n = 0; bool empty = false; MsmSortSpace *space = nullptr; };
@@ -1232,8 +1258,7 @@
     gr.table = sets[0].level_stride != 0;
     gr.red_windows = gr.table ? P : g.W;
     const size_t red_buckets = (size_t)gr.red_windows * g.B;
-    static const char *force_l = getenv("ZKG_RED_L_LOG");
-    const int red_l_log = force_l ? atoi(force_l) : red_buckets >= RED_LARGE_BUCKETS ? RED_L_LOG_LARGE : red_buckets > RED_SMALL_BUCKETS ? RED_L_LOG_SMALL : RED_L_LOG_TINY;
+    const int red_l_log = pick_red_l_log(red_buckets);
     gr.chunk_log = RG::LANES_LOG + red_l_log;
     gr.cpw = (g.B + (1u << gr.chunk_log) - 1) >> gr.chunk_log; gr.nred = (size_t)gr.red_windows * gr.cpw;
     gr.red_slots = 2;
@@ -1347,18 +1372,7 @@
     const size_t sl = (size_t)gr.red_slots;
     std::vector<XYZZ<F>> V(W);
     auto window = [&](int w) {
-        XYZZ<F> Usum = XYZZ<F>::inf(), suffix = XYZZ<F>::inf(), weighted = XYZZ<F>::inf(), Asum = XYZZ<F>::inf();
-        for (int ch = (int)cpw - 1; ch >= 0; --ch) {
-            const XYZZ<F> &P = red[sl * ((size_t)w * cpw + ch)], &U = red[sl * ((size_t)w * cpw + ch) + 1];
-            Usum.add(U);
-            if (sl == 3) Asum.add(red[sl * ((size_t)w * cpw + ch) + 2]);
-            if (ch >= 1) { suffix.add(P); weighted.add(suffix); }
-            else suffix.add(P);
-        }
-        if (sl == 3 && !Asum.is_inf()) Usum.add(xyzz_times_pow2(Asum, 3));
-        weighted = xyzz_times_pow2(weighted, (uint32_t)gr.chunk_log);
-        Usum.add(weighted); Usum.add(suffix);
-        V[w] = Usum;
+        V[w] = chunk_window_value(red + sl * (size_t)w * cpw, cpw, sl, (uint32_t)gr.chunk_log, w + 1 == (int)W && !gr.table ? g.split_t : 0u);
     };
     if (multi) { window(vec); return V[vec]; }
     if (gr.table) {
@@ -1483,6 +1497,7 @@
     const bool two_pass = !job->one_pass_sort && g.c >= 12 && n >= 49152 && (n >> cbits) <= RX_FINE_MAX && n <= ((size_t)1 << (31 - (g.c - 1 - cbits)));
     {
         ZeroList zl{};
+        zl.wide = g0.split_t ? mode.wide_out : nullptr;
         int k = 0;
         zl.p[k] = chist; zl.words[k++] = (CLASS_HIST_COPIES + 1) * (HEAVY_T_MAX + 2);
         for (int f = 0; f < 2; ++f) if (job->group[f].nsets) {
@@ -1567,6 +1582,13 @@
 }
 
 static MsmJob g_default_job;
+struct TopWindowStats { uint32_t split = 0, repeated = 0; };
+static TopWindowStats g_top_window_stats;
+static bool top_window_repeat(const MsmJob &J, MsmLaunchMode &mode) {
+    if (!mode.wide_out || !*static_cast<volatile const uint32_t *>(J.wide_flag)) return false;
+    mode.wide_out = nullptr; g_top_window_stats.repeated = 1;
+    return true;
+}
 struct HostScalarsStats { uint32_t pieces = 0, waits = 0, heavy[8] = {0}, pair[8] = {0}; };
 struct PieceStep {
     DevBuf scalars; MsmSortSpace space;
@@ -1631,6 +1653,8 @@
     msm_job_split_sets(job, sets, nsets, n, d_gather != nullptr, ls);
     if (job->g.W == 0 || n == 0) { job->empty = ls.empty = true; return ZKG_OK; }
     if ((uint64_t)n * job->g.W >= ((uint64_t)1 << 32)) { set_error("msm: n * windows exceeds the 32-bit index space of the sorted list (n < 2^28)"); return ZKG_ERROR; }
+    if (mode.wide_out && nsets == 1 && !sets[0].g2 && !any_table && job->window_hint == 0)
+        job->g.split_t = pick_top_split(job->g, RedGeom<Fq>::LANES_LOG + pick_red_l_log((size_t)job->g.W * job->g.B));
     job->converted_aside = false;
     const MsmBases &g1 = ls.by_field[0][0];
     if (!any_table && !d_gather && job->group[0].nsets == 1 && g1.index_sub == 0 && !g1.remap && !g1.p29) {
@@ -1758,9 +1782,18 @@
     if (d_g2_bases) { sets[nsets] = MsmBases(); sets[nsets].p = d_g2_bases; sets[nsets].g2 = true; ++nsets; }
     if (n >= ((size_t)1 << 28)) { set_error("msm: at most 2^28 - 1 points per call"); return ZKG_ERROR; }
     const size_t PIECE = (size_t)1 << 23;
+    g_top_window_stats = TopWindowStats();
     if (n <= PIECE || w0 != 0 || g_default_job.ws != 1) {
-        if (msm_job_launch(&g_default_job, sets, nsets, d_scalars, n, scalars_mont, nullptr)) return ZKG_ERROR;
-        return msm_job_finish(&g_default_job, out_g1, out_g2);
+        MsmLaunchMode mode; mode.timed = true;
+        if (n_g1 == 1 && !d_g2_bases) {
+            if (g_default_job.ensure_wide_flag()) return ZKG_ERROR;
+            *g_default_job.wide_flag = 0; mode.wide_out = g_default_job.wide_flag;
+        }
+        for (;;) {
+            if (msm_job_launch_as(&g_default_job, sets, nsets, d_scalars, n, scalars_mont, nullptr, mode) || msm_job_finish(&g_default_job, out_g1, out_g2)) return ZKG_ERROR;
+            g_top_window_stats.split = g_default_job.g.split_t != 0;
+            if (!top_window_repeat(g_default_job, mode)) return ZKG_OK;
+        }
     }
     G1 acc1[MSM_MAX_SETS]; G2 acc2[MSM_MAX_SETS];
     for (int i = 0; i < MSM_MAX_SETS; ++i) { acc1[i] = G1::inf(); acc2[i] = G2::inf(); }
@@ -1790,6 +1823,7 @@
     }
     return P;
 }
+static int host_scalars_run(const G1Affine *d_bases, const uint32_t *h_scalars, size_t n, bool mont, G1 *out, hipStream_t s, int max_pieces, MsmLaunchMode mode);
 int msm_g1_host_scalars(const G1Affine *d_bases, const uint32_t *h_scalars, size_t n, bool mont, G1 *out, hipStream_t s) {
     if (n >= ((size_t)1 << 28)) { set_error("msm: at most 2^28 - 1 points per call"); return ZKG_ERROR; }
     if (!n) { *out = G1::inf(); return ZKG_OK; }
@@ -1801,15 +1835,28 @@
         ZK_HIP(hipMemcpyAsync(tmp.p, h_scalars, n * 32, hipMemcpyHostToDevice, s));
         return msm_g1(d_bases, tmp.as<uint32_t>(), n, mont, out, s, false);
     }
+    MsmJob &J = g_default_job;
+    std::lock_guard<std::mutex> lk(J.mu);
+    g_top_window_stats = TopWindowStats();
+    if (J.ensure_wide_flag()) return ZKG_ERROR;
+    *J.wide_flag = 0;
+    MsmLaunchMode mode; mode.wide_out = J.wide_flag;
+    for (;;) {
+        if (host_scalars_run(d_bases, h_scalars, n, mont, out, s, pieces ? max_pieces : 1, mode)) return ZKG_ERROR;
+        g_top_window_stats.split = J.g.split_t != 0;
+        if (!top_window_repeat(J, mode)) return ZKG_OK;
+    }
+}
+static int host_scalars_run(const G1Affine *d_bases, const uint32_t *h_scalars, size_t n, bool mont, G1 *out, hipStream_t s, int max_pieces, MsmLaunchMode mode) {
     MsmJob &J = g_default_job; PieceStep &T = g_step;
-    std::lock_guard<std::mutex> lk(J.mu);
+    const bool pieces = max_pieces > 1;
     g_dominant_timer.new_call();
     if (T.scalars.reserve(n * 32)) return ZKG_ERROR;
     uint32_t *d_sc = T.scalars.as<uint32_t>();
     J.stream = s; J.w0 = 0; J.ws = 1; J.one_pass_sort = false;
     MsmBases set; set.p = d_bases;
     T.stats = HostScalarsStats();
-    MsmLaunchMode mode; mode.timed = true; mode.stream_waits = &T.stats.waits;
+    mode.timed = true; mode.stream_waits = &T.stats.waits;
     if (!pieces) {
         ZK_HIP(hipMemcpyAsync(d_sc, h_scalars, n * 32, hipMemcpyHostToDevice, s));
         if (msm_job_launch_as(&J, &set, 1, d_sc, n, mont, nullptr, mode)) return ZKG_ERROR;
@@ -1875,6 +1922,11 @@
     return words;
 }
 
+void msm_top_window_stats(uint32_t out[2]) {
+    std::lock_guard<std::mutex> lk(g_default_job.mu);
+    out[0] = g_top_window_stats.split; out[1] = g_top_window_stats.repeated;
+}
+
 int msm_g1(const G1Affine *d_bases, const uint32_t *d_scalars, size_t n, bool mont, G1 *out, hipStream_t s, bool mostly_bits) {
     return msm_shared(&d_bases, 1, nullptr, d_scalars, n, mont, out, nullptr, s, 0, 1, mostly_bits);
 }
```

After: 57.06, median of 6. About the same (+0.3%).
